# wing02/MyLdpcCppApi

Measured on AMD Instinct MI355X. Metric: decoded Mbit/s (info bits), DVB-S2 N=64800 rate-1/2, 50 iters, higher is better.
Workload: dtype f32; 1 GPU; DVB-S2-profile (64800,32400) rate-1/2 (seeded IRA table with the standard's structure, E=226799), batch 4096 frames per GPU, 50 iterations, sum-product fp32 (probability domain), all-zero codeword + AWGN sigma=0.95 (no frame converges), early termination on, inputs resident in HBM; global_batch=4096, frames_per_gpu=4096, algo=sp, frames_per_launch=4096, parallelism=frames sharded over 1 GPU(s), all-gather of decoded bytes, frames_converged=0

## Files before the change

include/ldpc_hip.h:

```cpp
#ifndef LDPC_HIP_H_
#define LDPC_HIP_H_

#include <stddef.h>
#include <stdint.h>

#ifdef __cplusplus
extern "C" {
#endif

#define LDPC_HIP_ABI_VERSION 3

enum ldpc_status {
    LDPC_OK = 0,
    LDPC_ERR_ARG = 1,
    LDPC_ERR_HIP = 2,
    LDPC_ERR_NOMEM = 3,
    LDPC_ERR_UNSUPPORTED = 4,
    LDPC_ERR_STATE = 5
};

enum ldpc_algo {
    LDPC_ALGO_SP = 0,
    LDPC_ALGO_MS = 1,
    LDPC_ALGO_LAYERED = 2,
// ... 75 lines not shown

typedef struct ldpc_decode_stats {
    int32_t iterations_launched;
    int32_t batch_time;
    int64_t frames;
    int64_t frames_converged;
    float ms_total;
    float ms_check;
    float ms_var;
    float ms_other;
    int32_t launches_check;
    int32_t launches_var;
    int64_t frame_rounds;
} ldpc_decode_stats;

int ldpc_abi_version(void);
const char *ldpc_last_error(void);
int ldpc_device_count(int *count);

int ldpc_graph_create(const int32_t *rows, const int32_t *cols, int64_t E, int32_t M, int32_t N,
                      ldpc_graph **out);
int ldpc_graph_destroy(ldpc_graph *g);
int ldpc_graph_info(const ldpc_graph *g, int32_t *M, int32_t *N, int64_t *E, int32_t *max_row_deg,
                    int32_t *max_col_deg);

void ldpc_decoder_config_init(ldpc_decoder_config *cfg);
int ldpc_decoder_config_init_sized(ldpc_decoder_config *cfg, uint32_t struct_size);
#define ldpc_decoder_config_init(cfg) ((void)ldpc_decoder_config_init_sized((cfg), (uint32_t)sizeof(ldpc_decoder_config)))
int ldpc_decoder_create(const ldpc_graph *g, const ldpc_decoder_config *cfg, ldpc_decoder **out);
int ldpc_decoder_create_multi(const ldpc_graph *g, const ldpc_decoder_config *cfg, const int32_t *devices,
                              int32_t n_devices, ldpc_decoder **out);
int ldpc_decoder_destroy(ldpc_decoder *d);
int ldpc_shard_range(int64_t frames, int32_t part, int32_t parts, int32_t unit, int64_t *lo, int64_t *hi);

int ldpc_decode(ldpc_decoder *d, const float *llr_host, int64_t frames, uint8_t *out_host,
                int64_t out_bytes, int32_t *iters);

int ldpc_decode_device(ldpc_decoder *d, const float *llr_dev, int64_t frames, uint8_t *out_dev,
                       int64_t out_bytes, int32_t *iters_dev, void *stream);

int64_t ldpc_out_bytes(int32_t K, int64_t frames, int32_t pack_mode);

enum ldpc_soft_kind { LDPC_SOFT_POSTERIOR = 1, LDPC_SOFT_EXTRINSIC = 2 };
int ldpc_decode_soft_device(ldpc_decoder *d, const float *llr_dev, int64_t frames, uint8_t *out_dev, int64_t out_bytes,
                            int32_t *iters_dev, float *soft_dev, int64_t soft_floats, int32_t soft_kind, void *stream);
int ldpc_decode_soft(ldpc_decoder *d, const float *llr_host, int64_t frames, uint8_t *out_host, int64_t out_bytes,
                     int32_t *iters, float *soft_host, int64_t soft_floats, int32_t soft_kind);

enum ldpc_llr_type { LDPC_LLR_F32 = 0, LDPC_LLR_F16 = 1, LDPC_LLR_I8 = 2 };
int ldpc_decode_typed_device(ldpc_decoder *d, const void *llr_dev, int32_t llr_type, float llr_unit, int64_t frames,
                             uint8_t *out_dev, int64_t out_bytes, int32_t *iters_dev, void *stream);
int ldpc_decode_soft_typed_device(ldpc_decoder *d, const void *llr_dev, int32_t llr_type, float llr_unit, int64_t frames,
                                  uint8_t *out_dev, int64_t out_bytes, int32_t *iters_dev, float *soft_dev,
                                  int64_t soft_floats, int32_t soft_kind, void *stream);
int ldpc_decode_typed(ldpc_decoder *d, const void *llr_host, int32_t llr_type, float llr_unit, int64_t frames,
                      uint8_t *out_host, int64_t out_bytes, int32_t *iters);
int ldpc_decode_soft_typed(ldpc_decoder *d, const void *llr_host, int32_t llr_type, float llr_unit, int64_t frames,
                           uint8_t *out_host, int64_t out_bytes, int32_t *iters, float *soft_host, int64_t soft_floats,
                           int32_t soft_kind);
int ldpc_llr_quantize_device(const float *y_dev, int64_t count, int32_t llr_type, float llr_unit, void *out_dev,
                             int32_t device, void *stream);

int ldpc_decoder_set_timing(ldpc_decoder *d, int enable);
int ldpc_decoder_stats(ldpc_decoder *d, ldpc_decode_stats *stats);
int ldpc_decoder_crc_stops(ldpc_decoder *d, int64_t *frames);

typedef struct ldpc_kernel_time {
    int32_t phase;
    int32_t degree;
    int32_t launches;
    float ms_total;
    int64_t bytes_total;
    char name[64];
    int64_t bytes_moved;
} ldpc_kernel_time;
int ldpc_decoder_kernel_times(ldpc_decoder *d, ldpc_kernel_time *out, int32_t capacity,
                              int32_t *count);

int ldpc_decoder_link_form(ldpc_decoder *d, int32_t *form, int32_t *calibrated, float ms[3]);

int ldpc_decoder_placement(ldpc_decoder *d, int32_t *candidates, int32_t *kept, float ms[16]);
int ldpc_decoder_array_addresses(ldpc_decoder *d, uint64_t out[4]);

int ldpc_decoder_set_tap(ldpc_decoder *d, int32_t iter);
int ldpc_decoder_dump(ldpc_decoder *d, int32_t which, float *host_out, int64_t count);

int ldpc_awgn_device(float *llr_dev, int64_t frames, int32_t N, const uint8_t *bits_dev, float sd,
                     uint64_t seed, int64_t first_frame, int32_t device, void *stream);
int ldpc_count_errors_device(const uint8_t *out_dev, const uint8_t *ref_dev, int64_t frames,
                             int64_t bytes_per_frame, int64_t errors[3], int32_t device, void *stream);

typedef struct ldpc_encoder ldpc_encoder;
enum ldpc_code_format {
    LDPC_CODE_PACKED = 0,
    LDPC_CODE_BITS = 1
};
enum ldpc_parity_kind { LDPC_PARITY_DUAL_DIAGONAL = 1, LDPC_PARITY_STAIRCASE = 2, LDPC_PARITY_DENSE = 3  };
int ldpc_parity_structure(const ldpc_graph *g, int32_t K, int32_t block_rows, int32_t out[8]);
int ldpc_encoder_create(const ldpc_graph *g, int32_t K, int32_t block_rows, int32_t max_frames, int32_t device,
                        ldpc_encoder **out);
int ldpc_encoder_destroy(ldpc_encoder *e);
int ldpc_encode_device(ldpc_encoder *e, const uint8_t *src_dev, int64_t src_bytes, int64_t frames, uint8_t *code_dev,
                       int64_t code_bytes, int32_t format, void *stream);
int ldpc_encode(ldpc_encoder *e, const uint8_t *src_host, int64_t src_bytes, uint8_t *code_host, int64_t code_bytes);
int64_t ldpc_code_bytes(int32_t N, int64_t frames, int32_t format);

int ldpc_graph_systematic_order(const ldpc_graph *g, int32_t *perm , int32_t *rank);
int ldpc_parity_dense(const ldpc_graph *g, int32_t K, int64_t out[4]);
int ldpc_parity_dense_rows(const ldpc_graph *g, int32_t K, int32_t first, int32_t rows, uint64_t *t_out, int64_t words);
int ldpc_encoder_create_dense(const ldpc_graph *g, int32_t K, int32_t max_frames, int32_t device, ldpc_encoder **out);

typedef struct ldpc_rate_spec {
    uint32_t struct_size;
    int32_t  N;
    int32_t  punctured;
    int32_t  filler_lo, filler_hi;
    float    fill_llr;
    float    erasure_llr;
} ldpc_rate_spec;
void ldpc_rate_spec_init(ldpc_rate_spec *spec, int32_t N);
int ldpc_rate_lengths(const ldpc_rate_spec *spec, int32_t *Ncb, int32_t *L);
int ldpc_rate_index(const ldpc_rate_spec *spec, int32_t k0, int32_t E, int32_t *index_out);
int ldpc_rate_match_device(const ldpc_rate_spec *spec, const uint8_t *code_dev, int32_t code_format, int64_t frames, int32_t k0,
                           int32_t E, uint8_t *tx_dev, int64_t tx_bytes, int32_t tx_format, int32_t device, void *stream);
int ldpc_rate_recover_device(const ldpc_rate_spec *spec, const float *rx_dev, int64_t frames, int32_t k0, int32_t E, float *soft_dev,
                             int32_t accumulate, float *y_dev, int32_t device, void *stream);
int ldpc_rate_match(const ldpc_rate_spec *spec, const uint8_t *code_host, int32_t code_format, int64_t frames, int32_t k0, int32_t E,
                    uint8_t *tx_host, int64_t tx_bytes, int32_t tx_format, int32_t device);
int ldpc_rate_recover(const ldpc_rate_spec *spec, const float *rx_host, int64_t frames, int32_t k0, int32_t E, float *soft_host,
                      int32_t accumulate, float *y_host, int32_t device);

typedef struct ldpc_modem_spec {
    uint32_t struct_size;
    int32_t  Qm;
    int32_t  interleave;
} ldpc_modem_spec;
void ldpc_modem_spec_init(ldpc_modem_spec *spec, int32_t Qm);
int64_t ldpc_modem_symbol_floats(const ldpc_modem_spec *spec, int32_t E);
int ldpc_modem_index(const ldpc_modem_spec *spec, int32_t E, int32_t *index_out);
int ldpc_modem_points(int32_t Qm, float *iq);
int ldpc_modem_transmit_device(const ldpc_modem_spec *spec, const uint8_t *tx_dev, int32_t tx_format, int64_t frames, int32_t E,
                               float sd, uint64_t seed, int64_t first_frame, float *sym_dev, int64_t sym_floats, int32_t device,
                               void *stream);
int ldpc_modem_demap_device(const ldpc_modem_spec *spec, const float *sym_dev, int64_t frames, int32_t E, float *rx_dev,
                            int32_t device, void *stream);
int ldpc_modem_transmit(const ldpc_modem_spec *spec, const uint8_t *tx_host, int32_t tx_format, int64_t frames, int32_t E, float sd,
                        uint64_t seed, int64_t first_frame, float *sym_host, int64_t sym_floats, int32_t device);
int ldpc_modem_demap(const ldpc_modem_spec *spec, const float *sym_host, int64_t frames, int32_t E, float *rx_host, int32_t device);

enum ldpc_crc_kind { LDPC_CRC16 = 16, LDPC_CRC24A = 24, LDPC_CRC24B = 25 };
typedef struct ldpc_tb_spec {
    uint32_t struct_size;
    int32_t  A;
    int32_t  tb_crc;
    int32_t  C;
    int32_t  cb_crc;
    int32_t  K;
} ldpc_tb_spec;
void ldpc_tb_spec_init(ldpc_tb_spec *spec, int32_t A, int32_t K);
int ldpc_tb_layout(const ldpc_tb_spec *spec, int32_t out[6]);
int ldpc_crc_bits(int32_t kind, const uint8_t *bytes, int64_t nbits, uint32_t *crc);
int ldpc_crc_weights(int32_t kind, int32_t nbits, uint32_t *w);
int ldpc_tb_frame_crc(const ldpc_tb_spec *spec, int32_t *kind, int32_t *bits);
int ldpc_tb_attach_device(const ldpc_tb_spec *spec, const uint8_t *payload_dev, int64_t tbs, uint8_t *src_dev, int64_t src_bytes,
                          int32_t device, void *stream);
int ldpc_tb_check_device(const ldpc_tb_spec *spec, const uint8_t *dec_dev, int64_t tbs, uint8_t *payload_dev, uint8_t *cb_ok_dev,
// ... 50 lines not shown
```

myldpccppapi_amd/_lib.py:

```python
import ctypes
import os
import sys

_HERE = os.path.dirname(os.path.abspath(__file__))
LIB_PATH = os.environ.get("LDPC_HIP_LIB") or os.path.join(_HERE, "libldpc_hip.so")
_lib = None


class LdpcError(RuntimeError):
    def __init__(self, code, message):
        super().__init__("ldpc_hip error %d: %s" % (code, message))
        self.code = code


class DecoderConfig(ctypes.Structure):
    _fields_ = [("struct_size", ctypes.c_uint32), ("K", ctypes.c_int32),
                ("max_batch", ctypes.c_int32), ("algo", ctypes.c_int32),
                ("msg_dtype", ctypes.c_int32), ("max_iter", ctypes.c_int32),
                ("llr_scale", ctypes.c_float), ("early_term", ctypes.c_int32),
                ("device", ctypes.c_int32), ("layer_rows", ctypes.c_int32),
                ("pack_mode", ctypes.c_int32), ("frames_per_lane", ctypes.c_int32),
                ("poll_interval", ctypes.c_int32),
                ("tune_flags", ctypes.c_int32), ("tune_rows_per_wave", ctypes.c_int32),
                ("tune_cols_per_wave", ctypes.c_int32), ("tune_link_rows", ctypes.c_int32),
                ("tune_compact", ctypes.c_int32), ("tune_ldsp_grid", ctypes.c_int32),
                ("tune_ldsp_shape", ctypes.c_int32), ("tune_place", ctypes.c_int32),
                ("host_input", ctypes.c_int32),
                ("host_copy_threads", ctypes.c_int32), ("tune_q_order", ctypes.c_int32),
                ("ms_scale", ctypes.c_float), ("ms_offset", ctypes.c_float)]


class DecoderConfigCrc(DecoderConfig):
    _fields_ = [("crc_kind", ctypes.c_int32), ("crc_bits", ctypes.c_int32)]


class _MsgTail(ctypes.Union):
    _fields_ = [("msg_reserved", ctypes.c_int32 * 3), ("post_bits", ctypes.c_int32)]


class DecoderConfigMsg(DecoderConfigCrc):
    _anonymous_ = ("_tail",)
    _fields_ = [("msg_bits", ctypes.c_int32), ("_tail", _MsgTail)]


class DecodeStats(ctypes.Structure):
    _fields_ = [("iterations_launched", ctypes.c_int32), ("batch_time", ctypes.c_int32),
                ("frames", ctypes.c_int64), ("frames_converged", ctypes.c_int64),
                ("ms_total", ctypes.c_float), ("ms_check", ctypes.c_float),
                ("ms_var", ctypes.c_float), ("ms_other", ctypes.c_float),
                ("launches_check", ctypes.c_int32), ("launches_var", ctypes.c_int32),
                ("frame_rounds", ctypes.c_int64)]


class KernelTime(ctypes.Structure):
    _fields_ = [("phase", ctypes.c_int32), ("degree", ctypes.c_int32), ("launches", ctypes.c_int32),
                ("ms_total", ctypes.c_float), ("bytes_total", ctypes.c_int64), ("name", ctypes.c_char * 64),
                ("bytes_moved", ctypes.c_int64)]


class RateSpec(ctypes.Structure):
    _fields_ = [("struct_size", ctypes.c_uint32), ("N", ctypes.c_int32), ("punctured", ctypes.c_int32),
                ("filler_lo", ctypes.c_int32), ("filler_hi", ctypes.c_int32),
                ("fill_llr", ctypes.c_float), ("erasure_llr", ctypes.c_float)]


class ModemSpec(ctypes.Structure):
    _fields_ = [("struct_size", ctypes.c_uint32), ("Qm", ctypes.c_int32), ("interleave", ctypes.c_int32)]


class TbSpec(ctypes.Structure):
    _fields_ = [("struct_size", ctypes.c_uint32), ("A", ctypes.c_int32), ("tb_crc", ctypes.c_int32), ("C", ctypes.c_int32),
                ("cb_crc", ctypes.c_int32), ("K", ctypes.c_int32)]


class BchSpec(ctypes.Structure):
    _fields_ = [("struct_size", ctypes.c_uint32), ("m", ctypes.c_int32), ("prim", ctypes.c_uint32), ("t", ctypes.c_int32),
                ("n", ctypes.c_int32), ("row_bytes", ctypes.c_int32)]


EXPORTS = (
    "ldpc_abi_version", "ldpc_last_error", "ldpc_device_count", "ldpc_graph_create",
    "ldpc_graph_destroy", "ldpc_graph_info", "ldpc_decoder_config_init", "ldpc_decoder_create",
    "ldpc_decoder_create_multi", "ldpc_shard_range", "ldpc_decoder_destroy", "ldpc_decode", "ldpc_decode_device", "ldpc_out_bytes",
    "ldpc_decoder_set_timing", "ldpc_decoder_stats", "ldpc_decoder_kernel_times", "ldpc_decoder_set_tap",
    "ldpc_decoder_dump", "ldpc_awgn_device", "ldpc_count_errors_device", "ldpc_hbm_probe_device", "ldpc_hbm_sustained_device",
    "ldpc_host_block_plan", "ldpc_host_locked_ranges", "ldpc_decoder_link_form", "ldpc_decoder_placement", "ldpc_decoder_array_addresses",
    "ldpc_parity_structure", "ldpc_encoder_create", "ldpc_encoder_destroy", "ldpc_encode_device", "ldpc_encode", "ldpc_code_bytes",
    "ldpc_rate_spec_init", "ldpc_rate_lengths", "ldpc_rate_index", "ldpc_rate_match_device", "ldpc_rate_recover_device",
    "ldpc_rate_match", "ldpc_rate_recover",
    "ldpc_modem_spec_init", "ldpc_modem_symbol_floats", "ldpc_modem_index", "ldpc_modem_points", "ldpc_modem_transmit_device",
    "ldpc_modem_demap_device", "ldpc_modem_transmit", "ldpc_modem_demap",
    "ldpc_tb_spec_init", "ldpc_tb_layout", "ldpc_crc_bits", "ldpc_tb_attach_device", "ldpc_tb_check_device", "ldpc_tb_tally_device",
    "ldpc_tb_attach", "ldpc_tb_check",
    "ldpc_decoder_crc_stops", "ldpc_crc_weights", "ldpc_tb_frame_crc", "ldpc_decoder_config_init_sized",
    "ldpc_decode_soft_device", "ldpc_decode_soft",
    "ldpc_decode_typed_device", "ldpc_decode_soft_typed_device", "ldpc_decode_typed", "ldpc_decode_soft_typed",
    "ldpc_llr_quantize_device",
    "ldpc_bch_spec_init", "ldpc_bch_layout", "ldpc_bch_generator", "ldpc_bch_encode_device", "ldpc_bch_decode_device",
    "ldpc_bch_tally_device", "ldpc_bch_encode", "ldpc_bch_decode",
    "ldpc_osd_create", "ldpc_osd_destroy", "ldpc_osd_device", "ldpc_osd_run", "ldpc_osd_info",
    "ldpc_graph_systematic_order", "ldpc_parity_dense", "ldpc_parity_dense_rows", "ldpc_encoder_create_dense",
)


def load():
    global _lib
    if _lib is not None:
        return _lib
    if not os.path.exists(LIB_PATH):
        raise OSError("%s not built: run `python -c 'import __graft_entry__ as g; g.build()'` "
                      "or `make -C myldpccppapi_amd/csrc`" % LIB_PATH)
    if "torch" not in sys.modules:
        try:
            import torch
        except Exception:
            pass
    L = ctypes.CDLL(LIB_PATH, mode=ctypes.RTLD_GLOBAL)
    i32p = ctypes.POINTER(ctypes.c_int32)
    i64p = ctypes.POINTER(ctypes.c_int64)
    vp = ctypes.c_void_p
    L.ldpc_abi_version.restype = ctypes.c_int
    L.ldpc_last_error.restype = ctypes.c_char_p
    L.ldpc_device_count.argtypes = [ctypes.POINTER(ctypes.c_int)]
    L.ldpc_graph_create.argtypes = [i32p, i32p, ctypes.c_int64, ctypes.c_int32, ctypes.c_int32,
                                    ctypes.POINTER(vp)]
    L.ldpc_graph_destroy.argtypes = [vp]
    L.ldpc_graph_info.argtypes = [vp, i32p, i32p, i64p, i32p, i32p]
    L.ldpc_decoder_config_init.argtypes = [ctypes.POINTER(DecoderConfig)]
    L.ldpc_decoder_config_init.restype = None
    L.ldpc_decoder_config_init_sized.argtypes = [ctypes.POINTER(DecoderConfig), ctypes.c_uint32]
    L.ldpc_decoder_create.argtypes = [vp, ctypes.POINTER(DecoderConfig), ctypes.POINTER(vp)]
    L.ldpc_decoder_create_multi.argtypes = [vp, ctypes.POINTER(DecoderConfig), i32p, ctypes.c_int32,
                                            ctypes.POINTER(vp)]
    L.ldpc_shard_range.argtypes = [ctypes.c_int64, ctypes.c_int32, ctypes.c_int32, ctypes.c_int32, i64p, i64p]
    L.ldpc_decoder_destroy.argtypes = [vp]
    L.ldpc_decode.argtypes = [vp, vp, ctypes.c_int64, vp, ctypes.c_int64, vp]
    L.ldpc_decode_device.argtypes = [vp, vp, ctypes.c_int64, vp, ctypes.c_int64, vp, vp]
    L.ldpc_decode_soft.argtypes = [vp, vp, ctypes.c_int64, vp, ctypes.c_int64, vp, vp, ctypes.c_int64, ctypes.c_int32]
    L.ldpc_decode_soft_device.argtypes = [vp, vp, ctypes.c_int64, vp, ctypes.c_int64, vp, vp, ctypes.c_int64, ctypes.c_int32, vp]
    f32, i32 = ctypes.c_float, ctypes.c_int32
    L.ldpc_decode_typed.argtypes = [vp, vp, i32, f32, ctypes.c_int64, vp, ctypes.c_int64, vp]
    L.ldpc_decode_typed_device.argtypes = [vp, vp, i32, f32, ctypes.c_int64, vp, ctypes.c_int64, vp, vp]
    L.ldpc_decode_soft_typed.argtypes = [vp, vp, i32, f32, ctypes.c_int64, vp, ctypes.c_int64, vp, vp, ctypes.c_int64, i32]
    L.ldpc_decode_soft_typed_device.argtypes = [vp, vp, i32, f32, ctypes.c_int64, vp, ctypes.c_int64, vp, vp, ctypes.c_int64, i32, vp]
    L.ldpc_llr_quantize_device.argtypes = [vp, ctypes.c_int64, i32, f32, vp, i32, vp]
    L.ldpc_out_bytes.argtypes = [ctypes.c_int32, ctypes.c_int64, ctypes.c_int32]
    L.ldpc_out_bytes.restype = ctypes.c_int64
    L.ldpc_decoder_set_timing.argtypes = [vp, ctypes.c_int]
    L.ldpc_decoder_stats.argtypes = [vp, ctypes.POINTER(DecodeStats)]
    L.ldpc_decoder_kernel_times.argtypes = [vp, ctypes.POINTER(KernelTime), ctypes.c_int32, i32p]
    L.ldpc_decoder_set_tap.argtypes = [vp, ctypes.c_int32]
    L.ldpc_decoder_dump.argtypes = [vp, ctypes.c_int32, vp, ctypes.c_int64]
    L.ldpc_awgn_device.argtypes = [vp, ctypes.c_int64, ctypes.c_int32, vp, ctypes.c_float, ctypes.c_uint64,
                                   ctypes.c_int64, ctypes.c_int32, vp]
    L.ldpc_count_errors_device.argtypes = [vp, vp, ctypes.c_int64, ctypes.c_int64, i64p, ctypes.c_int32, vp]
    L.ldpc_hbm_sustained_device.argtypes = [ctypes.c_int32, ctypes.c_int64, ctypes.c_int32, ctypes.POINTER(ctypes.c_double)]
    L.ldpc_hbm_probe_device.argtypes = [ctypes.c_int32, ctypes.c_int64, ctypes.c_int32,
                                        ctypes.POINTER(ctypes.c_double), ctypes.POINTER(ctypes.c_double)]
    L.ldpc_host_block_plan.argtypes = [ctypes.c_uint64, ctypes.c_int64, ctypes.c_int32, ctypes.c_int32, ctypes.c_int64,
                                       ctypes.POINTER(ctypes.c_uint64)]
    L.ldpc_host_locked_ranges.argtypes = [i64p, i64p]
    L.ldpc_decoder_array_addresses.argtypes = [vp, ctypes.POINTER(ctypes.c_uint64)]
    L.ldpc_decoder_placement.argtypes = [vp, i32p, i32p, ctypes.POINTER(ctypes.c_float)]
    L.ldpc_decoder_link_form.argtypes = [vp, i32p, i32p, ctypes.POINTER(ctypes.c_float)]
    L.ldpc_parity_structure.argtypes = [vp, ctypes.c_int32, ctypes.c_int32, i32p]
    L.ldpc_encoder_create.argtypes = [vp, ctypes.c_int32, ctypes.c_int32, ctypes.c_int32, ctypes.c_int32, ctypes.POINTER(vp)]
    L.ldpc_encoder_destroy.argtypes = [vp]
    L.ldpc_encode_device.argtypes = [vp, vp, ctypes.c_int64, ctypes.c_int64, vp, ctypes.c_int64, ctypes.c_int32, vp]
    L.ldpc_encode.argtypes = [vp, vp, ctypes.c_int64, vp, ctypes.c_int64]
    L.ldpc_code_bytes.argtypes = [ctypes.c_int32, ctypes.c_int64, ctypes.c_int32]
    L.ldpc_code_bytes.restype = ctypes.c_int64
    rsp = ctypes.POINTER(RateSpec)
    L.ldpc_rate_spec_init.argtypes = [rsp, ctypes.c_int32]
    L.ldpc_rate_spec_init.restype = None
    L.ldpc_rate_lengths.argtypes = [rsp, i32p, i32p]
    L.ldpc_rate_index.argtypes = [rsp, ctypes.c_int32, ctypes.c_int32, vp]
    L.ldpc_rate_match_device.argtypes = [rsp, vp, ctypes.c_int32, ctypes.c_int64, ctypes.c_int32, ctypes.c_int32, vp,
                                         ctypes.c_int64, ctypes.c_int32, ctypes.c_int32, vp]
    L.ldpc_rate_recover_device.argtypes = [rsp, vp, ctypes.c_int64, ctypes.c_int32, ctypes.c_int32, vp, ctypes.c_int32, vp,
                                           ctypes.c_int32, vp]
    L.ldpc_rate_match.argtypes = [rsp, vp, ctypes.c_int32, ctypes.c_int64, ctypes.c_int32, ctypes.c_int32, vp,
                                  ctypes.c_int64, ctypes.c_int32, ctypes.c_int32]
    L.ldpc_rate_recover.argtypes = [rsp, vp, ctypes.c_int64, ctypes.c_int32, ctypes.c_int32, vp, ctypes.c_int32, vp,
                                    ctypes.c_int32]
    msp = ctypes.POINTER(ModemSpec)
    L.ldpc_modem_spec_init.argtypes = [msp, ctypes.c_int32]
    L.ldpc_modem_spec_init.restype = None
    L.ldpc_modem_symbol_floats.argtypes = [msp, ctypes.c_int32]
    L.ldpc_modem_symbol_floats.restype = ctypes.c_int64
    L.ldpc_modem_index.argtypes = [msp, ctypes.c_int32, vp]
    L.ldpc_modem_points.argtypes = [ctypes.c_int32, vp]
    L.ldpc_modem_transmit_device.argtypes = [msp, vp, ctypes.c_int32, ctypes.c_int64, ctypes.c_int32, ctypes.c_float, ctypes.c_uint64,
                                             ctypes.c_int64, vp, ctypes.c_int64, ctypes.c_int32, vp]
    L.ldpc_modem_demap_device.argtypes = [msp, vp, ctypes.c_int64, ctypes.c_int32, vp, ctypes.c_int32, vp]
    L.ldpc_modem_transmit.argtypes = [msp, vp, ctypes.c_int32, ctypes.c_int64, ctypes.c_int32, ctypes.c_float, ctypes.c_uint64,
                                      ctypes.c_int64, vp, ctypes.c_int64, ctypes.c_int32]
    L.ldpc_modem_demap.argtypes = [msp, vp, ctypes.c_int64, ctypes.c_int32, vp, ctypes.c_int32]
    tsp = ctypes.POINTER(TbSpec)
    L.ldpc_tb_spec_init.argtypes = [tsp, ctypes.c_int32, ctypes.c_int32]
    L.ldpc_tb_spec_init.restype = None
    L.ldpc_tb_layout.argtypes = [tsp, i32p]
    L.ldpc_crc_bits.argtypes = [ctypes.c_int32, vp, ctypes.c_int64, ctypes.POINTER(ctypes.c_uint32)]
    L.ldpc_tb_attach_device.argtypes = [tsp, vp, ctypes.c_int64, vp, ctypes.c_int64, ctypes.c_int32, vp]
    L.ldpc_tb_check_device.argtypes = [tsp, vp, ctypes.c_int64, vp, vp, vp, ctypes.c_int32, vp]
    L.ldpc_tb_tally_device.argtypes = [vp, vp, vp, ctypes.c_int64, ctypes.c_int64, i64p, ctypes.c_int32, vp]
    L.ldpc_tb_attach.argtypes = [tsp, vp, ctypes.c_int64, vp, ctypes.c_int64, ctypes.c_int32]
    L.ldpc_tb_check.argtypes = [tsp, vp, ctypes.c_int64, vp, vp, vp, ctypes.c_int32]
    L.ldpc_decoder_crc_stops.argtypes = [vp, i64p]
    L.ldpc_crc_weights.argtypes = [ctypes.c_int32, ctypes.c_int32, vp]
    L.ldpc_tb_frame_crc.argtypes = [tsp, i32p, i32p]
    bsp = ctypes.POINTER(BchSpec)
    L.ldpc_bch_spec_init.argtypes = [bsp, ctypes.c_int32, ctypes.c_int32, ctypes.c_int32]
    L.ldpc_bch_spec_init.restype = None
    L.ldpc_bch_layout.argtypes = [bsp, i32p]
    L.ldpc_bch_generator.argtypes = [ctypes.c_int32, ctypes.c_uint32, ctypes.c_int32, vp, ctypes.c_int32, i32p]
    L.ldpc_bch_encode_device.argtypes = [bsp, vp, ctypes.c_int64, vp, ctypes.c_int64, ctypes.c_int32, vp]
    L.ldpc_bch_decode_device.argtypes = [bsp, vp, ctypes.c_int64, vp, vp, ctypes.c_int32, vp]
    L.ldpc_bch_tally_device.argtypes = [vp, vp, vp, ctypes.c_int64, ctypes.c_int64, i64p, ctypes.c_int32, vp]
    L.ldpc_bch_encode.argtypes = [bsp, vp, ctypes.c_int64, vp, ctypes.c_int64, ctypes.c_int32]
    L.ldpc_bch_decode.argtypes = [bsp, vp, ctypes.c_int64, vp, vp, ctypes.c_int32]
    L.ldpc_osd_create.argtypes = [vp, i32, i32, i32, ctypes.POINTER(vp)]
    L.ldpc_osd_destroy.argtypes = [vp]
    L.ldpc_osd_device.argtypes = [vp, vp, ctypes.c_int64, i32, f32, vp, ctypes.c_int64, vp, vp, vp, vp]
    L.ldpc_osd_run.argtypes = [vp, vp, ctypes.c_int64, i32, f32, vp, ctypes.c_int64, vp, vp, vp]
    L.ldpc_osd_info.argtypes = [vp, i32p]
    L.ldpc_graph_systematic_order.argtypes = [vp, vp, i32p]
    L.ldpc_parity_dense.argtypes = [vp, i32, i64p]
    L.ldpc_parity_dense_rows.argtypes = [vp, i32, i32, i32, vp, ctypes.c_int64]
    L.ldpc_encoder_create_dense.argtypes = [vp, i32, i32, i32, ctypes.POINTER(vp)]
    _lib = L
    return L


def check(rc):
    if rc != 0:
        raise LdpcError(rc, load().ldpc_last_error().decode("utf-8", "replace"))
```

myldpccppapi_amd/capi.py:

```python
import ctypes

import numpy as np

from . import _lib
from ._lib import DecoderConfig, DecodeStats, LdpcError

ALGO_SP, ALGO_MS, ALGO_LAYERED, ALGO_MS_FUSED, ALGO_LAYERED_HOST, ALGO_BP, ALGO_LAYERED_BP = 0, 1, 2, 3, 4, 5, 6
ALGO_LAYERED_FX = 8
MSG_F32, MSG_F16, MSG_F8, MSG_I8 = 0, 1, 2, 4
PACK_BYTES, PACK_BITS = 0, 1
CODE_PACKED, CODE_BITS = 0, 1
CODE_FORMATS = {"packed": CODE_PACKED, "bits": CODE_BITS}
PARITY_KINDS = {1: "dual_diagonal", 2: "staircase", 3: "dense"}
HOST_INPUT = {"auto": 0, "staged": 1, "lock_pages": 2}
SOFT_POSTERIOR, SOFT_EXTRINSIC = 1, 2
SOFT_KINDS = {"posterior": SOFT_POSTERIOR, "extrinsic": SOFT_EXTRINSIC}
LLR_F32, LLR_F16, LLR_I8 = 0, 1, 2
LLR_TYPES = {"f32": LLR_F32, "f16": LLR_F16, "i8": LLR_I8}
LLR_DTYPES = {np.dtype(np.float32): LLR_F32, np.dtype(np.float16): LLR_F16, np.dtype(np.int8): LLR_I8}
ALGOS = {"sp": ALGO_SP, "ms": ALGO_MS, "layered": ALGO_LAYERED, "ms_fused": ALGO_MS_FUSED,
         "layered_host": ALGO_LAYERED_HOST, "bp": ALGO_BP, "layered_bp": ALGO_LAYERED_BP, "layered_fx": ALGO_LAYERED_FX}

TUNE_FIELDS = {"fused": 0, "ldsp": 2, "ldsp_ext": 4, "ldsp_pack": 6, "link_narrow": 8, "check_wide": 10,
               "syn_xcd": 12, "fused_pack": 14, "fused_loop": 16, "device_tail": 18, "merge": 20, "link_deep": 22, "link_half": 24,
               "link_guided": 26, "tiles_first": 28}
TUNE_INTS = ("rows_per_wave", "cols_per_wave", "link_rows", "compact", "ldsp_grid", "ldsp_per_cu", "ldsp_waves", "place", "q_order")


def apply_tune(cfg, tune):
    flags, shape = 0, 0
    for k, v in (tune or {}).items():
        if k in TUNE_FIELDS:
            if v is not None:
                flags |= (1 if v else 2) << TUNE_FIELDS[k]
        elif k == "ldsp_per_cu":
            shape |= int(v) & 255
        elif k == "ldsp_waves":
            shape |= (int(v) & 255) << 8
        elif k in TUNE_INTS:
            setattr(cfg, "tune_" + k, int(v))
        else:
            raise KeyError("unknown tuning field %r" % k)
    cfg.tune_flags, cfg.tune_ldsp_shape = flags, shape


def hbm_probe(device=0, nbytes=1 << 30, reps=5, by_policy=False):
    g = ctypes.c_double(0.0)
    two = (ctypes.c_double * 2)(0.0, 0.0)
    _lib.check(_lib.load().ldpc_hbm_probe_device(int(device), int(nbytes), int(reps), ctypes.byref(g), two))
    return (g.value, two[0], two[1]) if by_policy else g.value


def hbm_sustained(device=0, nbytes=1 << 30, milliseconds=300):
    g = ctypes.c_double(0.0)
    _lib.check(_lib.load().ldpc_hbm_sustained_device(int(device), int(nbytes), int(milliseconds), ctypes.byref(g)))
    return g.value


def tune_from_env(env=None):
    import os
    env = os.environ if env is None else env
    t = {}
    for name, key in (("FUSED", "fused"), ("LDSP", "ldsp"), ("LDSP_EXT", "ldsp_ext"), ("LDSP_PACK", "ldsp_pack"),
                      ("LINK_NARROW", "link_narrow"), ("CHECK_WIDE", "check_wide"), ("SYN_XCD", "syn_xcd"),
                      ("FUSED_LOOP", "fused_loop"), ("DEVICE_TAIL", "device_tail"), ("MERGE", "merge"), ("LINK_DEEP", "link_deep"), ("LINK_HALF", "link_half"),
                      ("LINK_GUIDED", "link_guided"), ("TILES_FIRST", "tiles_first")):
        if "LDPC_TUNE_" + name in env:
            t[key] = int(env["LDPC_TUNE_" + name]) != 0
    if "LDPC_TUNE_NO_PACK" in env:
        t["fused_pack"] = False
    for name, key in (("RPW", "rows_per_wave"), ("CPW", "cols_per_wave"), ("LDSP_GRID", "ldsp_grid"),
                      ("LDSP_PER_CU", "ldsp_per_cu"), ("LDSP_WAVES", "ldsp_waves")):
        if "LDPC_TUNE_" + name in env:
            t[key] = int(env["LDPC_TUNE_" + name])
    for name, key in (("LINK_RPW", "link_rows"), ("COMPACT", "compact")):
        if "LDPC_TUNE_" + name in env:
            v = int(env["LDPC_TUNE_" + name])
            t[key] = v if v > 0 else -1
    return t


def shard_range(frames, part, parts, unit=1):
    lo, hi = ctypes.c_int64(), ctypes.c_int64()
    _lib.check(_lib.load().ldpc_shard_range(int(frames), int(part), int(parts), int(unit),
                                            ctypes.byref(lo), ctypes.byref(hi)))
    return lo.value, hi.value


def host_block_plan(base, frames, N, max_batch, group):
    out = (ctypes.c_uint64 * 6)()
    _lib.check(_lib.load().ldpc_host_block_plan(int(base), int(frames), int(N), int(max_batch), int(group), out))
    return tuple(int(x) for x in out)


def host_locked_ranges():
    a, b = ctypes.c_int64(-1), ctypes.c_int64(-1)
    _lib.check(_lib.load().ldpc_host_locked_ranges(ctypes.byref(a), ctypes.byref(b)))
    return a.value, b.value


def device_count():
    n = ctypes.c_int(0)
    rc = _lib.load().ldpc_device_count(ctypes.byref(n))
    return n.value if rc == 0 else 0


def quantize_device(y_ptr, count, llr_type, llr_unit, out_ptr, device=0, stream=None):
    _lib.check(_lib.load().ldpc_llr_quantize_device(y_ptr, int(count), LLR_TYPES.get(llr_type, llr_type), float(llr_unit), out_ptr,
                                                    int(device), stream))


def out_bytes(K, frames, pack_mode=PACK_BYTES):
    return int(_lib.load().ldpc_out_bytes(K, frames, pack_mode))


def code_bytes(N, frames, fmt="packed"):
    return int(_lib.load().ldpc_code_bytes(int(N), int(frames), CODE_FORMATS.get(fmt, fmt)))


def parity_structure(graph, K, block_rows=0):
    out = (ctypes.c_int32 * 8)()
    _lib.check(_lib.load().ldpc_parity_structure(graph._h, int(K), int(block_rows), out))
    return dict(kind=PARITY_KINDS[out[0]], c=out[1], x=out[2], a=out[3], b=out[4], ext_rows=out[5], z=out[6])
# ... 5 lines not shown
    _lib.check(_lib.load().ldpc_graph_systematic_order(graph._h, perm.ctypes.data, ctypes.byref(rank)))
    return perm, rank.value


def dense_parity(graph, K):
    out = (ctypes.c_int64 * 4)()
    _lib.check(_lib.load().ldpc_parity_dense(graph._h, int(K), out))
    return dict(rho=out[0], rank_hp=out[1], M=out[2], t_words=out[3])


def dense_parity_rows(graph, K, first, rows):
    tw = (graph.M + 63) // 64
    out = np.zeros((max(int(rows), 0), tw), np.uint64)
    _lib.check(_lib.load().ldpc_parity_dense_rows(graph._h, int(K), int(first), int(rows), out.ctypes.data, out.size))
    return out


class Graph:

    def __init__(self, rows, cols, M, N):
        L = _lib.load()
        self.rows = np.ascontiguousarray(rows, np.int32)
        self.cols = np.ascontiguousarray(cols, np.int32)
        if self.rows.shape != self.cols.shape or self.rows.ndim != 1:
            raise ValueError("rows and cols must be 1-D arrays of equal length")
        self.M, self.N, self.E = int(M), int(N), int(self.rows.size)
        self._h = ctypes.c_void_p()
        i32p = ctypes.POINTER(ctypes.c_int32)
        _lib.check(L.ldpc_graph_create(self.rows.ctypes.data_as(i32p), self.cols.ctypes.data_as(i32p),
                                       self.E, self.M, self.N, ctypes.byref(self._h)))

    def info(self):
        L = _lib.load()
        M, N, rd, cd = (ctypes.c_int32() for _ in range(4))
        E = ctypes.c_int64()
        _lib.check(L.ldpc_graph_info(self._h, ctypes.byref(M), ctypes.byref(N), ctypes.byref(E),
                                     ctypes.byref(rd), ctypes.byref(cd)))
        return dict(M=M.value, N=N.value, E=E.value, max_row_deg=rd.value, max_col_deg=cd.value)

    def close(self):
        h, self._h = getattr(self, "_h", None), None
        if h and _lib is not None and _lib._lib is not None:
            _lib._lib.ldpc_graph_destroy(h)

    def __del__(self):
        try:
            self.close()
        except Exception:
            pass


class Decoder:

    def __init__(self, graph, K, max_batch, algo="sp", max_iter=40, llr_scale=8.0, early_term=True,
                 device=0, layer_rows=0, pack_mode=PACK_BYTES, frames_per_lane=0, poll_interval=0,
                 msg_dtype=MSG_F32, tune=None, devices=None, host_input="auto", host_copy_threads=0,
                 ms_scale=0.0, ms_offset=0.0, crc_kind=0, crc_bits=0, msg_bits=0, post_bits=0):
        L = _lib.load()
        cfg = _lib.DecoderConfigMsg()
        _lib.check(L.ldpc_decoder_config_init_sized(ctypes.byref(cfg), ctypes.sizeof(cfg)))
        cfg.K, cfg.max_batch = int(K), int(max_batch)
        cfg.algo = ALGOS[algo] if isinstance(algo, str) else int(algo)
        cfg.msg_dtype = {"f32": MSG_F32, "f16": MSG_F16, "f8": MSG_F8, "i8": MSG_I8}.get(msg_dtype, msg_dtype)
        cfg.msg_bits = int(msg_bits)
        cfg.post_bits = int(post_bits)
        cfg.max_iter, cfg.llr_scale = int(max_iter), float(llr_scale)
        cfg.early_term, cfg.device, cfg.layer_rows = int(bool(early_term)), int(device), int(layer_rows)
        cfg.pack_mode, cfg.frames_per_lane, cfg.poll_interval = int(pack_mode), int(frames_per_lane), int(poll_interval)
        apply_tune(cfg, tune)
        cfg.host_input = HOST_INPUT[host_input] if isinstance(host_input, str) else int(host_input)
        cfg.host_copy_threads = int(host_copy_threads)
        cfg.ms_scale, cfg.ms_offset = float(ms_scale), float(ms_offset)
        cfg.crc_kind, cfg.crc_bits = int(CRC_KINDS.get(crc_kind, crc_kind)), int(crc_bits)
        self.cfg = cfg
        self.graph = graph
        self.K, self.N, self.E = int(K), graph.N, graph.E
        self._h = ctypes.c_void_p()
        if devices is None:
            _lib.check(L.ldpc_decoder_create(graph._h, ctypes.byref(cfg), ctypes.byref(self._h)))
        else:
            devs = (ctypes.c_int32 * len(devices))(*[int(x) for x in devices])
            _lib.check(L.ldpc_decoder_create_multi(graph._h, ctypes.byref(cfg), devs, len(devices),
                                                   ctypes.byref(self._h)))

    def decode(self, llr, want_iters=True, soft=None, llr_unit=None):
        L = _lib.load()
        if llr_unit is not None:
            llr = np.asarray(llr)
            if llr.dtype not in LLR_DTYPES:
                raise TypeError("llr_unit given: llr must be int8, float16 or float32, not %s" % llr.dtype)
            llr = np.ascontiguousarray(llr).reshape(-1, self.N)
            frames, ty = llr.shape[0], LLR_DTYPES[llr.dtype]
            out = np.zeros(out_bytes(self.K, frames, self.cfg.pack_mode), np.uint8)
            iters = np.zeros(frames, np.int32)
            if soft is None:
                _lib.check(L.ldpc_decode_typed(self._h, llr.ctypes.data, ty, float(llr_unit), frames, out.ctypes.data, out.size,
                                               iters.ctypes.data if want_iters else None))
                return out, iters
            vals = np.zeros((frames, self.N), np.float32)
            _lib.check(L.ldpc_decode_soft_typed(self._h, llr.ctypes.data, ty, float(llr_unit), frames, out.ctypes.data, out.size,
                                                iters.ctypes.data if want_iters else None, vals.ctypes.data, vals.size,
                                                SOFT_KINDS.get(soft, soft)))
            return out, iters, vals
        llr = np.ascontiguousarray(llr, np.float32).reshape(-1, self.N)
        frames = llr.shape[0]
        out = np.zeros(out_bytes(self.K, frames, self.cfg.pack_mode), np.uint8)
        iters = np.zeros(frames, np.int32)
        if soft is None:
            _lib.check(L.ldpc_decode(self._h, llr.ctypes.data, frames, out.ctypes.data, out.size,
                                     iters.ctypes.data if want_iters else None))
            return out, iters
        vals = np.zeros((frames, self.N), np.float32)
        _lib.check(L.ldpc_decode_soft(self._h, llr.ctypes.data, frames, out.ctypes.data, out.size,
                                      iters.ctypes.data if want_iters else None, vals.ctypes.data, vals.size,
                                      SOFT_KINDS.get(soft, soft)))
        return out, iters, vals

    def decode_device(self, llr_ptr, frames, out_ptr, out_nbytes, iters_ptr=None, stream=None, soft_ptr=None, soft_floats=0,
                      soft="posterior", llr_type=None, llr_unit=None):
        if llr_type is not None or llr_unit is not None:
            ty = LLR_TYPES.get(llr_type, llr_type) if llr_type is not None else LLR_F32
            unit = 1.0 if llr_unit is None else float(llr_unit)
            if soft_ptr is None and not soft_floats:
                _lib.check(_lib.load().ldpc_decode_typed_device(self._h, llr_ptr, ty, unit, frames, out_ptr, out_nbytes, iters_ptr,
                                                                stream))
            else:
                _lib.check(_lib.load().ldpc_decode_soft_typed_device(self._h, llr_ptr, ty, unit, frames, out_ptr, out_nbytes,
                                                                     iters_ptr, soft_ptr, int(soft_floats),
                                                                     SOFT_KINDS.get(soft, soft), stream))
        elif soft_ptr is None and not soft_floats:
            _lib.check(_lib.load().ldpc_decode_device(self._h, llr_ptr, frames, out_ptr, out_nbytes,
                                                      iters_ptr, stream))
        else:
            _lib.check(_lib.load().ldpc_decode_soft_device(self._h, llr_ptr, frames, out_ptr, out_nbytes, iters_ptr, soft_ptr,
                                                           int(soft_floats), SOFT_KINDS.get(soft, soft), stream))

    def set_timing(self, enable=True):
        _lib.check(_lib.load().ldpc_decoder_set_timing(self._h, int(enable)))

    def stats(self):
        st = DecodeStats()
        _lib.check(_lib.load().ldpc_decoder_stats(self._h, ctypes.byref(st)))
        return {f: getattr(st, f) for f, _ in st._fields_}

    def crc_stops(self):
        n = ctypes.c_int64(0)
        _lib.check(_lib.load().ldpc_decoder_crc_stops(self._h, ctypes.byref(n)))
        return n.value

    def kernel_times(self):
        arr = (_lib.KernelTime * 64)()
        n = ctypes.c_int32(0)
        _lib.check(_lib.load().ldpc_decoder_kernel_times(self._h, arr, 64, ctypes.byref(n)))
        return [dict(name=arr[i].name.decode(), phase=arr[i].phase, degree=arr[i].degree,
                     launches=arr[i].launches, ms_total=arr[i].ms_total, bytes_total=arr[i].bytes_total,
                     bytes_moved=arr[i].bytes_moved)
                for i in range(n.value)]

    def link_form(self):
        form, cal = ctypes.c_int32(-1), ctypes.c_int32(0)
        ms = (ctypes.c_float * 3)()
        _lib.check(_lib.load().ldpc_decoder_link_form(self._h, ctypes.byref(form), ctypes.byref(cal), ms))
        if form.value < 0:
            return None
        return {"form": ("wide", "narrow", "half")[form.value], "chosen_by_measurement": bool(cal.value),
                "ms_per_launch": {"wide": round(ms[0], 4), "narrow": round(ms[1], 4), "half": round(ms[2], 4)}}
# ... 365 lines not shown
```

myldpccppapi_amd/csrc/decoder.hpp:

```cpp
#pragma once

#include <hip/hip_runtime.h>
#include <stdint.h>

#include <memory>
#include <type_traits>
#include <vector>

#include "../../include/ldpc_hip.h"
#include "flood_tables.hpp"
#include "layered_kernels.hpp"
#include "fused_kernels.hpp"
#include "ldsp_kernels.hpp"
#include "engines.hpp"
#include "tune.hpp"
#include "host_stage.hpp"
#include "hip_host.hpp"

#ifndef LDPC_IDLE_FAT
#define LDPC_IDLE_FAT 8
#endif

namespace ldpc {

template <typename Fn> inline int dispatch_v(int V, Fn &&fn)
{
    return V == 1 ? fn(std::integral_constant<int, 1>{})
                  : V == 2 ? fn(std::integral_constant<int, 2>{}) : fn(std::integral_constant<int, 4>{});
}

template <typename Fn> inline void dispatch_msg(int msg_kind, Fn &&fn)
{
    if (msg_kind == LDPC_MSG_I8) fn(q8any{});
    else if (msg_kind == LDPC_MSG_F8) fn(f8{});
    else if (msg_kind == LDPC_MSG_F16) fn(_Float16{});
    else fn(float{});
}

struct RowClass {
    int degree = 0;
    int count = 0;
    DevBuf<int32_t> e0;
    std::vector<int32_t> h_e0;
    DevBuf<int32_t> link_col, link_pos;
    int linked = 0;
    int n_big = 0, small_rows = 1;
};
struct ColClass {
    int degree = 0;
    int count = 0;
    DevBuf<int32_t> col, edge;
    int64_t q_base = -1;
};

struct ClassGroup {
    int bucket = 0, lo = 0, hi = 0;
    int blocks = 0;
    int blocks_fat = 0;
    std::vector<int> members;
    DevBuf<GroupClass> table, table_fat;
};

constexpr int kIdleFat = LDPC_IDLE_FAT;

struct FloodPlan {
    DevBuf<uint8_t> chan, Q, R;
    int msg_size = 4;
    int msg_kind = LDPC_MSG_F32;
    int msg_bits = 0;
    DevBuf<int32_t> qpos, col_qedge;
    std::vector<int32_t> h_qpos;
    std::vector<RowClass> row_classes;
    std::vector<ColClass> col_classes;
    std::vector<ClassGroup> check_groups, var_groups;
    std::vector<int> check_solo, var_solo;
    DevBuf<int32_t> extra_e0, extra_deg;
    int n_extra = 0;
    int64_t extra_edges = 0;
    FloodFns fns;

    int link_form = 1;
    bool link_deep = false;
    bool syn_xcd = true;
    bool check_wide = false;
    int link_rpw = 16;
    int cus = 256;
    bool link_calibrated = false;
    float link_cal_ms[3] = {0, 0, 0};
    int place_candidates = 0, place_kept = 0;
    float place_ms[16] = {};

    bool tail_enabled = false;
    int TO = 0, TA = 0;
    DevBuf<int32_t> tail_state, tail_map, running;

    std::unique_ptr<ldpc_decoder> child;
    DevBuf<int32_t> cmap;
    DevBuf<int32_t> cinv;
    DevBuf<unsigned long long> cmoved;
    int child_capacity = kCompactCapacity;
    int compact_threshold = kCompactCapacity;
    bool is_child = false;
    ldpc_decoder *handed_to = nullptr;
    HostBuf<int32_t> h_active;
    DevBuf<int32_t> soft_map;

    HostBuf<int32_t> h_summary;
    Event ev_summary;
    bool summary_pending = false;
    int idle_after = 0;

    bool first_round_from_chan = false;
};

struct HostSlot {
    DevBuf<float> llr;
    DevBuf<uint8_t> out;
    DevBuf<int32_t> iters;
    HostBuf<uint8_t> h_out;
    HostBuf<int32_t> h_iters;
    DevBuf<float> soft;
    HostBuf<float> h_soft;
    HostBuf<uint8_t> h_head;
    Event h2d_done, all_done;
    bool busy = false;
    int64_t off = 0, n = 0, dst = 0, copy_bytes = 0;
    HostBuf<int32_t> h_sum;
    int g_iterations = 0, g_tiles = 0, g_children = 0, g_child_f[3] = {0, 0, 0};
};
struct RingChunk { HostBuf<uint8_t> h; Event ev; bool used = false; };
struct CallCounts { bool valid = false; int32_t iterations = 0, batch_time = 0; int64_t frames = 0, converged = 0, frame_rounds = 0, crc_stops = 0; };

struct HostPath {
    Stream copy_stream;
    HostSlot slot[3];
    CallCounts call;
    bool suppress_poll = false;
    std::vector<RingChunk> ring;
    size_t ring_next = 0;
    std::unique_ptr<Worker> stager;
    std::vector<std::unique_ptr<Worker>> copy_helpers;
    std::vector<Job> copy_jobs;
    Job stage_job[3];
    bool stage_pending[3] = {false, false, false};
    std::vector<void *> locked_blocks, stuck_blocks;
};

struct TimedSpan {
    Event a, b;
    int kind = 0;
    int degree = 0;
    int64_t bytes = 0;
    int64_t moved = 0;
    int lo = 0;
};

struct Timing {
    bool timing = false;
    int timing_every = 0;
    int64_t timing_calls = 0;
    std::vector<TimedSpan> spans;
// ... 105 lines not shown
```

myldpccppapi_amd/csrc/engine_flood.hip:

```cpp
#include <hip/hip_runtime.h>

#include <algorithm>
#include <map>
#include <vector>

#include "flood_round.hpp"
#include "flood_handover.hpp"
#include "crc_term_kernels.hpp"
#include "soft_kernels.hpp"
#include "decoder.hpp"
#include "graph.hpp"

using ldpc::set_error;

namespace {

using ldpc::DevBuf;
using ldpc::RowClass;
using ldpc::ColClass;
using ldpc::ClassGroup;
using ldpc::kIdleFat;
using ldpc::dispatch_v;
using ldpc::span_begin;
using ldpc::span_end;
using ldpc::kVarBuckets;
using ldpc::kCheckBuckets;
using ldpc::kVarBucketLo;
using ldpc::kVarBucketHi;
using ldpc::kCheckBucketLo;
using ldpc::kCheckBucketHi;

template <int V>
__global__ void summary_kernel(const int32_t *iters, const uint64_t *done, const uint64_t *fail,
                               int64_t frames, int32_t freeze, int32_t *summary)
{
    constexpr int F = 64 * V;
    const int64_t f = (int64_t)blockIdx.x * blockDim.x + threadIdx.x;
    if (f >= frames) return;
    const int64_t tile = f / F;
    const int fi = (int)(f % F);
    const int l = fi / V, v = fi % V;
    atomicMax(&summary[0], iters[f]);
    const uint64_t ok = freeze ? done[tile * V + v] : ~fail[tile * V + v];
    if ((ok >> l) & 1ull) atomicAdd(&summary[1], 1);
}

static inline dim3 flood_grid(const ldpc_decoder *d, unsigned blocks, unsigned tiles, int32_t *tiles_first, bool linked = false)
{
    const bool want = d->tune.tiles_first == 1 || (d->tune.tiles_first == 0 && linked);
    *tiles_first = (blocks <= 65535u && want) ? 1 : 0;
    return *tiles_first ? dim3(tiles, blocks) : dim3(blocks, tiles);
}

static ldpc::CheckArgs check_args(const ldpc_decoder *d, const ldpc::TailRef &tr, int rows_per_wave, bool from_chan,
                                  const int32_t *e0 = nullptr, int n_rows = 0, int degree = 0)
{
    ldpc::CheckArgs a{d->flood.Q.p, d->flood.R.p, e0, d->done.p, d->E, n_rows, rows_per_wave, degree, d->ms_scale, tr};
    a.ms_offset = d->ms_offset;
    a.qpos = d->flood.qpos.p;
    if (from_chan) { a.first_chan = d->flood.chan.p; a.edge_col = d->edge_col.p; a.N = d->N; }
    return a;
}

template <int V> int run_flooding(ldpc_decoder *d, const ldpc::LlrIn &llr, int64_t frames,
                                  uint8_t *out_dev, int64_t out_bytes, int32_t *iters_dev,
                                  hipStream_t s, int start_round = 1);

template <int V> int enqueue_check_phase(ldpc_decoder *d, hipStream_t s, int tiles, int64_t frames, int it, int max_iter,
                                         bool fat, const ldpc::TailRef &tr)
{
    using namespace ldpc;
    const int64_t msz = d->flood.msg_size;
    const bool from_chan = it == 1 && d->flood.first_round_from_chan;
    for (auto &rc : d->flood.row_classes) {
        if (!rc.linked) continue;
        LDPC_HIP_TRY(span_begin(d, s, 4, rc.degree,
                           (2 * msz * rc.degree * rc.count + msz * 5 * rc.linked + 2 * msz * d->flood.extra_edges) * frames,
                           msz * ((int64_t)rc.degree * rc.count + rc.linked +
                                  ((int64_t)rc.degree * rc.count - 2 * rc.linked) +
                                  (it < max_iter ? 2 * rc.linked : 0) + 2 * d->flood.extra_edges) * frames));
        CheckArgs a = check_args(d, tr, d->flood.link_rpw, false, rc.e0.p, rc.count, rc.degree);
        const bool soft_reads = d->soft.dst && (d->cfg.early_term || it == max_iter);
        LinkArgs lk{rc.link_col.p, rc.link_pos.p, d->flood.chan.p, d->flood.Q.p, d->hard.p, d->N,
                    (it < max_iter) ? 1 : 0, (d->tm.tap_iter || soft_reads) ? 1 : 0, d->flood.extra_e0.p, d->flood.extra_deg.p, d->flood.n_extra, 0,
                    rc.n_big, rc.small_rows};
        const int variant = (d->flood.link_form == 2 && !d->flood.fns.link_half[rc.degree]) ? 1 : d->flood.link_form;
        const int waves = link_chunk_count(d->flood.link_rpw, rc.n_big, rc.small_rows, rc.count) * (variant == 1 ? V : variant == 2 ? V / 2 : 1);
        lk.link_blocks = (waves + kWavesPerBlock - 1) / kWavesPerBlock;
        const dim3 grid = flood_grid(d, lk.link_blocks + (d->flood.n_extra + kWavesPerBlock - 1) / kWavesPerBlock, tiles, &a.tiles_first, true);
        (variant == 2 ? d->flood.fns.link_half : variant == 1 ? (d->flood.link_deep ? d->flood.fns.link_deep : d->flood.fns.link_narrow) : d->flood.fns.link)
            [rc.degree]<<<grid, kBlock, 0, s>>>(a, lk);
        LDPC_HIP_TRY(span_end(d, s));
    }
    for (auto &g : d->flood.check_groups) {
        int64_t edges = 0;
        for (int i : g.members) edges += (int64_t)d->flood.row_classes[i].degree * d->flood.row_classes[i].count;
        LDPC_HIP_TRY(span_begin(d, s, 5, g.hi, 2 * msz * edges * frames, -1, g.lo));
        CheckArgs a = check_args(d, tr, (d->tune.rows_per_wave ? d->tune.rows_per_wave : 2) * (fat ? kIdleFat : 1), from_chan);
        const dim3 grid = flood_grid(d, fat ? g.blocks_fat : g.blocks, tiles, &a.tiles_first);
        d->flood.fns.check_group[g.bucket]<<<grid, kBlock, 0, s>>>(a, fat ? g.table_fat.p : g.table.p, (int)g.members.size());
        LDPC_HIP_TRY(span_end(d, s));
    }
    for (int ci : d->flood.check_solo) {
        RowClass &rc = d->flood.row_classes[ci];
        LDPC_HIP_TRY(span_begin(d, s, 0, rc.degree, 2 * msz * rc.degree * rc.count * frames));
        const int slotk = rc.degree <= d->flood.fns.max_check_unrolled ? rc.degree : 0;
        const bool narrow = slotk && (!d->flood.check_wide || rc.degree > kMaxUnrolledDegree);
        const int rpw = (d->tune.rows_per_wave ? d->tune.rows_per_wave : (narrow ? 2 : 1)) * (fat ? kIdleFat : 1);
        CheckArgs a = check_args(d, tr, rpw, from_chan, rc.e0.p, rc.count, rc.degree);
        const int waves = ((rc.count + rpw - 1) / rpw) * (narrow ? V : 1);
        const dim3 grid = flood_grid(d, (waves + kWavesPerBlock - 1) / kWavesPerBlock, tiles, &a.tiles_first);
        (narrow ? d->flood.fns.check : d->flood.fns.check_wide)[slotk]<<<grid, kBlock, 0, s>>>(a);
        LDPC_HIP_TRY(span_end(d, s));
    }
    return LDPC_OK;
}

template <int V> int enqueue_var_phase(ldpc_decoder *d, hipStream_t s, int tiles, int64_t frames, int it, int max_iter,
                                       bool fat, const ldpc::TailRef &tr)
{
    using namespace ldpc;
    const int64_t msz = d->flood.msg_size;
    const int wq = (it < max_iter) ? 1 : 0;
    for (auto &g : d->flood.var_groups) {
        int64_t units = 0;
        for (int i : g.members) units += (int64_t)((wq ? 2 : 1) * d->flood.col_classes[i].degree + 1) * d->flood.col_classes[i].count;
        LDPC_HIP_TRY(span_begin(d, s, 6, g.hi, msz * units * frames, -1, g.lo));
        VarArgs a{d->flood.R.p, d->flood.Q.p, d->flood.chan.p, d->hard.p, d->done.p, nullptr, nullptr,
                  d->E, d->N, 0, (d->tune.cols_per_wave ? d->tune.cols_per_wave : 1) * (fat ? kIdleFat : 1), wq, 0, tr};
        const dim3 grid = flood_grid(d, fat ? g.blocks_fat : g.blocks, tiles, &a.tiles_first);
        d->flood.fns.var_group[g.bucket]<<<grid, kBlock, 0, s>>>(a, fat ? g.table_fat.p : g.table.p, (int)g.members.size());
        LDPC_HIP_TRY(span_end(d, s));
    }
    for (int ci : d->flood.var_solo) {
        ColClass &cc = d->flood.col_classes[ci];
        LDPC_HIP_TRY(span_begin(d, s, 1, cc.degree, msz * ((wq ? 2 : 1) * cc.degree + 1) * cc.count * frames));
        VarArgs a{d->flood.R.p, d->flood.Q.p, d->flood.chan.p, d->hard.p, d->done.p, cc.col.p, cc.edge.p,
                  d->E, d->N, cc.count, 1, wq, cc.degree, tr};
        const int cpw = (d->tune.cols_per_wave ? d->tune.cols_per_wave : 1) * (fat ? kIdleFat : 1);
        a.cols_per_wave = cpw;
        a.q_base = cc.q_base;
        const int slotk = cc.degree <= kMaxUnrolledDegree ? cc.degree : 0;
        const int waves = (cc.count + cpw - 1) / cpw;
        const dim3 grid = flood_grid(d, (waves + kWavesPerBlock - 1) / kWavesPerBlock, tiles, &a.tiles_first);
        d->flood.fns.var[slotk]<<<grid, kBlock, 0, s>>>(a);
        LDPC_HIP_TRY(span_end(d, s));
    }
    return LDPC_OK;
}

template <int V> int enqueue_soft(ldpc_decoder *d, hipStream_t s, int tiles, int64_t frames, const uint64_t *fail,
                                  const ldpc::TailRef &tr)
{
    using namespace ldpc;
    LDPC_HIP_TRY(span_begin(d, s, 7, 0, ((int64_t)d->flood.msg_size * (d->E + d->N) + 4 * (int64_t)d->N) * frames));
    SoftArgs a{d->flood.chan.p, d->flood.R.p, d->col_ptr.p, d->col_edge.p, d->done.p, fail, d->soft.dst, nullptr,
               d->soft.fmap, d->flood.tail_map.p, d->E, frames, d->N, d->soft.kind == LDPC_SOFT_EXTRINSIC ? 1 : 0, tr};
    const dim3 grid((unsigned)((d->N + kInitCols - 1) / kInitCols), (unsigned)tiles);
    dispatch_msg(d->flood.msg_kind, [&](auto t) { soft_settle_kernel<V, decltype(t)><<<grid, kBlock, 0, s>>>(a); });
    LDPC_HIP_TRY(span_end(d, s));
    return LDPC_OK;
}

template <int V> int compact_and_finish(ldpc_decoder *d, int64_t frames, int count, int it, hipStream_t s)
{
    using namespace ldpc;
    ldpc_decoder *c = d->flood.child.get();
    while (c->flood.child && count <= c->flood.child->cfg.max_batch) c = c->flood.child.get();
    const int cv = c->V, cf = 64 * cv;
    const unsigned ct = (unsigned)((count + cf - 1) / cf);
    const unsigned cg = ct * (unsigned)cv;
    if (cg > (unsigned)kBackWords) return set_error(LDPC_ERR_STATE, "hand-over of %d frames: more than %d mask words per column", count, kBackWords);
    LDPC_HIP_TRY(hipMemsetAsync(d->active.p, 0, sizeof(int32_t), s));
    compact_list_kernel<V><<<(unsigned)((frames + kBlock - 1) / kBlock), kBlock, 0, s>>>(d->done.p, frames, d->flood.cmap.p,
                                                                                         d->active.p, d->flood.child_capacity);
    const dim3 ge((unsigned)((d->E + kWavesPerBlock - 1) / kWavesPerBlock), cg);
    const dim3 gn((unsigned)((d->N + kWavesPerBlock - 1) / kWavesPerBlock), cg);
    const bool rowwise = count >= 128;
    const int ptiles = (int)((frames + 64 * V - 1) / (64 * V));
    dispatch_msg(d->flood.msg_kind, [&](auto t) {
        using T = decltype(t);
        const T *pq = (const T *)d->flood.Q.p, *pc = (const T *)d->flood.chan.p;
        T *cq = (T *)c->flood.Q.p, *cc = (T *)c->flood.chan.p;
        if (rowwise) {
            constexpr int rpb = gather_rows_per_block<T>();
            compact_gather_rows_kernel<V, T><<<(unsigned)((d->E + rpb - 1) / rpb), kBlock, 0, s>>>(pq, cq, d->flood.cmap.p, count, d->E, ptiles, cf, d->flood.qpos.p, c->flood.qpos.p);
            compact_gather_rows_kernel<V, T><<<(unsigned)((d->N + rpb - 1) / rpb), kBlock, 0, s>>>(pc, cc, d->flood.cmap.p, count, d->N, ptiles, cf);
        } else {
            compact_gather_kernel<V, T><<<ge, kBlock, 0, s>>>(pq, cq, d->flood.cmap.p, count, d->E, cf, d->flood.qpos.p, c->flood.qpos.p);
            compact_gather_kernel<V, T><<<gn, kBlock, 0, s>>>(pc, cc, d->flood.cmap.p, count, d->N, cf);
        }
    });
    LDPC_HIP_TRY(hipMemsetAsync(c->hard.p, 0, (size_t)ct * d->N * cv * sizeof(uint64_t), s));
    if (d->cfg.algo == LDPC_ALGO_SP) {
        if (ptiles * V <= kGatherParentWords && count <= 2 * kCompactCapacity)
            compact_hard_lds_kernel<V><<<(unsigned)((d->N + 63) / 64), kBlock, 0, s>>>(d->hard.p, c->hard.p, d->flood.cmap.p, count, d->N, cv, ptiles, (int)cg);
        else
            compact_hard_kernel<V><<<gn, kBlock, 0, s>>>(d->hard.p, c->hard.p, d->flood.cmap.p, count, d->N, cv);
    }
    compact_child_state_kernel<0><<<ct, 64, 0, s>>>(c->done.p, c->iters.p, count, d->cfg.max_iter, cv);
    LDPC_HIP_TRY(hipGetLastError());
    c->tm.timing = false;
    c->tm.tap_iter = 0;
    c->soft = SoftReq{};
    if (d->soft.dst) {
        LDPC_HIP_TRY(c->flood.soft_map.ensure((size_t)c->cfg.max_batch));
        soft_map_kernel<0><<<(unsigned)((count + kBlock - 1) / kBlock), kBlock, 0, s>>>(c->flood.soft_map.p, d->flood.cmap.p, d->soft.fmap, count);
        c->soft = SoftReq{d->soft.dst, d->soft.kind, c->flood.soft_map.p};
    }
    const int rc = dispatch_v(cv, [&](auto v) { return run_flooding<decltype(v)::value>(c, ldpc::LlrIn{}, count, nullptr, 0, nullptr, s, it + 1); });
    c->soft = SoftReq{};
    if (rc) return rc;
    d->flood.handed_to = c;
    LDPC_HIP_TRY(hipMemsetAsync(d->flood.cmoved.p, 0, d->flood.cmoved.n * sizeof(unsigned long long), s));
    compact_inverse_kernel<V><<<(unsigned)((count + 255) / 256), 256, 0, s>>>(d->flood.cmap.p, count, d->flood.cinv.p, d->flood.cmoved.p, cv);
    compact_hard_back_kernel<V><<<dim3((unsigned)((d->N + kBlock - 1) / kBlock), (unsigned)ptiles), kBlock, 0, s>>>(
        d->hard.p, c->hard.p, d->flood.cinv.p, d->flood.cmoved.p, d->N, cv, (int)cg);
    compact_finish_kernel<V><<<(unsigned)((count + 63) / 64), 64, 0, s>>>(d->done.p, d->iters.p, c->done.p, c->iters.p, d->flood.cmap.p, count, cv);
    LDPC_HIP_TRY(hipGetLastError());
    return LDPC_OK;
}

template <int V> int run_flooding(ldpc_decoder *d, const ldpc::LlrIn &llr, int64_t frames,
                                  uint8_t *out_dev, int64_t out_bytes, int32_t *iters_dev,
                                  hipStream_t s, int start_round)
{
    using namespace ldpc;
    const int F = 64 * V;
    const int tiles = (int)((frames + F - 1) / F);
    const int64_t msz = d->flood.msg_size;
    const int max_iter = d->cfg.max_iter;
    const int rounds = d->tm.tap_iter ? std::min(d->tm.tap_iter, max_iter) : max_iter;
    const bool freeze = d->cfg.early_term != 0;
    const size_t slot = (size_t)d->flood.TA * V;

    const bool resume = start_round > 1;
    LDPC_HIP_TRY(hipMemsetAsync(d->failw.p, 0, d->failw.n * sizeof(uint64_t), s));
    LDPC_HIP_TRY(hipMemsetAsync(d->summary.p, 0, 4 * sizeof(int32_t), s));
    d->flood.handed_to = nullptr;
    if (!resume && d->flood.summary_pending) {
        if (hipEventQuery(d->flood.ev_summary.e) == hipSuccess) {
            d->flood.summary_pending = false;
            d->flood.idle_after = (d->flood.h_summary.p[0] > 0 && d->flood.h_summary.p[0] < max_iter) ? d->flood.h_summary.p[0] + 1 : 0;
        } else {
            (void)hipGetLastError();
        }
    }
    const int idle_after = (freeze && !resume && !d->tm.tap_iter && d->cfg.poll_interval == 0) ? d->flood.idle_after : 0;
    const bool use_tail = d->flood.tail_enabled && freeze && !resume && !d->tm.tap_iter && tiles >= 4 * d->flood.TO;
    const TailRef tr{use_tail ? d->flood.tail_state.p : nullptr, d->T, d->flood.TO};
    TailArgs ta{};
    if (use_tail) {
        LDPC_HIP_TRY(hipMemsetAsync(d->flood.tail_state.p, 0, 4 * sizeof(int32_t), s));
        LDPC_HIP_TRY(hipMemsetAsync(d->flood.running.p, 0, d->flood.running.n * sizeof(int32_t), s));
        ta = TailArgs{d->flood.tail_state.p, d->flood.tail_map.p, d->flood.running.p, d->done.p, d->iters.p, d->flood.Q.p, d->flood.chan.p, d->hard.p,
                      d->E, frames, d->N, tiles, d->T, d->flood.TO * F, std::min(d->flood.compact_threshold, d->flood.TO * F), 0, max_iter};
    }

    bool q_less = (d->cfg.algo == LDPC_ALGO_MS || d->cfg.algo == LDPC_ALGO_BP) && !resume && !d->tm.tap_iter && max_iter > 1 && d->flood.n_extra == 0;
    for (auto &rc : d->flood.row_classes) if (rc.linked) q_less = false;
    for (int ci : d->flood.check_solo) if (d->flood.row_classes[ci].degree > d->flood.fns.max_check_unrolled) q_less = false;
    d->flood.first_round_from_chan = q_less;
    if (!resume) {
        LDPC_HIP_TRY(span_begin(d, s, 3));
        InitArgs a{llr.p, d->flood.chan.p, q_less ? nullptr : d->flood.Q.p, d->hard.p, d->col_ptr.p, d->flood.col_qedge.p,
                   d->E, frames, d->N, d->cfg.llr_scale, llr.unit};
        dim3 grid((d->N + kInitCols - 1) / kInitCols, tiles);
        d->flood.fns.init_in[llr.type]<<<grid, kBlock, 0, s>>>(a);
        StateArgs st{d->done.p, nullptr, d->iters.p, nullptr, frames, 0, max_iter, freeze ? 1 : 0};
        state_kernel<V><<<use_tail ? d->flood.TA : tiles, 64, 0, s>>>(st);
        LDPC_HIP_TRY(span_end(d, s));
    }

    int launched = start_round - 1;
    bool poll_dense = false;
    for (int it = start_round; it <= rounds; ++it) {
        const bool fat = idle_after > 0 && it > idle_after;
        {
            const int rcp = enqueue_check_phase<V>(d, s, tiles, frames, it, max_iter, fat, tr);
            if (rcp) return rcp;
        }
        {
            const int rcv = enqueue_var_phase<V>(d, s, tiles, frames, it, max_iter, fat, tr);
            if (rcv) return rcv;
        }
        launched = it;
        if (freeze || it == rounds) {
            LDPC_HIP_TRY(span_begin(d, s, 3));
            uint64_t *fw = d->failw.p + (size_t)it * slot;
            const int rbk = (d->M + kBlock - 1) / kBlock;
            SyndromeArgs sa{d->row_ptr.p, d->edge_col.p, d->hard.p, fw, d->done.p, d->M, d->N,
                            d->flood.syn_xcd ? tiles : 0, rbk, tr};
            dim3 sgrid = d->flood.syn_xcd ? dim3(8 * rbk * ((tiles + 7) / 8)) : dim3(rbk, tiles);
            syndrome_kernel<V><<<sgrid, kBlock, 0, s>>>(sa);
            if (d->cfg.crc_kind) {
                CrcTermArgs ca{d->hard.p, fw, d->done.p, d->crc_w.p, d->summary.p + 3, d->N, d->cfg.crc_bits, tr};
                crc_term_kernel<V><<<dim3((unsigned)tiles, V), 64 * crc_term_waves(d->cfg.crc_bits), 0, s>>>(ca);
            }
            if (d->soft.dst) {
                LDPC_HIP_TRY(span_end(d, s));
                const int rcs = enqueue_soft<V>(d, s, tiles, frames, (freeze && it < rounds) ? fw : nullptr, tr);
                if (rcs) return rcs;
                LDPC_HIP_TRY(span_begin(d, s, 3));
            }
            StateArgs st{d->done.p, fw, d->iters.p, nullptr, frames, it, max_iter, 1, tr, use_tail ? d->flood.running.p : nullptr,
                         d->summary.p + 2};
            const bool poll = freeze && it < rounds && d->cfg.poll_interval > 0 && !d->host.suppress_poll &&
                              ((it % d->cfg.poll_interval) == 0 || poll_dense);
            if (poll) {
                LDPC_HIP_TRY(hipMemsetAsync(d->active.p, 0, sizeof(int32_t), s));
                st.active = d->active.p;
            }
            state_kernel<V><<<tiles, 64, 0, s>>>(st);
            if (use_tail && it < rounds) {
                ta.iter = it;
                const unsigned tg = (unsigned)std::min<int64_t>(1024, d->E + 2 * (int64_t)d->N);
                dispatch_msg(d->flood.msg_kind, [&](auto t) { tail_gather_kernel<V, decltype(t)><<<tg, kBlock, 0, s>>>(ta); });
            }
            LDPC_HIP_TRY(span_end(d, s));
            if (poll) {
                LDPC_HIP_TRY(hipMemcpyAsync(d->flood.h_active.p, d->active.p, sizeof(int32_t),
                                       hipMemcpyDeviceToHost, s));
                LDPC_HIP_TRY(hipStreamSynchronize(s));
                const int running = *d->flood.h_active.p;
                if (running == 0) break;
                if ((int64_t)running * 10 <= frames * 9 && d->flood.child && tiles > 1 &&
                    (double)d->E * (double)frames * 4.0 * (double)msz > 1.5e9) poll_dense = true;
                if (d->flood.child && running <= d->flood.compact_threshold && (int64_t)running * 4 <= frames && tiles > 1 && !d->tm.tap_iter) {
                    const int rc = compact_and_finish<V>(d, frames, running, it, s);
                    if (rc) return rc;
                    launched = d->flood.handed_to->last_iterations;
                    break;
                }
            }
        }
    }
    d->last_iterations = launched;
    d->last_tiles = tiles;
    if (resume) return LDPC_OK;

    LDPC_HIP_TRY(span_begin(d, s, 3));
    if (use_tail) tail_scatter_kernel<V><<<2048, kBlock, 0, s>>>(ta);
    {
        PackArgs pa{d->hard.p, out_dev, d->iters.p, iters_dev, frames, out_bytes, d->N, d->cfg.K,
                    d->cfg.pack_mode};
        const bool pack = (out_dev || iters_dev) && frames;
        if (d->cfg.pack_mode == LDPC_PACK_BYTES) {
            if (pack) pack_kernel<V><<<pack_grid<V>(d->cfg.K, tiles), kBlock, 0, s>>>(pa);
        } else {
            const int64_t n = std::max<int64_t>(out_bytes, frames);
            dim3 grid((unsigned)((n + kBlock - 1) / kBlock));
            if (pack) pack_kernel<V><<<grid, kBlock, 0, s>>>(pa);
        }
        summary_kernel<V><<<(unsigned)((frames + 255) / 256), 256, 0, s>>>(
            d->iters.p, d->done.p, d->failw.p, frames, 1, d->summary.p);
        if (!d->flood.is_child && d->cfg.poll_interval == 0 && freeze && !d->flood.summary_pending) {
            LDPC_HIP_TRY(hipMemcpyAsync(d->flood.h_summary.p, d->summary.p, 2 * sizeof(int32_t), hipMemcpyDeviceToHost, s));
            LDPC_HIP_TRY(hipEventRecord(d->flood.ev_summary.e, s));
            d->flood.summary_pending = true;
        }
    }
    LDPC_HIP_TRY(span_end(d, s));
    LDPC_HIP_TRY(hipGetLastError());
    return LDPC_OK;
}

int build_classes(ldpc_decoder *d, const ldpc_graph *g)
{
    std::map<int, std::vector<int32_t>> rows_by_deg, cols_by_deg, rowids_by_deg;
    for (int32_t m = 0; m < g->M; ++m) {
        const int deg = g->row_ptr[m + 1] - g->row_ptr[m];
        if (deg > 0) { rows_by_deg[deg].push_back(g->row_ptr[m]); rowids_by_deg[deg].push_back(m); }
    }
    std::vector<char> fused_col((size_t)g->N, 0);
    d->flood.row_classes.resize(rows_by_deg.size());
    size_t i = 0;
    for (auto &kv : rows_by_deg) {
// ... 44 lines not shown
                for (int idx = 0; idx < rc.count; ++idx)
                    if (lcol[idx] >= 0) fused_col[lcol[idx]] = 0;
                rc.linked = 0;
            }
        }
    }
    for (int32_t n = 0; n < g->N; ++n) {
        const int deg = g->col_ptr[n + 1] - g->col_ptr[n];
        if (!fused_col[n]) cols_by_deg[deg].push_back(n);
    }
    d->flood.col_classes.resize(cols_by_deg.size());
    i = 0;
    for (auto &kv : cols_by_deg) {
        ColClass &cc = d->flood.col_classes[i++];
        cc.degree = kv.first;
        cc.count = (int)kv.second.size();
        std::vector<int32_t> edges;
        edges.reserve((size_t)cc.count * std::max(cc.degree, 1));
        for (int32_t n : kv.second)
            for (int32_t p = g->col_ptr[n]; p < g->col_ptr[n + 1]; ++p) edges.push_back(g->col_edge[p]);
        if (edges.empty()) edges.push_back(0);
        LDPC_HIP_TRY(cc.col.upload(kv.second));
        LDPC_HIP_TRY(cc.edge.upload(edges));
    }
    {
        d->flood.h_qpos.assign((size_t)g->E, -1);
        int64_t slot = 0;
        if (d->tune.q_order >= 0)
            for (ColClass &cc : d->flood.col_classes) {
                cc.q_base = slot;
                const std::vector<int32_t> &members = cols_by_deg[cc.degree];
                for (size_t ci = 0; ci < members.size(); ++ci)
                    for (int k = 0; k < cc.degree; ++k)
                        d->flood.h_qpos[(size_t)g->col_edge[(size_t)g->col_ptr[members[ci]] + k]] = (int32_t)(slot + (int64_t)k * cc.count + (int64_t)ci);
                slot += (int64_t)cc.degree * cc.count;
            }
        for (int64_t e = 0; e < g->E; ++e)
            if (d->flood.h_qpos[(size_t)e] < 0) d->flood.h_qpos[(size_t)e] = d->tune.q_order >= 0 ? (int32_t)slot++ : (int32_t)e;
        std::vector<int32_t> cq((size_t)g->E);
        for (int64_t p = 0; p < g->E; ++p) cq[(size_t)p] = d->flood.h_qpos[(size_t)g->col_edge[(size_t)p]];
        LDPC_HIP_TRY(d->flood.qpos.upload(d->flood.h_qpos));
        LDPC_HIP_TRY(d->flood.col_qedge.upload(cq));
    }
    return LDPC_OK;
}

int plan_launches(ldpc_decoder *d)
{
    using ldpc::GroupClass;
    const int V = d->V;
    const bool merge = ldpc::tune_pick(d->tune.merge, true) && !d->flood.check_wide;
    d->flood.check_groups.clear(); d->flood.var_groups.clear(); d->flood.check_solo.clear(); d->flood.var_solo.clear();
    d->flood.n_extra = 0; d->flood.extra_edges = 0;
    int linked_classes = 0;
    int64_t unlinked_rows = 0;
    for (auto &rc : d->flood.row_classes) { if (rc.linked) ++linked_classes; else unlinked_rows += rc.count; }
    const bool as_extra = merge && linked_classes == 1 && unlinked_rows > 0 && unlinked_rows <= 64;
    std::vector<int> cb[kCheckBuckets], vb[kVarBuckets];
    std::vector<int32_t> xe0, xdeg;
    for (int i = 0; i < (int)d->flood.row_classes.size(); ++i) {
        RowClass &rc = d->flood.row_classes[i];
        if (rc.linked) continue;
        if (as_extra) {
            for (int32_t e : rc.h_e0) { xe0.push_back(e); xdeg.push_back(rc.degree); d->flood.extra_edges += rc.degree; }
            continue;
        }
        int b = -1;
        for (int k = 0; k < kCheckBuckets; ++k)
            if (rc.degree >= kCheckBucketLo[k] && rc.degree <= kCheckBucketHi[k] && rc.degree <= d->flood.fns.max_check_unrolled &&
                d->flood.fns.check_group[k]) b = k;
        if (merge && b >= 0) cb[b].push_back(i); else d->flood.check_solo.push_back(i);
    }
    if (as_extra) {
        d->flood.n_extra = (int)xe0.size();
        LDPC_HIP_TRY(d->flood.extra_e0.upload(xe0));
        LDPC_HIP_TRY(d->flood.extra_deg.upload(xdeg));
    }
    for (int i = 0; i < (int)d->flood.col_classes.size(); ++i) {
        const ColClass &cc = d->flood.col_classes[i];
        int b = -1;
        for (int k = 0; k < kVarBuckets; ++k)
            if (cc.degree >= kVarBucketLo[k] && cc.degree <= kVarBucketHi[k] && d->flood.fns.var_group[k]) b = k;
        if (merge && b >= 0) vb[b].push_back(i); else d->flood.var_solo.push_back(i);
    }
    const int rpw = d->tune.rows_per_wave ? d->tune.rows_per_wave : 2, cpw = d->tune.cols_per_wave ? d->tune.cols_per_wave : 1;
    auto make = [&](std::vector<ClassGroup> &groups, std::vector<int> &solo, const std::vector<int> &members, int bucket,
                    int lo, int hi, bool rows) -> hipError_t {
        if (members.size() < 2) { for (int i : members) solo.push_back(i); return hipSuccess; }
        groups.emplace_back();
        ClassGroup &g = groups.back();
        g.bucket = bucket; g.lo = lo; g.hi = hi; g.members = members;
        std::vector<GroupClass> tab, tabf;
        constexpr int fatk = kIdleFat;
        for (int i : members) {
            GroupClass gc{};
            if (rows) {
                const RowClass &rc = d->flood.row_classes[i];
                gc.degree = rc.degree; gc.count = rc.count; gc.ids = rc.e0.p; gc.edges = nullptr; gc.q_base = -1;
            } else {
                const ColClass &cc = d->flood.col_classes[i];
                gc.degree = cc.degree; gc.count = cc.count; gc.ids = cc.col.p; gc.edges = cc.edge.p; gc.q_base = cc.q_base;
            }
            auto blocks_of = [&](int per_wave) {
                const int waves = ((gc.count + per_wave - 1) / per_wave) * (rows ? V / d->flood.fns.check_group_width : 1);
                return (waves + ldpc::kWavesPerBlock - 1) / ldpc::kWavesPerBlock;
            };
            gc.block_begin = g.blocks;
            tab.push_back(gc);
            g.blocks += blocks_of(rows ? rpw : cpw);
            gc.block_begin = g.blocks_fat;
            tabf.push_back(gc);
            g.blocks_fat += blocks_of((rows ? rpw : cpw) * fatk);
        }
        const hipError_t e = g.table.upload(tab);
        return e != hipSuccess ? e : g.table_fat.upload(tabf);
    };
    for (int k = 0; k < kCheckBuckets; ++k) LDPC_HIP_TRY(make(d->flood.check_groups, d->flood.check_solo, cb[k], k, kCheckBucketLo[k], kCheckBucketHi[k], true));
    for (int k = 0; k < kVarBuckets; ++k) LDPC_HIP_TRY(make(d->flood.var_groups, d->flood.var_solo, vb[k], k, kVarBucketLo[k], kVarBucketHi[k], false));
    return LDPC_OK;
}

int setup_flooding(ldpc_decoder *d, const ldpc_graph *g, size_t TF)
{
    const ldpc_decoder_config *cfg = &d->cfg;
    const bool i8 = cfg->msg_dtype == LDPC_MSG_I8;
    d->flood.msg_kind = cfg->msg_dtype;
    d->flood.msg_bits = i8 ? (cfg->msg_bits ? cfg->msg_bits : 8) : 0;
    d->flood.msg_size = (i8 || cfg->msg_dtype == LDPC_MSG_F8) ? 1 : cfg->msg_dtype == LDPC_MSG_F16 ? 2 : 4;
    LDPC_HIP_TRY(d->flood.chan.alloc(TF * d->N * d->flood.msg_size));
    LDPC_HIP_TRY(d->flood.Q.alloc(TF * (size_t)d->E * d->flood.msg_size));
    LDPC_HIP_TRY(d->flood.R.alloc(TF * (size_t)d->E * d->flood.msg_size));
    int rc = build_classes(d, g);
    if (rc) return rc;
    ldpc::FloodFns *fns = &d->flood.fns;
    if (cfg->algo == LDPC_ALGO_SP) ldpc::fill_flood_sp(d->V, fns);
    else if (i8) {
        const int q = d->flood.msg_bits;
        if (d->ms_corr) (q == 4 ? ldpc::fill_flood_msci4 : q == 5 ? ldpc::fill_flood_msci5 : q == 6 ? ldpc::fill_flood_msci6 : ldpc::fill_flood_msci8)(d->V, fns);
        else (q == 4 ? ldpc::fill_flood_msi4 : q == 5 ? ldpc::fill_flood_msi5 : q == 6 ? ldpc::fill_flood_msi6 : ldpc::fill_flood_msi8)(d->V, fns);
    }
    else if (cfg->algo == LDPC_ALGO_BP && cfg->msg_dtype == LDPC_MSG_F16) ldpc::fill_flood_bp16(d->V, fns);
    else if (cfg->algo == LDPC_ALGO_BP) ldpc::fill_flood_bp(d->V, fns);
    else if (d->ms_corr && cfg->msg_dtype == LDPC_MSG_F8) ldpc::fill_flood_msc8(d->V, fns);
    else if (cfg->msg_dtype == LDPC_MSG_F8) ldpc::fill_flood_ms8(d->V, fns);
    else if (d->ms_corr && cfg->msg_dtype == LDPC_MSG_F16) ldpc::fill_flood_msc16(d->V, fns);
    else if (d->ms_corr) ldpc::fill_flood_msc(d->V, fns);
    else if (cfg->msg_dtype == LDPC_MSG_F16) ldpc::fill_flood_ms16(d->V, fns);
    else ldpc::fill_flood_ms(d->V, fns);
    return plan_launches(d);
}

template <int V> int calibrate_link(ldpc_decoder *d)
{
    using namespace ldpc;
    RowClass *rcp = nullptr;
    for (auto &rc : d->flood.row_classes) if (rc.linked) rcp = &rc;
    if (!rcp || !d->flood.fns.link[rcp->degree] || !d->flood.fns.link_narrow[rcp->degree]) return LDPC_OK;
    RowClass &rc = *rcp;
    const int tiles = d->T;
    hipStream_t s = d->stream.s;
    LDPC_HIP_TRY(hipMemsetAsync(d->flood.Q.p, 0, d->flood.Q.n, s));
    LDPC_HIP_TRY(hipMemsetAsync(d->flood.chan.p, 0, d->flood.chan.n, s));
    LDPC_HIP_TRY(hipMemsetAsync(d->done.p, 0, d->done.n * sizeof(uint64_t), s));
    ldpc::Event ev[2];
    LDPC_HIP_TRY(ev[0].create());
    LDPC_HIP_TRY(ev[1].create());
    float best[3] = {1e30f, 1e30f, 1e30f};
    const int candidates = d->flood.fns.link_half[rc.degree] ? 3 : 2;
    const bool skip_narrow = d->flood.msg_size == 1;
    hipError_t err = hipSuccess;
    for (int rep = 0; rep < 4 && err == hipSuccess; ++rep) {
        for (int nar = 0; nar < candidates && err == hipSuccess; ++nar) {
            if (nar == 1 && skip_narrow) continue;
            CheckArgs a = check_args(d, TailRef{nullptr, 0, 0}, d->flood.link_rpw, false, rc.e0.p, rc.count, rc.degree);
            LinkArgs lk{rc.link_col.p, rc.link_pos.p, d->flood.chan.p, d->flood.Q.p, d->hard.p, d->N, 1, 0, nullptr, nullptr, 0, 0,
                        rc.n_big, rc.small_rows};
            const int waves = link_chunk_count(d->flood.link_rpw, rc.n_big, rc.small_rows, rc.count) * (nar == 1 ? V : nar == 2 ? V / 2 : 1);
            lk.link_blocks = (waves + kWavesPerBlock - 1) / kWavesPerBlock;
            const dim3 grid = flood_grid(d, lk.link_blocks, tiles, &a.tiles_first, true);
            err = hipEventRecord(ev[0].e, s);
            (nar == 2 ? d->flood.fns.link_half : nar == 1 ? d->flood.fns.link_narrow : d->flood.fns.link)[rc.degree]<<<grid, kBlock, 0, s>>>(a, lk);
            if (err == hipSuccess) err = hipEventRecord(ev[1].e, s);
            if (err == hipSuccess) err = hipEventSynchronize(ev[1].e);
            float ms = 0;
            if (err == hipSuccess) err = hipEventElapsedTime(&ms, ev[0].e, ev[1].e);
            if (err == hipSuccess && rep > 0 && ms < best[nar]) best[nar] = ms;
        }
    }
    if (err != hipSuccess) return set_error(LDPC_ERR_HIP, "link calibration: %s", hipGetErrorString(err));
    LDPC_HIP_TRY(hipGetLastError());
    int pick = 0;
    for (int k = 0; k < candidates; ++k) { d->flood.link_cal_ms[k] = best[k]; if (best[k] < best[pick]) pick = k; }
    d->flood.link_form = pick;
    d->flood.link_calibrated = true;
    return LDPC_OK;
}

template <int V> int time_check_phase(ldpc_decoder *d, float *ms_out)
{
    hipStream_t s = d->stream.s;
    LDPC_HIP_TRY(hipMemsetAsync(d->flood.Q.p, 0, d->flood.Q.n, s));
    LDPC_HIP_TRY(hipMemsetAsync(d->flood.chan.p, 0, d->flood.chan.n, s));
    LDPC_HIP_TRY(hipMemsetAsync(d->done.p, 0, d->done.n * sizeof(uint64_t), s));
    ldpc::Event ev[2];
    LDPC_HIP_TRY(ev[0].create());
    LDPC_HIP_TRY(ev[1].create());
    float best = 1e30f;
    hipError_t err = hipSuccess;
    int rc = LDPC_OK;
    for (int rep = 0; rep < 4 && err == hipSuccess && rc == LDPC_OK; ++rep) {
        err = hipEventRecord(ev[0].e, s);
        rc = enqueue_check_phase<V>(d, s, d->T, (int64_t)d->T * d->F, 1, d->cfg.max_iter, false, ldpc::TailRef{nullptr, 0, 0});
        if (rc == LDPC_OK)
            rc = enqueue_var_phase<V>(d, s, d->T, (int64_t)d->T * d->F, 1, d->cfg.max_iter, false, ldpc::TailRef{nullptr, 0, 0});
        if (err == hipSuccess) err = hipEventRecord(ev[1].e, s);
        if (err == hipSuccess) err = hipEventSynchronize(ev[1].e);
        float ms = 0;
        if (err == hipSuccess) err = hipEventElapsedTime(&ms, ev[0].e, ev[1].e);
        if (err == hipSuccess && rep > 0 && ms < best) best = ms;
    }
    if (rc) return rc;
    if (err != hipSuccess) return set_error(LDPC_ERR_HIP, "placement search: %s", hipGetErrorString(err));
    *ms_out = best;
    return LDPC_OK;
}

template <int V> int placement_search(ldpc_decoder *d, size_t TF)
{
    const size_t bq = TF * (size_t)d->E * d->flood.msg_size, bc = TF * d->N * d->flood.msg_size;
    const int want = d->tune.place == 0 ? (2 * bq + bc >= ((size_t)256 << 20) ? 6 : 1) : d->tune.place;
    if (want <= 1) return LDPC_OK;
    float best_ms = 0.0f;
    int rc = time_check_phase<V>(d, &best_ms);
    if (rc) return rc;
    std::vector<DevBuf<uint8_t>> held;
    d->flood.place_ms[0] = best_ms;
    d->flood.place_candidates = 1;
    d->flood.place_kept = 0;
    float lo = best_ms, hi = best_ms;
    for (int stage = 0; stage < 2; ++stage) {
        DevBuf<uint8_t> &arr = stage == 0 ? d->flood.R : d->flood.Q;
        for (int c = 1; c < want; ++c) {
            if (lo < 0.91f * hi && best_ms <= lo && d->flood.place_candidates >= 4) break;
            size_t free_b = 0, total_b = 0;
            if (hipMemGetInfo(&free_b, &total_b) != hipSuccess || free_b < 2 * bq + ((size_t)2 << 30)) break;
            DevBuf<uint8_t> cand, spacer;
            const size_t period = (size_t)16 << 30;
            if (c == 1 && arr.n < period && free_b > period + 2 * bq + ((size_t)2 << 30)) {
                if (spacer.alloc(period - arr.n) != hipSuccess) (void)hipGetLastError();
            }
            if (cand.alloc(arr.n) != hipSuccess) { (void)hipGetLastError(); break; }
            spacer.release();
            std::swap(arr, cand);
            float ms = 0.0f;
            rc = time_check_phase<V>(d, &ms);
            if (rc) return rc;
            if (d->flood.place_candidates < 16) d->flood.place_ms[d->flood.place_candidates] = ms;
            lo = std::min(lo, ms); hi = std::max(hi, ms);
            if (ms < best_ms) {
                best_ms = ms;
                d->flood.place_kept = d->flood.place_candidates;
            } else {
                std::swap(arr, cand);
            }
            ++d->flood.place_candidates;
            held.push_back(std::move(cand));
        }
    }
    return LDPC_OK;
}

}

int ldpc::engine_flood_setup(ldpc_decoder *d, const ldpc_graph *g, size_t TF, bool top_level)
{
    int rc = setup_flooding(d, g, TF);
    if (rc || !top_level) return rc;
    const ldpc::Tune &tune = d->tune;
    if (tune.link_narrow == 0 && tune.link_half == 0 && !tune.link_deep && d->V >= 2) {
        rc = dispatch_v(d->V, [&](auto v) { return calibrate_link<decltype(v)::value>(d); });
        if (rc) return rc;
    }
    return dispatch_v(d->V, [&](auto v) { return placement_search<decltype(v)::value>(d, TF); });
}

int ldpc::engine_flood_run(ldpc_decoder *d, const LlrIn &llr, int64_t frames, uint8_t *out_dev, int64_t out_bytes,
                           int32_t *iters_dev, hipStream_t s)
{
    return dispatch_v(d->V, [&](auto v) { return run_flooding<decltype(v)::value>(d, llr, frames, out_dev, out_bytes, iters_dev, s); });
}
```

myldpccppapi_amd/csrc/flood_check.hpp:

```cpp
#pragma once

#include "flood_common.hpp"

namespace ldpc {

template <int D, int V>
__device__ __forceinline__ void check_sp(const float (&x)[D][V], float (&out)[D][V])
{
#pragma unroll
    for (int v = 0; v < V; ++v) {
        if (D == 1) { out[0][v] = 1.0f; continue; }
        {
            float p = x[1][v];
#pragma unroll
            for (int j = 2; j < D; ++j) p *= x[j][v];
            out[0][v] = p;
        }
        float pre = x[0][v];
#pragma unroll
        for (int k = 1; k < D; ++k) {
            float p = pre;
#pragma unroll
            for (int j = k + 1; j < D; ++j) p *= x[j][v];
            out[k][v] = p;
// ... 3 lines not shown
}

template <int D, int V, bool CORR = false, typename T = float>
__device__ __forceinline__ void check_ms(const float (&x)[D][V], float (&out)[D][V], MsCorr c = MsCorr{1.0f, 0.0f})
{
#pragma unroll
    for (int v = 0; v < V; ++v) {
        float m1 = 1000.0f, m2 = 1000.0f;
        int idx = -1;
        unsigned par = 0;
#pragma unroll
        for (int j = 0; j < D; ++j) {
            const float a = __builtin_fabsf(x[j][v]);
            par ^= (x[j][v] < 0.0f) ? 1u : 0u;
            if (a < m1) { m2 = m1; m1 = a; idx = j; }
            else if (a < m2) { m2 = a; }
        }
        if (CORR) { m1 = ms_corr<T>(m1, c); m2 = ms_corr<T>(m2, c); }
        else { m1 = MsgStart<T>::of(m1); m2 = MsgStart<T>::of(m2); }
#pragma unroll
        for (int k = 0; k < D; ++k) {
            const float b = (k == idx) ? m2 : m1;
            const unsigned s = par ^ ((x[k][v] < 0.0f) ? 1u : 0u);
            out[k][v] = s ? -b : b;
        }
    }
}

__device__ __forceinline__ float bp_clamp(float x)
{
    const float a = fminf(__builtin_fabsf(x), 1000.0f);
    return (x < 0.0f) ? -a : a;
}
__device__ __forceinline__ float bp_corr(float x) { return fmaxf(__builtin_fmaf(-0.25f, x, 0.6931472f), 0.0f); }
__device__ __forceinline__ float bp_boxplus(float u, float v)
{
    const float au = __builtin_fabsf(u), av = __builtin_fabsf(v);
    const float m = fminf(au, av);
    const float s = au + av;
    const float d = __builtin_fabsf(au - av);
    const float g = fmaxf((m + bp_corr(s)) - bp_corr(d), 0.0f);
    return ((u < 0.0f) != (v < 0.0f)) ? -g : g;
}

template <int D, int W, typename T>
__device__ __forceinline__ void check_bp(const float (&x)[D][W], float (&out)[D][W])
{
#pragma unroll
    for (int w = 0; w < W; ++w) {
        float t[D];
#pragma unroll
        for (int j = 0; j < D; ++j) t[j] = bp_clamp(x[j][w]);
        if constexpr (D == 1) {
            out[0][w] = MsgRound<T>::of(1000.0f);
        } else if constexpr (D == 2) {
            out[0][w] = MsgRound<T>::of(t[1]);
            out[1][w] = MsgRound<T>::of(t[0]);
        } else {
            float b[D];
            b[D - 1] = t[D - 1];
#pragma unroll
            for (int j = D - 2; j >= 1; --j) b[j] = bp_boxplus(t[j], b[j + 1]);
            out[0][w] = MsgRound<T>::of(b[1]);
            float f = t[0];
#pragma unroll
            for (int k = 1; k <= D - 2; ++k) {
                out[k][w] = MsgRound<T>::of(bp_boxplus(f, b[k + 1]));
                f = bp_boxplus(f, t[k]);
            }
            out[D - 1][w] = MsgRound<T>::of(f);
        }
    }
}

template <int ALGO, int D, int W, typename T>
__device__ __forceinline__ void check_node(const float (&x)[D][W], float (&out)[D][W], const MsCorr &c)
{
    if (ALGO == kAlgoSP) check_sp<D, W>(x, out);
    else if (ALGO == kAlgoBP) check_bp<D, W, T>(x, out);
    else if (ALGO == kAlgoMS) check_ms<D, W, false, T>(x, out);
    else check_ms<D, W, true, T>(x, out, c);
}

template <int ALGO, int D, int V, int W, typename T>
__device__ __forceinline__ void check_rows(const T *Qu, unsigned lane_off, T *Rt, const int32_t *__restrict__ e0s, int r_begin, int r_end,
                                           const T *Ct, const int32_t *__restrict__ edge_col,
                                           const int32_t *__restrict__ qpos, const MsCorr &c)
{
    const int lane = threadIdx.x & 63;
    constexpr size_t F = 64 * V;
    for (int r = r_begin; r < r_end; ++r) {
        const int e0 = e0s[r];
        float x[D][W], out[D][W];
        if (ALGO != kAlgoSP && Ct) {
#pragma unroll
            for (int k = 0; k < D; ++k) vload<W>(x[k], Ct + (size_t)edge_col[e0 + k] * F);
        } else {
            int sl[D];
            row_slots<D>(qpos, e0, lane, sl);
#pragma unroll
            for (int k = 0; k < D; ++k) vload<W>(x[k], Qu + (size_t)sl[k] * F + lane_off);
        }
        check_node<ALGO, D, W, T>(x, out, c);
#pragma unroll
        for (int k = 0; k < D; ++k) vstore<W>(Rt + (size_t)(e0 + k) * F, out[k]);
    }
}

template <int ALGO, int D, int V, int W, typename T>
__global__ __launch_bounds__(kBlock) void check_kernel(const CheckArgs a)
{
    constexpr size_t F = 64 * V;
    constexpr int SUB = V / W;
    const int lane = threadIdx.x & 63;
    const GridPos gp = grid_pos(a.tiles_first);
    const int tile = tile_select<V>(a.tail, a.done, gp.row);
    if (tile < 0) return;
    const int wave = gp.block * kWavesPerBlock + wave_id_in_block();
    const int sub = wave % SUB;
    const int r_begin = (wave / SUB) * a.rows_per_wave;
    const int r_end = min(r_begin + a.rows_per_wave, a.n_rows);
    const unsigned lane_off = (unsigned)sub * 64 * W + (unsigned)lane * W;
    const T *Qu = static_cast<const T *>(a.Q) + (size_t)tile * (size_t)a.E * F;
    T *Rt = static_cast<T *>(a.R) + (size_t)tile * (size_t)a.E * F + lane_off;

    const T *Ct = (ALGO != kAlgoSP && a.first_chan)
                      ? static_cast<const T *>(a.first_chan) + (size_t)tile * (size_t)a.N * F + lane_off : nullptr;
    check_rows<ALGO, D, V, W, T>(Qu, lane_off, Rt, a.cls_e0, r_begin, r_end, Ct, a.edge_col, a.qpos, ms_corr_of(a));
}

template <int ALGO, int V, typename T>
__device__ __forceinline__ void check_row_generic(const T *Qu, unsigned lane_off, T *Rt, int e0, int D,
                                                  const int32_t *__restrict__ qpos, const MsCorr &c)
{
    constexpr size_t F = 64 * V;
    if (ALGO == kAlgoBP) {
        auto load = [&](int j, float (&t)[V]) {
            vload<V>(t, Qu + (size_t)edge_slot(qpos, e0 + j) * F + lane_off);
#pragma unroll
            for (int v = 0; v < V; ++v) t[v] = bp_clamp(t[v]);
        };
        auto store = [&](int k, float (&o)[V]) {
#pragma unroll
            for (int v = 0; v < V; ++v) o[v] = MsgRound<T>::of(o[v]);
            vstore<V>(Rt + (size_t)(e0 + k) * F, o);
        };
        if (D <= 0) return;
        float f[V], b[V], t[V];
        if (D == 1) {
#pragma unroll
            for (int v = 0; v < V; ++v) b[v] = 1000.0f;
            store(0, b);
            return;
        }
        load(0, f);
        for (int k = 0; k < D - 1; ++k) {
            load(D - 1, b);
            for (int j = D - 2; j > k; --j) {
                load(j, t);
#pragma unroll
                for (int v = 0; v < V; ++v) b[v] = bp_boxplus(t[v], b[v]);
            }
            if (k == 0) { store(0, b); continue; }
            float o[V];
#pragma unroll
            for (int v = 0; v < V; ++v) o[v] = bp_boxplus(f[v], b[v]);
            store(k, o);
            load(k, t);
#pragma unroll
            for (int v = 0; v < V; ++v) f[v] = bp_boxplus(f[v], t[v]);
        }
        store(D - 1, f);
        return;
    }
    if (ALGO != kAlgoSP) {
        float m1[V], m2[V];
        int idx[V];
        unsigned par[V];
#pragma unroll
        for (int v = 0; v < V; ++v) { m1[v] = 1000.0f; m2[v] = 1000.0f; idx[v] = -1; par[v] = 0; }
        for (int j = 0; j < D; ++j) {
            float xj[V];
            vload<V>(xj, Qu + (size_t)edge_slot(qpos, e0 + j) * F + lane_off);
#pragma unroll
            for (int v = 0; v < V; ++v) {
                const float m = __builtin_fabsf(xj[v]);
                par[v] ^= (xj[v] < 0.0f) ? 1u : 0u;
                if (m < m1[v]) { m2[v] = m1[v]; m1[v] = m; idx[v] = j; }
                else if (m < m2[v]) { m2[v] = m; }
            }
        }
        if (ALGO == kAlgoMSC) {
#pragma unroll
            for (int v = 0; v < V; ++v) { m1[v] = ms_corr<T>(m1[v], c); m2[v] = ms_corr<T>(m2[v], c); }
        } else {
#pragma unroll
            for (int v = 0; v < V; ++v) { m1[v] = MsgStart<T>::of(m1[v]); m2[v] = MsgStart<T>::of(m2[v]); }
        }
        for (int k = 0; k < D; ++k) {
            float xk[V], o[V];
            vload<V>(xk, Qu + (size_t)edge_slot(qpos, e0 + k) * F + lane_off);
#pragma unroll
            for (int v = 0; v < V; ++v) {
                const float b = (k == idx[v]) ? m2[v] : m1[v];
                const unsigned sg = par[v] ^ ((xk[v] < 0.0f) ? 1u : 0u);
                o[v] = sg ? -b : b;
            }
            vstore<V>(Rt + (size_t)(e0 + k) * F, o);
        }
        return;
    }
    for (int k = 0; k < D; ++k) {
        float o[V];
        float p[V];
#pragma unroll
        for (int v = 0; v < V; ++v) p[v] = 1.0f;
        for (int j = 0; j < D; ++j) {
            if (j == k) continue;
            float xj[V];
            vload<V>(xj, Qu + (size_t)edge_slot(qpos, e0 + j) * F + lane_off);
#pragma unroll
            for (int v = 0; v < V; ++v) p[v] *= xj[v];
        }
#pragma unroll
        for (int v = 0; v < V; ++v) o[v] = p[v];
        vstore<V>(Rt + (size_t)(e0 + k) * F, o);
    }
}

template <int ALGO, int V, typename T>
__global__ __launch_bounds__(kBlock) void check_kernel_generic(const CheckArgs a)
{
    constexpr size_t F = 64 * V;
    const int lane = threadIdx.x & 63;
    const GridPos gp = grid_pos(a.tiles_first);
    const int tile = tile_select<V>(a.tail, a.done, gp.row);
    if (tile < 0) return;
    const int wave = gp.block * kWavesPerBlock + wave_id_in_block();
    const int r_begin = wave * a.rows_per_wave;
    const int r_end = min(r_begin + a.rows_per_wave, a.n_rows);
    const T *Qu = static_cast<const T *>(a.Q) + (size_t)tile * (size_t)a.E * F;
    T *Rt = static_cast<T *>(a.R) + (size_t)tile * (size_t)a.E * F + (size_t)lane * V;
    for (int r = r_begin; r < r_end; ++r) check_row_generic<ALGO, V, T>(Qu, (unsigned)lane * V, Rt, a.cls_e0[r], a.degree, a.qpos, ms_corr_of(a));
}

template <int ALGO, int V, typename T, int D, int DLO, int W = 1> struct CheckDispatch {
    static __device__ __forceinline__ void run(int deg, const T *Qu, unsigned lane_off, T *Rt, const int32_t *e0s, int rb, int re,
                                               const T *Ct, const int32_t *edge_col, const int32_t *qpos, const MsCorr &c)
    {
        if (deg == D) check_rows<ALGO, D, V, W, T>(Qu, lane_off, Rt, e0s, rb, re, Ct, edge_col, qpos, c);
        else CheckDispatch<ALGO, V, T, D - 1, DLO, W>::run(deg, Qu, lane_off, Rt, e0s, rb, re, Ct, edge_col, qpos, c);
    }
};
template <int ALGO, int V, typename T, int DLO, int W> struct CheckDispatch<ALGO, V, T, DLO, DLO, W> {
    static __device__ __forceinline__ void run(int, const T *Qu, unsigned lane_off, T *Rt, const int32_t *e0s, int rb, int re,
                                               const T *Ct, const int32_t *edge_col, const int32_t *qpos, const MsCorr &c)
    {
        check_rows<ALGO, DLO, V, W, T>(Qu, lane_off, Rt, e0s, rb, re, Ct, edge_col, qpos, c);
    }
};

template <int ALGO, int V, typename T, int DLO, int DHI, int W = 1>
__global__ __launch_bounds__(kBlock) void check_group_kernel(const CheckArgs a, const GroupClass *__restrict__ cls, int n_classes)
{
    constexpr size_t F = 64 * V;
    constexpr int SUB = V / W;
    const int lane = threadIdx.x & 63;
    const GridPos gp = grid_pos(a.tiles_first);
    const int tile = tile_select<V>(a.tail, a.done, gp.row);
    if (tile < 0) return;
    int c = 0;
    while (c + 1 < n_classes && gp.block >= cls[c + 1].block_begin) ++c;
    const int wave = (gp.block - cls[c].block_begin) * kWavesPerBlock + wave_id_in_block();
    const int sub = wave % SUB;
    const int r_begin = (wave / SUB) * a.rows_per_wave;
    const int r_end = min(r_begin + a.rows_per_wave, cls[c].count);
    const unsigned lane_off = (unsigned)sub * 64 * W + (unsigned)lane * W;
    const T *Qu = static_cast<const T *>(a.Q) + (size_t)tile * (size_t)a.E * F;
    T *Rt = static_cast<T *>(a.R) + (size_t)tile * (size_t)a.E * F + lane_off;
    const T *Ct = (ALGO != kAlgoSP && a.first_chan)
                      ? static_cast<const T *>(a.first_chan) + (size_t)tile * (size_t)a.N * F + lane_off : nullptr;
    CheckDispatch<ALGO, V, T, DHI, DLO, W>::run(cls[c].degree, Qu, lane_off, Rt, cls[c].ids, r_begin, r_end, Ct, a.edge_col, a.qpos, ms_corr_of(a));
}

}
```

myldpccppapi_amd/csrc/flood_link.hpp:

```cpp
#pragma once

#include "flood_check.hpp"
#include "flood_var.hpp"

namespace ldpc {

struct LinkArgs {
    const int32_t *__restrict__ link_col;
    const int32_t *__restrict__ link_pos;
    const void *__restrict__ chan;
    void *Qw;
    uint64_t *hard;
    int32_t N;
    int32_t write_q;
    int32_t store_all;
    const int32_t *__restrict__ extra_e0;
    const int32_t *__restrict__ extra_deg;
    int32_t n_extra;
    int32_t link_blocks;
    int32_t n_big, small_rows;
};

__host__ __device__ inline void link_chunk_rows(int c, int rows_per_wave, int n_big, int small_rows, int n_rows,
                                               int *rb, int *re)
{
    int b, e;
    if (c < n_big) { b = c * rows_per_wave; e = b + rows_per_wave; }
    else { b = n_big * rows_per_wave + (c - n_big) * small_rows; e = b + small_rows; }
    *rb = b < n_rows ? b : n_rows;
    *re = e < n_rows ? e : n_rows;
}
__host__ __device__ inline int link_chunk_count(int rows_per_wave, int n_big, int small_rows, int n_rows)
{
    const int rest = n_rows - n_big * rows_per_wave;
    return n_big + (rest > 0 ? (rest + small_rows - 1) / small_rows : 0);
}

template <int ALGO, int V, typename T>
__device__ __forceinline__ void link_extra_rows(const CheckArgs &a, const LinkArgs &g, int tile, int block)
{
    constexpr size_t F = 64 * V;
    const int lane = threadIdx.x & 63;
    const int w = (block - g.link_blocks) * kWavesPerBlock + wave_id_in_block();
    if (w >= g.n_extra) return;
    const T *Qu = static_cast<const T *>(a.Q) + (size_t)tile * (size_t)a.E * F;
    T *Rt = static_cast<T *>(a.R) + (size_t)tile * (size_t)a.E * F + (size_t)lane * V;
    check_row_generic<ALGO, V, T>(Qu, (unsigned)lane * V, Rt, g.extra_e0[w], g.extra_deg[w], a.qpos, ms_corr_of(a));
}

#ifdef LDPC_LINK_WIDE_WAVES
#define LDPC_LINK_WIDE_ATTR __attribute__((amdgpu_waves_per_eu(LDPC_LINK_WIDE_WAVES, LDPC_LINK_WIDE_WAVES)))
#else
#define LDPC_LINK_WIDE_ATTR
#endif
template <int ALGO, int D, int V, typename T>
__global__ __launch_bounds__(kBlock) LDPC_LINK_WIDE_ATTR void check_link_kernel(const CheckArgs a, const LinkArgs g)
{
    constexpr size_t F = 64 * V;
    const int lane = threadIdx.x & 63;
    const GridPos gp = grid_pos(a.tiles_first);
    const int tile = tile_select<V>(a.tail, a.done, gp.row);
    if (tile < 0) return;
    if (gp.block >= g.link_blocks) { link_extra_rows<ALGO, V, T>(a, g, tile, gp.block); return; }
    const int wave = gp.block * kWavesPerBlock + wave_id_in_block();
    int r_begin, r_end;
    link_chunk_rows(wave, a.rows_per_wave, g.n_big, g.small_rows, a.n_rows, &r_begin, &r_end);
    const size_t lane_off = (size_t)lane * V;
    const unsigned lane_q = (unsigned)lane * V;
    const T *Qt = static_cast<const T *>(a.Q) + (size_t)tile * (size_t)a.E * F;
    T *Qwt = static_cast<T *>(g.Qw) + (size_t)tile * (size_t)a.E * F;
    T *Rt = static_cast<T *>(a.R) + (size_t)tile * (size_t)a.E * F + lane_off;
    const T *chan_t = static_cast<const T *>(g.chan) + (size_t)tile * (size_t)g.N * F + lane_off;
    uint64_t *hard_t = g.hard + (size_t)tile * (size_t)g.N * V;
    uint64_t frozen[V];
#pragma unroll
    for (int v = 0; v < V; ++v) frozen[v] = a.done[(size_t)tile * V + v];

    int pend_col = -1, pend_edge = 0, pend_kb = 0;
    float pend_r[V];
#pragma unroll
    for (int v = 0; v < V; ++v) pend_r[v] = 0.0f;

    float x[D][V];
    int qc[D], qn[D];
#pragma unroll
    for (int k = 0; k < D; ++k) qc[k] = qn[k] = 0;
    if (r_begin < r_end) {
        row_slots<D>(a.qpos, a.cls_e0[r_begin], lane, qc);
#pragma unroll
        for (int k = 0; k < D; ++k) vload<V>(x[k], Qt + (size_t)qc[k] * F + lane_q);
    }
    for (int r = r_begin; r < r_end; ++r) {
        const int e0 = a.cls_e0[r];
        const int next_col = (r + 1 < r_end) ? g.link_col[r] : -1;
        const int pos = g.link_pos[r];
        const int ka = next_col >= 0 ? (pos & 255) : -1;
        const int kb = pend_col >= 0 ? pend_kb : -1;
        if (r + 1 < r_end) row_slots<D>(a.qpos, a.cls_e0[r + 1], lane, qn);
        float ch[V];
        uint64_t old_w[V];
        if (pend_col >= 0) {
            vload<V>(ch, chan_t + (size_t)pend_col * F);
#pragma unroll
            for (int v = 0; v < V; ++v) old_w[v] = hard_t[(size_t)pend_col * V + v];
        }
        float out[D][V];
        check_node<ALGO, D, V, T>(x, out, ms_corr_of(a));
        if (r + 1 < r_end) {
#pragma unroll
            for (int k = 0; k < D; ++k) vload<V>(x[k], Qt + (size_t)qn[k] * F + lane_q);
        }
#pragma unroll
        for (int k = 0; k < D; ++k)
            if ((k != ka && k != kb) || g.store_all) vstore<V>(Rt + (size_t)(e0 + k) * F, out[k]);

        if (pend_col >= 0) {
            float rr[2][V], q[2][V];
#pragma unroll
            for (int v = 0; v < V; ++v) {
                rr[0][v] = pend_r[v];
                float t = out[0][v];
#pragma unroll
                for (int k = 1; k < D; ++k) t = (k == kb) ? out[k][v] : t;
                rr[1][v] = t;
            }
            uint64_t new_w[V];
            if (ALGO == kAlgoSP) {
                float f0[V], f1[V];
                var_sp<2, V>(ch, rr, q, f0, f1);
#pragma unroll
                for (int v = 0; v < V; ++v) {
                    const bool oldb = (old_w[v] >> lane) & 1ull;
                    const bool b = (f0[v] > f1[v]) ? false : ((f0[v] < f1[v]) ? true : oldb);
                    new_w[v] = __ballot(b);
                }
            } else {
#pragma unroll
                for (int v = 0; v < V; ++v) {
                    float p = ch[v];
                    p += rr[0][v];
                    p += rr[1][v];
                    q[0][v] = p - rr[0][v];
                    q[1][v] = p - rr[1][v];
                    new_w[v] = __ballot(!(p > 0.0f));
                }
            }
            if (lane == 0) {
#pragma unroll
                for (int v = 0; v < V; ++v)
                    hard_t[(size_t)pend_col * V + v] = (old_w[v] & frozen[v]) | (new_w[v] & ~frozen[v]);
            }
            if (g.write_q) {
                int qw1 = qc[0];
#pragma unroll
                for (int k = 1; k < D; ++k) qw1 = (k == kb) ? qc[k] : qw1;
                vstore<V>(Qwt + (size_t)pend_edge * F + lane_q, q[0]);
                vstore<V>(Qwt + (size_t)qw1 * F + lane_q, q[1]);
            }
        }
        pend_col = next_col;
        if (next_col >= 0) {
            pend_edge = qc[0];
#pragma unroll
            for (int k = 1; k < D; ++k) pend_edge = (k == ka) ? qc[k] : pend_edge;
            pend_kb = (pos >> 8) & 255;
#pragma unroll
            for (int v = 0; v < V; ++v) {
                float t = out[0][v];
#pragma unroll
                for (int k = 1; k < D; ++k) t = (k == ka) ? out[k][v] : t;
                pend_r[v] = t;
            }
        }
#pragma unroll
        for (int k = 0; k < D; ++k) qc[k] = qn[k];
    }
}

template <int ALGO, int D, int V, typename T, int W = 1>
__global__ __launch_bounds__(kBlock) void check_link_narrow_kernel(const CheckArgs a, const LinkArgs g)
{
    constexpr size_t F = 64 * V;
    constexpr int SUBS = V / W;
    constexpr int FB = 64 / SUBS;
    const int lane = threadIdx.x & 63;
    const GridPos gp = grid_pos(a.tiles_first);
    const int tile = tile_select<V>(a.tail, a.done, gp.row);
    if (tile < 0) return;
    if (gp.block >= g.link_blocks) { link_extra_rows<ALGO, V, T>(a, g, tile, gp.block); return; }
    const int wave = gp.block * kWavesPerBlock + wave_id_in_block();
    const int sub = wave % SUBS;
    int r_begin, r_end;
    link_chunk_rows(wave / SUBS, a.rows_per_wave, g.n_big, g.small_rows, a.n_rows, &r_begin, &r_end);
    const size_t lane_off = (size_t)sub * 64 * W + (size_t)lane * W;
    const unsigned lane_q = (unsigned)lane_off;
    const T *Qt = static_cast<const T *>(a.Q) + (size_t)tile * (size_t)a.E * F;
    T *Qwt = static_cast<T *>(g.Qw) + (size_t)tile * (size_t)a.E * F;
    T *Rt = static_cast<T *>(a.R) + (size_t)tile * (size_t)a.E * F + lane_off;
    const T *chan_t = static_cast<const T *>(g.chan) + (size_t)tile * (size_t)g.N * F + lane_off;
    uint8_t *hard_b = reinterpret_cast<uint8_t *>(g.hard + (size_t)tile * (size_t)g.N * V) + (size_t)sub * (FB / 8);
    const uint64_t frozen_field = (a.done[(size_t)tile * V + (lane < V ? lane : 0)] >> (sub * FB)) &
                                  (FB == 64 ? ~0ull : ((1ull << (FB & 63)) - 1ull));

    auto load_field = [&](int col, int word) -> uint64_t {
        const uint8_t *p = hard_b + ((size_t)col * V + word) * 8;
        if (FB == 64) return *reinterpret_cast<const uint64_t *>(p);
        if (FB == 32) return *reinterpret_cast<const uint32_t *>(p);
        return *reinterpret_cast<const uint16_t *>(p);
    };

    int pend_col = -1, pend_edge = 0, pend_kb = 0;
    float pend_r[W];
#pragma unroll
    for (int w = 0; w < W; ++w) pend_r[w] = 0.0f;
    float x[D][W];
    int qc[D], qn[D];
#pragma unroll
    for (int k = 0; k < D; ++k) qc[k] = qn[k] = 0;
    if (r_begin < r_end) {
        row_slots<D>(a.qpos, a.cls_e0[r_begin], lane, qc);
#pragma unroll
        for (int k = 0; k < D; ++k) vload<W>(x[k], Qt + (size_t)qc[k] * F + lane_q);
    }
    for (int r = r_begin; r < r_end; ++r) {
        const int e0 = a.cls_e0[r];
        const int next_col = (r + 1 < r_end) ? g.link_col[r] : -1;
        const int pos = g.link_pos[r];
        const int ka = next_col >= 0 ? (pos & 255) : -1;
        const int kb = pend_col >= 0 ? pend_kb : -1;
        if (r + 1 < r_end) row_slots<D>(a.qpos, a.cls_e0[r + 1], lane, qn);
        float ch[W];
        uint64_t old_mine[W];
#pragma unroll
        for (int w = 0; w < W; ++w) { ch[w] = 0.0f; old_mine[w] = 0; }
        if (pend_col >= 0) {
            vload<W>(ch, chan_t + (size_t)pend_col * F);
#pragma unroll
            for (int w = 0; w < W; ++w) old_mine[w] = load_field(pend_col, (W * lane + w) % V);
        }
        float out[D][W];
        check_node<ALGO, D, W, T>(x, out, ms_corr_of(a));
        if (r + 1 < r_end) {
#pragma unroll
            for (int k = 0; k < D; ++k) vload<W>(x[k], Qt + (size_t)qn[k] * F + lane_q);
        }
#pragma unroll
        for (int k = 0; k < D; ++k)
            if ((k != ka && k != kb) || g.store_all) vstore<W>(Rt + (size_t)(e0 + k) * F, out[k]);

        if (pend_col >= 0) {
            float rr[2][W], q[2][W];
#pragma unroll
            for (int w = 0; w < W; ++w) {
                rr[0][w] = pend_r[w];
                float t = out[0][w];
#pragma unroll
                for (int k = 1; k < D; ++k) t = (k == kb) ? out[k][w] : t;
                rr[1][w] = t;
            }
            uint64_t ballot[W];
            if (ALGO == kAlgoSP) {
                float f0[W], f1[W];
                var_sp<2, W>(ch, rr, q, f0, f1);
#pragma unroll
                for (int w = 0; w < W; ++w) {
                    const bool oldb = (old_mine[w] >> ((W * lane + w) / V)) & 1ull;
                    const bool bit = (f0[w] > f1[w]) ? false : ((f0[w] < f1[w]) ? true : oldb);
                    ballot[w] = __ballot(bit);
                }
            } else {
#pragma unroll
                for (int w = 0; w < W; ++w) {
                    float p = ch[w];
                    p += rr[0][w];
                    p += rr[1][w];
                    q[0][w] = p - rr[0][w];
                    q[1][w] = p - rr[1][w];
                    ballot[w] = __ballot(!(p > 0.0f));
                }
            }
            if (lane < V) {
                uint64_t bw = ballot[0];
#pragma unroll
                for (int w = 1; w < W; ++w) bw = (lane % W == w) ? ballot[w] : bw;
                const uint64_t nf = compress_stride<SUBS>(bw >> (lane / W));
                const uint64_t of = load_field(pend_col, lane);
                const uint64_t res = (of & frozen_field) | (nf & ~frozen_field);
                uint8_t *p = hard_b + ((size_t)pend_col * V + lane) * 8;
                if (FB == 64) *reinterpret_cast<uint64_t *>(p) = res;
                else if (FB == 32) *reinterpret_cast<uint32_t *>(p) = (uint32_t)res;
                else *reinterpret_cast<uint16_t *>(p) = (uint16_t)res;
            }
            if (g.write_q) {
                int qw1 = qc[0];
#pragma unroll
                for (int k = 1; k < D; ++k) qw1 = (k == kb) ? qc[k] : qw1;
                vstore<W>(Qwt + (size_t)pend_edge * F + lane_q, q[0]);
                vstore<W>(Qwt + (size_t)qw1 * F + lane_q, q[1]);
            }
        }
        pend_col = next_col;
        if (next_col >= 0) {
            pend_edge = qc[0];
#pragma unroll
            for (int k = 1; k < D; ++k) pend_edge = (k == ka) ? qc[k] : pend_edge;
            pend_kb = (pos >> 8) & 255;
#pragma unroll
            for (int w = 0; w < W; ++w) {
                float t = out[0][w];
#pragma unroll
                for (int k = 1; k < D; ++k) t = (k == ka) ? out[k][w] : t;
                pend_r[w] = t;
            }
        }
#pragma unroll
        for (int k = 0; k < D; ++k) qc[k] = qn[k];
    }
}

template <int ALGO, int D, int V, typename T>
__global__ __launch_bounds__(kBlock) void check_link_narrow2_kernel(const CheckArgs a, const LinkArgs g)
{
    constexpr size_t F = 64 * V;
    constexpr int FB = 64 / V;
    const int lane = threadIdx.x & 63;
    const GridPos gp = grid_pos(a.tiles_first);
    const int tile = tile_select<V>(a.tail, a.done, gp.row);
    if (tile < 0) return;
    if (gp.block >= g.link_blocks) { link_extra_rows<ALGO, V, T>(a, g, tile, gp.block); return; }
    const int wave = gp.block * kWavesPerBlock + wave_id_in_block();
    const int sub = wave % V;
    int r_begin, r_end;
    link_chunk_rows(wave / V, a.rows_per_wave, g.n_big, g.small_rows, a.n_rows, &r_begin, &r_end);
    const size_t lane_off = (size_t)sub * 64 + lane;
    const T *Qt = static_cast<const T *>(a.Q) + (size_t)tile * (size_t)a.E * F + lane_off;
    T *Qwt = static_cast<T *>(g.Qw) + (size_t)tile * (size_t)a.E * F + lane_off;
    T *Rt = static_cast<T *>(a.R) + (size_t)tile * (size_t)a.E * F + lane_off;
    const T *chan_t = static_cast<const T *>(g.chan) + (size_t)tile * (size_t)g.N * F + lane_off;
    const int my_word = lane % V, my_bit = lane / V;
    uint8_t *hard_b = reinterpret_cast<uint8_t *>(g.hard + (size_t)tile * (size_t)g.N * V) + (size_t)sub * (FB / 8);
    const uint64_t frozen_field = (a.done[(size_t)tile * V + (lane < V ? lane : 0)] >> (sub * FB)) &
                                  (FB == 64 ? ~0ull : ((1ull << FB) - 1ull));

    auto load_field = [&](int col, int word) -> uint64_t {
        const uint8_t *p = hard_b + ((size_t)col * V + word) * 8;
        if (V == 1) return *reinterpret_cast<const uint64_t *>(p);
        if (V == 2) return *reinterpret_cast<const uint32_t *>(p);
        return *reinterpret_cast<const uint16_t *>(p);
    };

    int pend_col = -1, pend_edge = 0, pend_kb = 0;
    float pend_r = 0.0f;
    float b0[D], b1[D], b2[D];
    auto load_row = [&](float (&dst)[D], int r) {
        const int e = a.cls_e0[r];
#pragma unroll
        for (int k = 0; k < D; ++k) { float t[1]; vload<1>(t, Qt + (size_t)edge_slot(a.qpos, e + k) * F); dst[k] = t[0]; }
    };
    if (r_begin < r_end) load_row(b0, r_begin);
    if (r_begin + 1 < r_end) load_row(b1, r_begin + 1);
    auto step = [&](int r, float (&x)[D], float (&pre)[D]) {
        const int e0 = a.cls_e0[r];
        const int next_col = (r + 1 < r_end) ? g.link_col[r] : -1;
        const int pos = g.link_pos[r];
        const int ka = next_col >= 0 ? (pos & 255) : -1;
        const int kb = pend_col >= 0 ? pend_kb : -1;
        float ch[1] = {0.0f};
        uint64_t old_mine = 0;
        if (pend_col >= 0) {
            vload<1>(ch, chan_t + (size_t)pend_col * F);
            old_mine = load_field(pend_col, my_word);
        }
        if (r + 2 < r_end) load_row(pre, r + 2);
        float xx[D][1], out[D][1];
#pragma unroll
        for (int k = 0; k < D; ++k) xx[k][0] = x[k];
        check_node<ALGO, D, 1, T>(xx, out, ms_corr_of(a));
#pragma unroll
        for (int k = 0; k < D; ++k)
            if ((k != ka && k != kb) || g.store_all) vstore<1>(Rt + (size_t)(e0 + k) * F, out[k]);

        if (pend_col >= 0) {
            float rr[2][1], q[2][1];
            rr[0][0] = pend_r;
            float t = out[0][0];
#pragma unroll
            for (int k = 1; k < D; ++k) t = (k == kb) ? out[k][0] : t;
            rr[1][0] = t;
            bool bit;
            if (ALGO == kAlgoSP) {
                float f0[1], f1[1];
                var_sp<2, 1>(ch, rr, q, f0, f1);
                const bool oldb = (old_mine >> my_bit) & 1ull;
                bit = (f0[0] > f1[0]) ? false : ((f0[0] < f1[0]) ? true : oldb);
            } else {
                float p = ch[0];
                p += rr[0][0];
                p += rr[1][0];
                q[0][0] = p - rr[0][0];
                q[1][0] = p - rr[1][0];
                bit = !(p > 0.0f);
            }
            const uint64_t ballot = __ballot(bit);
            if (lane < V) {
                const uint64_t nf = compress_stride<V>(ballot >> lane);
                const uint64_t of = load_field(pend_col, lane);
                const uint64_t res = (of & frozen_field) | (nf & ~frozen_field);
                uint8_t *p = hard_b + ((size_t)pend_col * V + lane) * 8;
                if (V == 1) *reinterpret_cast<uint64_t *>(p) = res;
                else if (V == 2) *reinterpret_cast<uint32_t *>(p) = (uint32_t)res;
                else *reinterpret_cast<uint16_t *>(p) = (uint16_t)res;
            }
            if (g.write_q) {
                vstore<1>(Qwt + (size_t)edge_slot(a.qpos, pend_edge) * F, q[0]);
                vstore<1>(Qwt + (size_t)edge_slot(a.qpos, e0 + kb) * F, q[1]);
            }
        }
        pend_col = next_col;
        if (next_col >= 0) {
            pend_edge = e0 + ka;
            pend_kb = (pos >> 8) & 255;
            float t = out[0][0];
#pragma unroll
            for (int k = 1; k < D; ++k) t = (k == ka) ? out[k][0] : t;
            pend_r = t;
        }
    };
    for (int r = r_begin; r < r_end; r += 3) {
        step(r, b0, b2);
        if (r + 1 < r_end) step(r + 1, b1, b0);
        if (r + 2 < r_end) step(r + 2, b2, b1);
    }
}

}
```

myldpccppapi_amd/csrc/flood_round.hpp:

```cpp
#pragma once

#include "flood_common.hpp"
#include "ldpc_expf.h"
#include "llr_input.hpp"

namespace ldpc {

struct InitArgs {
    const void *__restrict__ llr;
    void *__restrict__ chan;
    void *__restrict__ Q;
    uint64_t *__restrict__ hard;
    const int32_t *__restrict__ col_ptr;
    const int32_t *__restrict__ col_edge;
    int64_t E;
    int64_t frames;
    int32_t N;
    float llr_scale;
    float llr_unit;
};

constexpr int kInitCols = 32;

template <int ALGO, int V, typename T, typename IN = float>
__global__ __launch_bounds__(kBlock) void init_kernel(const InitArgs a)
{
    constexpr int F = 64 * V;
    constexpr int LD = F + 1;
    __shared__ float patch[kInitCols * LD];
    const int tile = blockIdx.y;
    const int n0 = blockIdx.x * kInitCols;
    const IN *__restrict__ llr = static_cast<const IN *>(a.llr);
    if constexpr (!std::is_same<IN, float>::value) {
        llr_patch_fill<IN, F, LD, kInitCols, kBlock, false>(patch, llr, a.llr_unit, a.frames, a.N, tile, n0, 1.0f);
    } else if ((a.N & 3) == 0 && n0 + kInitCols <= a.N && (reinterpret_cast<uintptr_t>(llr) & 15) == 0) {
        const int c4 = (threadIdx.x & 7) * 4, f0 = threadIdx.x >> 3;
        float4 vals[F / 32];
#pragma unroll
        for (int i = 0; i < F / 32; ++i) {
            const int64_t frame = (int64_t)tile * F + f0 + 32 * i;
            vals[i] = float4{1.0f, 1.0f, 1.0f, 1.0f};
            if (frame < a.frames) vals[i] = *reinterpret_cast<const float4 *>(llr + (size_t)frame * a.N + n0 + c4);
        }
#pragma unroll
        for (int i = 0; i < F / 32; ++i) {
            const int f = f0 + 32 * i;
            patch[(c4 + 0) * LD + f] = vals[i].x;
            patch[(c4 + 1) * LD + f] = vals[i].y;
            patch[(c4 + 2) * LD + f] = vals[i].z;
            patch[(c4 + 3) * LD + f] = vals[i].w;
        }
    } else {
        const int c = threadIdx.x & (kInitCols - 1);
        const int n = n0 + c;
        for (int f = threadIdx.x / kInitCols; f < F; f += kBlock / kInitCols) {
            const int64_t frame = (int64_t)tile * F + f;
            float y = 1.0f;
            if (frame < a.frames && n < a.N) y = llr[(size_t)frame * a.N + n];
            patch[c * LD + f] = y;
        }
    }
    __syncthreads();
    const int lane = threadIdx.x & 63;
    for (int c = threadIdx.x >> 6; c < kInitCols; c += kWavesPerBlock) {
        const int n = n0 + c;
        if (n >= a.N) break;
        float ch[V], q[V];
#pragma unroll
        for (int v = 0; v < V; ++v) {
            const float y = patch[c * LD + lane * V + v];
            if (ALGO == kAlgoSP) {
                const float t = ldpc_expf(a.llr_scale * y);
                ch[v] = t;
                q[v] = t / (1.0f + t) - 1.0f / (1.0f + t);
            } else if (ALGO == kAlgoBP) {
                float t = a.llr_scale * y;
                asm volatile("" : "+v"(t));
                ch[v] = q[v] = t;
            } else {
                const float c = MsgChan<T>::of(y, a.llr_scale);
                ch[v] = c;
                q[v] = c;
            }
        }
        vstore<V>(static_cast<T *>(a.chan) + ((size_t)tile * a.N + n) * F + (size_t)lane * V, ch);
        if (a.Q) {
            const int p0 = a.col_ptr[n], deg = a.col_ptr[n + 1] - p0;
            T *Qt = static_cast<T *>(a.Q) + (size_t)tile * (size_t)a.E * F + (size_t)lane * V;
            for (int k0 = 0; k0 < deg; k0 += 64) {
                const int m = min(64, deg - k0);
                const int mine = a.col_edge[p0 + k0 + (lane < m ? lane : m - 1)];
                for (int k = 0; k < m; ++k)
                    vstore<V>(Qt + (size_t)__builtin_amdgcn_readlane(mine, k) * F, q);
            }
        }
        if (lane < V) a.hard[((size_t)tile * a.N + n) * V + lane] = 0;
    }
}

struct SyndromeArgs {
    const int32_t *__restrict__ row_ptr;
    const int32_t *__restrict__ edge_col;
    const uint64_t *__restrict__ hard;
    uint64_t *__restrict__ fail;
    const uint64_t *__restrict__ done;
    int32_t M, N;
    int32_t tiles;
    int32_t row_blocks;
    TailRef tail;
};

template <int V> __global__ __launch_bounds__(kBlock) void syndrome_kernel(const SyndromeArgs a)
{
    int tile, rb;
    if (a.tiles > 0) {
        const int xcd = blockIdx.x & 7, j = blockIdx.x >> 3;
        tile = xcd + 8 * (j / a.row_blocks);
        rb = j % a.row_blocks;
        if (tile >= a.tiles) return;
    } else {
        tile = blockIdx.y;
        rb = blockIdx.x;
    }
    tile = tile_select<V>(a.tail, a.done, tile);
    if (tile < 0) return;
    const int m = rb * kBlock + threadIdx.x;
    const uint64_t *hard_t = a.hard + (size_t)tile * (size_t)a.N * V;
    uint64_t s[V];
#pragma unroll
    for (int v = 0; v < V; ++v) s[v] = 0;
    if (m < a.M) {
        for (int p = a.row_ptr[m]; p < a.row_ptr[m + 1]; ++p) {
            const int c = a.edge_col[p];
#pragma unroll
            for (int v = 0; v < V; ++v) s[v] ^= hard_t[(size_t)c * V + v];
        }
    }
    __shared__ uint64_t part[kWavesPerBlock][V];
#pragma unroll
    for (int v = 0; v < V; ++v) {
        uint64_t x = s[v];
#pragma unroll
        for (int off = 32; off >= 1; off >>= 1) {
            const uint32_t lo = __shfl_xor((uint32_t)x, off);
            const uint32_t hi = __shfl_xor((uint32_t)(x >> 32), off);
            x |= ((uint64_t)hi << 32) | lo;
        }
        if ((threadIdx.x & 63) == 0) part[threadIdx.x >> 6][v] = x;
    }
    __syncthreads();
    if (threadIdx.x < V) {
        uint64_t x = 0;
#pragma unroll
        for (int w = 0; w < kWavesPerBlock; ++w) x |= part[w][threadIdx.x];
        unsigned long long *dst = reinterpret_cast<unsigned long long *>(&a.fail[(size_t)tile * V + threadIdx.x]);
        const uint64_t seen = __hip_atomic_load(dst, __ATOMIC_RELAXED, __HIP_MEMORY_SCOPE_AGENT);
        if (x & ~seen) atomicOr(dst, (unsigned long long)x);
    }
}

struct StateArgs {
    uint64_t *__restrict__ done;
    const uint64_t *__restrict__ fail;
    int32_t *__restrict__ iters;
    int32_t *__restrict__ active;
    int64_t frames;
    int32_t iter;
    int32_t max_iter;
    int32_t freeze;
    TailRef tail;
    int32_t *__restrict__ running;
    int32_t *__restrict__ tile_rounds;
};

template <int V> __global__ void state_kernel(const StateArgs a)
{
    constexpr int F = 64 * V;
    int tile = blockIdx.x;
    if (a.tail.state && a.iter > 0 && a.tail.state[0]) {
        if (tile >= a.tail.n_tiles) return;
        tile = a.tail.base_tile + tile;
    }
    const int lane = threadIdx.x;
    int n_active = 0;
    bool worked = false;
#pragma unroll
    for (int v = 0; v < V; ++v) {
        const int64_t frame = (int64_t)tile * F + (int64_t)lane * V + v;
        const bool valid = frame < a.frames;
        uint64_t d;
        if (a.iter == 0) {
            d = __ballot(!valid);
            a.iters[(size_t)tile * F + lane * V + v] = a.max_iter;
        } else {
            const uint64_t old = a.done[(size_t)tile * V + v];
            worked = worked || old != ~0ull;
            const uint64_t clean = ~a.fail[(size_t)tile * V + v];
            const uint64_t newly = clean & ~old;
            if ((newly >> lane) & 1ull) a.iters[(size_t)tile * F + lane * V + v] = a.iter;
            d = a.freeze ? (old | clean) : old;
        }
        if (lane == 0) a.done[(size_t)tile * V + v] = d;
        n_active += __popcll(~d);
    }
    if (lane == 0 && n_active && a.active) atomicAdd(a.active, n_active);
    if (lane == 0 && n_active && a.running) atomicAdd(&a.running[a.iter], n_active);
    if (lane == 0 && worked && a.tile_rounds) atomicAdd(a.tile_rounds, 1);
}

struct PackArgs {
    const uint64_t *__restrict__ hard;
    uint8_t *__restrict__ out;
    const int32_t *__restrict__ iters_tile;
    int32_t *__restrict__ iters_out;
    int64_t frames;
    int64_t out_bytes;
    int32_t N, K;
    int32_t pack_mode;
};

template <int V> inline dim3 pack_grid(int32_t K, int tiles)
{
    const int chunks = K / 8 > 0 ? (K / 8 + 63) / 64 : 1;
    return dim3((unsigned)((chunks * V + kWavesPerBlock - 1) / kWavesPerBlock), (unsigned)tiles);
}

template <int V> __global__ __launch_bounds__(kBlock) void pack_kernel(const PackArgs a)
{
    constexpr int F = 64 * V;
    if (a.pack_mode == 0) {
        const int tile = blockIdx.y;
        const int kb = a.K / 8;
        if (blockIdx.x == 0 && a.iters_out) {
            for (int f = threadIdx.x; f < F; f += kBlock) {
                const int64_t frame = (int64_t)tile * F + f;
                if (frame < a.frames) a.iters_out[frame] = a.iters_tile[frame];
            }
        }
        if (!a.out) return;
        const int unit = (int)blockIdx.x * kWavesPerBlock + wave_id_in_block();
        const int v = unit % V;
// ... 36 lines not shown
```

myldpccppapi_amd/csrc/flood_tables.hpp:

```cpp
#pragma once

#include "flood_kernels.hpp"

namespace ldpc {

using CheckFn = void (*)(const CheckArgs);
using VarFn = void (*)(const VarArgs);
using LinkFn = void (*)(const CheckArgs, const LinkArgs);
using CheckGroupFn = void (*)(const CheckArgs, const GroupClass *, int);
using VarGroupFn = void (*)(const VarArgs, const GroupClass *, int);
using InitFn = void (*)(const InitArgs);

constexpr int kVarBuckets = 3, kCheckBuckets = 4;
constexpr int kVarBucketLo[kVarBuckets] = {1, 5, 9}, kVarBucketHi[kVarBuckets] = {4, 8, 16};
constexpr int kCheckBucketLo[kCheckBuckets] = {1, 9, 17, 25}, kCheckBucketHi[kCheckBuckets] = {8, 16, 24, 32};

struct FloodFns {
    CheckFn check[kMaxUnrolledCheckDegreeMS + 1] = {};
    CheckFn check_wide[kMaxUnrolledCheckDegreeMS + 1] = {};
    LinkFn link[kMaxUnrolledDegree + 1] = {};
    LinkFn link_narrow[kMaxUnrolledDegree + 1] = {};
    LinkFn link_deep[kMaxUnrolledDegree + 1] = {};
    LinkFn link_half[kMaxUnrolledDegree + 1] = {};
    VarFn var[kMaxUnrolledDegree + 1] = {};
    CheckGroupFn check_group[kCheckBuckets] = {};
    int check_group_width = 1;
    VarGroupFn var_group[kVarBuckets] = {};
    InitFn init = nullptr;
    InitFn init_in[3] = {};
    int max_check_unrolled = kMaxUnrolledDegree;
};

void fill_flood_sp(int V, FloodFns *f);
void fill_flood_ms(int V, FloodFns *f);
void fill_flood_ms16(int V, FloodFns *f);
void fill_flood_msc(int V, FloodFns *f);
void fill_flood_msc16(int V, FloodFns *f);
void fill_flood_ms8(int V, FloodFns *f);
void fill_flood_msc8(int V, FloodFns *f);
void fill_flood_msi4(int V, FloodFns *f);
void fill_flood_msci4(int V, FloodFns *f);
void fill_flood_msi5(int V, FloodFns *f);
void fill_flood_msci5(int V, FloodFns *f);
void fill_flood_msi6(int V, FloodFns *f);
void fill_flood_msci6(int V, FloodFns *f);
void fill_flood_msi8(int V, FloodFns *f);
void fill_flood_msci8(int V, FloodFns *f);
void fill_flood_bp(int V, FloodFns *f);
void fill_flood_bp16(int V, FloodFns *f);

}
```

myldpccppapi_amd/csrc/flood_tables_impl.hpp:

```cpp
#pragma once

#include "flood_tables.hpp"

namespace ldpc {
namespace tables {

template <int ALGO, int V, typename T, int D> struct FloodTable {
    static void fill(CheckFn *c, CheckFn *cw, VarFn *v)
    {
        c[D] = check_kernel<ALGO, D, V, 1, T>;
        cw[D] = check_kernel<ALGO, D, V, V, T>;
        v[D] = var_kernel<ALGO, D, V, T>;
        FloodTable<ALGO, V, T, D - 1>::fill(c, cw, v);
    }
};
template <int ALGO, int V, typename T> struct FloodTable<ALGO, V, T, 0> {
    static void fill(CheckFn *c, CheckFn *cw, VarFn *v)
    {
        c[0] = cw[0] = check_kernel_generic<ALGO, V, T>;
        v[0] = var_kernel_generic<ALGO, V, T>;
    }
};

template <int ALGO, int V, typename T, int D> struct CheckTableMS {
    static void fill(CheckFn *c, CheckFn *cw)
    {
        c[D] = cw[D] = check_kernel<ALGO, D, V, 1, T>;
        CheckTableMS<ALGO, V, T, D - 1>::fill(c, cw);
    }
};
template <int ALGO, int V, typename T> struct CheckTableMS<ALGO, V, T, kMaxUnrolledDegree> {
    static void fill(CheckFn *, CheckFn *) {}
};

template <int ALGO, int V, typename T, int D> struct LinkHalf {
    static LinkFn get() { return nullptr; }
};
template <int ALGO, typename T, int D> struct LinkHalf<ALGO, 4, T, D> {
    static LinkFn get() { return check_link_narrow_kernel<ALGO, D, 4, T, 2>; }
};
template <int ALGO, int V, typename T, int D> struct LinkTable {
    static void fill(LinkFn *t, LinkFn *tn, LinkFn *td, LinkFn *th)
    {
        t[D] = check_link_kernel<ALGO, D, V, T>;
        tn[D] = check_link_narrow_kernel<ALGO, D, V, T>;
        td[D] = check_link_narrow2_kernel<ALGO, D, V, T>;
        th[D] = LinkHalf<ALGO, V, T, D>::get();
        LinkTable<ALGO, V, T, D - 1>::fill(t, tn, td, th);
    }
};
template <int ALGO, int V, typename T> struct LinkTable<ALGO, V, T, 1> {
    static void fill(LinkFn *, LinkFn *, LinkFn *, LinkFn *) {}
};

template <int ALGO, int V, typename T> void fill_v(FloodFns *f)
{
    constexpr int DM = kMaxUnrolledDegree;
    FloodTable<ALGO, V, T, DM>::fill(f->check, f->check_wide, f->var);
    LinkTable<ALGO, V, T, DM>::fill(f->link, f->link_narrow, f->link_deep, f->link_half);
    constexpr int GW = sizeof(T) == 1 ? V : (sizeof(T) == 2 && V == 4) ? 2 : 1;
    f->check_group_width = GW;
    f->check_group[0] = check_group_kernel<ALGO, V, T, 1, 8, GW>;
    f->check_group[1] = check_group_kernel<ALGO, V, T, 9, 16, GW>;
    f->check_group[2] = f->check_group[3] = nullptr;
    f->var_group[0] = var_group_kernel<ALGO, V, T, 1, 4>;
    f->var_group[1] = var_group_kernel<ALGO, V, T, 5, 8>;
    f->var_group[2] = var_group_kernel<ALGO, V, T, 9, 16>;
    f->init = f->init_in[kLlrF32] = init_kernel<ALGO, V, T>;
    f->init_in[kLlrF16] = init_kernel<ALGO, V, T, _Float16>;
    f->init_in[kLlrI8] = init_kernel<ALGO, V, T, int8_t>;
    f->max_check_unrolled = DM;
    if (ALGO != kAlgoSP) {
        CheckTableMS<ALGO, V, T, kMaxUnrolledCheckDegreeMS>::fill(f->check, f->check_wide);
        f->check_group[2] = check_group_kernel<ALGO, V, T, 17, 24, GW>;
        f->check_group[3] = check_group_kernel<ALGO, V, T, 25, 32, GW>;
        f->max_check_unrolled = kMaxUnrolledCheckDegreeMS;
    }
}

template <int ALGO, typename T> void fill(int V, FloodFns *f)
{
    *f = FloodFns();
    if (V == 1) fill_v<ALGO, 1, T>(f);
    else if (V == 2) fill_v<ALGO, 2, T>(f);
    else fill_v<ALGO, 4, T>(f);
}

}
}
```

myldpccppapi_amd/csrc/introspect.hip:

```cpp
#include <hip/hip_runtime.h>

#include <algorithm>
#include <cstdio>
#include <cstring>
#include <vector>

#include "decoder.hpp"

using ldpc::set_error;

extern "C" {

int ldpc_decoder_set_timing(ldpc_decoder *d, int enable)
{
    if (!d) return set_error(LDPC_ERR_ARG, "decoder is NULL");
    if (!d->shards.empty()) {
        for (ldpc_decoder *sh : d->shards) {
            const int rc = ldpc_decoder_set_timing(sh, enable);
            if (rc) return rc;
        }
        return LDPC_OK;
    }
    if (d->tm.have_last) {
        LDPC_HIP_TRY(hipSetDevice(d->cfg.device));
// ... 114 lines not shown
    static const char *algo_name_corr_f16[] = {"sp16", "msc16", "layered16", "ms_fused16", "layered_host16", "bp16", "layered_bp16"};
    static const char *algo_name_f8[] = {"sp8", "ms8", "layered8", "ms_fused8", "layered_host8", "bp8", "layered_bp8"};
    static const char *algo_name_corr_f8[] = {"sp8", "msc8", "layered8", "ms_fused8", "layered_host8", "bp8", "layered_bp8"};
    const int msz = d->flood.msg_size;
    char name_i8[8];
    snprintf(name_i8, sizeof name_i8, "%s%d", d->ms_corr ? "msci" : "msi", d->flood.msg_bits);
    const char *algo_name_i8[] = {"sp", name_i8, "layered", "ms_fused", "layered_host", "bp", "layered_bp"};
    const char **algo_name = d->flood.msg_kind == LDPC_MSG_I8 ? algo_name_i8
                             : d->ms_corr ? (msz == 1 ? algo_name_corr_f8 : msz == 2 ? algo_name_corr_f16 : algo_name_corr_f32)
                                          : (msz == 1 ? algo_name_f8 : msz == 2 ? algo_name_f16 : algo_name_f32);
    for (size_t i = 0; i < d->tm.spans_used; ++i) {
        const ldpc::TimedSpan &sp = d->tm.spans[i];
        float ms = 0;
        LDPC_HIP_TRY(hipEventElapsedTime(&ms, sp.a.e, sp.b.e));
        const int phase = (sp.kind == 4 || sp.kind == 5) ? 0 : (sp.kind == 6 ? 1 : ((sp.kind == 7 || sp.kind == 8) ? 3 : sp.kind));
        char name[64];
        if (sp.kind == 3) snprintf(name, sizeof name, "other");
        else if (sp.kind == 7) snprintf(name, sizeof name, "soft_settle_kernel");
        else if (sp.kind == 8) snprintf(name, sizeof name, "llr_widen_kernel");
        else if (d->use_fused && d->use_ldsp)
            snprintf(name, sizeof name, "%s[%dx%d,%d]", d->cfg.algo == LDPC_ALGO_LAYERED
                     ? (d->ms_corr ? "layered_ldsp_corr_kernel" : "layered_ldsp_kernel")
                     : (d->ms_corr ? "flood_ldsp_corr_kernel" : "flood_ldsp_kernel"),
                     d->ldsp.grid, d->ldsp.block, d->ldsp.wg_frames);
        else if (d->use_fused)
            snprintf(name, sizeof name, "%s", d->cfg.algo == LDPC_ALGO_SP ? "fused_sp_kernel"
                     : d->cfg.algo == LDPC_ALGO_LAYERED ? "fused_layered_kernel" : "fused_flood_kernel");
        else if (d->cfg.algo == LDPC_ALGO_LAYERED_FX)
            snprintf(name, sizeof name, "layer_kernel<lfx,%d,%d>", sp.degree, d->V);
        else if (sp.kind == 5 || sp.kind == 6)
            snprintf(name, sizeof name, "%s<%s,%d-%d,%d>", sp.kind == 5 ? "check_group_kernel" : "var_group_kernel",
                     algo_name[d->cfg.algo], sp.lo, sp.degree, d->V);
        else snprintf(name, sizeof name, "%s<%s,%d,%d>", phase_name[sp.kind], algo_name[d->cfg.algo], sp.degree, d->V);
        int k = 0;
        for (; k < *count; ++k)
            if (!strcmp(out[k].name, name)) break;
        if (k == *count) {
            if (*count == capacity) continue;
            ++*count;
            memset(&out[k], 0, sizeof out[k]);
            out[k].phase = phase;
            out[k].degree = sp.degree;
            memcpy(out[k].name, name, sizeof name);
        }
        ++out[k].launches;
        out[k].ms_total += ms;
        out[k].bytes_total += sp.bytes;
        out[k].bytes_moved += sp.moved;
    }
    return LDPC_OK;
}

int ldpc_decoder_link_form(ldpc_decoder *d, int32_t *form, int32_t *calibrated, float ms[3])
{
    if (!d) return set_error(LDPC_ERR_ARG, "decoder is NULL");
    if (!d->shards.empty()) return ldpc_decoder_link_form(d->shards[0], form, calibrated, ms);
    bool linked = false;
    for (auto &rc : d->flood.row_classes) linked = linked || rc.linked;
    if (form) *form = linked ? d->flood.link_form : -1;
    if (calibrated) *calibrated = d->flood.link_calibrated ? 1 : 0;
    if (ms) for (int k = 0; k < 3; ++k) ms[k] = d->flood.link_calibrated && d->flood.link_cal_ms[k] < 1e29f ? d->flood.link_cal_ms[k] : 0.0f;
    return LDPC_OK;
}

int ldpc_decoder_placement(ldpc_decoder *d, int32_t *candidates, int32_t *kept, float ms[16])
{
    if (!d) return set_error(LDPC_ERR_ARG, "decoder is NULL");
    if (!d->shards.empty()) return ldpc_decoder_placement(d->shards[0], candidates, kept, ms);
    if (candidates) *candidates = d->flood.place_candidates;
    if (kept) *kept = d->flood.place_kept;
    if (ms) for (int k = 0; k < 16; ++k) ms[k] = k < d->flood.place_candidates ? d->flood.place_ms[k] : 0.0f;
    return LDPC_OK;
}

int ldpc_decoder_array_addresses(ldpc_decoder *d, uint64_t out[4])
{
    if (!d || !out) return set_error(LDPC_ERR_ARG, "decoder/out is NULL");
    if (!d->shards.empty()) return ldpc_decoder_array_addresses(d->shards[0], out);
    out[0] = (uint64_t)(uintptr_t)d->flood.Q.p; out[1] = (uint64_t)(uintptr_t)d->flood.R.p;
    out[2] = (uint64_t)(uintptr_t)d->flood.chan.p; out[3] = (uint64_t)(uintptr_t)d->hard.p;
    return LDPC_OK;
}

int ldpc_decoder_set_tap(ldpc_decoder *d, int32_t iter)
{
    if (!d) return set_error(LDPC_ERR_ARG, "decoder is NULL");
    if (iter < 0) return set_error(LDPC_ERR_ARG, "iter < 0");
    if (!d->shards.empty()) return set_error(LDPC_ERR_STATE, "debug taps need a single-device handle");
    d->tm.tap_iter = iter;
    return LDPC_OK;
}

static float e4m3_widen(uint8_t b)
{
    const uint32_t sign = (uint32_t)(b & 0x80) << 24, e = (b >> 3) & 15, m = b & 7;
    uint32_t bits;
    if (e == 15 && m == 7) bits = 0x7fc00000u;
    else if (e == 0) {
        const float sub = (float)m * 0.001953125f;
        memcpy(&bits, &sub, 4);
    } else bits = ((e + 120) << 23) | (m << 20);
    bits |= sign;
    float out;
    memcpy(&out, &bits, 4);
    return out;
}

int ldpc_decoder_dump(ldpc_decoder *d, int32_t which, float *host_out, int64_t count)
{
    if (!d || !host_out) return set_error(LDPC_ERR_ARG, "decoder/host_out is NULL");
    if (!d->shards.empty()) return set_error(LDPC_ERR_STATE, "debug taps need a single-device handle");
    if (!d->tm.have_last) return set_error(LDPC_ERR_STATE, "no decode call to dump");
    LDPC_HIP_TRY(hipSetDevice(d->cfg.device));
    d->wait_for_own_work();
    const int64_t frames = d->last_frames;
    const int V = d->V, F = d->F;
    const int tiles = (int)((frames + F - 1) / F);
    if (d->use_fused && d->cfg.algo == LDPC_ALGO_SP) {
        if (!d->fused.dump_p.p) return set_error(LDPC_ERR_STATE, "fused dump needs set_tap() before the decode");
        const int64_t per = (which == 0 || which == 1) ? d->E : d->N;
        if (which < 0 || which > 3 || count != frames * per) return set_error(LDPC_ERR_ARG, "bad `which`/count");
        if (which == 3) {
            std::vector<uint8_t> b((size_t)count);
            LDPC_HIP_TRY(hipMemcpy(b.data(), d->fused.dump_b.p, (size_t)count, hipMemcpyDeviceToHost));
            for (int64_t i = 0; i < count; ++i) host_out[i] = (float)b[i];
            return LDPC_OK;
        }
        const float *src = which == 0 ? d->fused.dump_r.p : (which == 1 ? d->fused.dump_q.p : d->fused.dump_p.p);
        LDPC_HIP_TRY(hipMemcpy(host_out, src, (size_t)count * sizeof(float), hipMemcpyDeviceToHost));
        return LDPC_OK;
    }
    if (d->use_fused) {
        const float *dump_r = d->use_ldsp ? d->ldsp.dump_r.p : d->fused.dump_r.p;
        const float *dump_p = d->use_ldsp ? d->ldsp.dump_p.p : d->fused.dump_p.p;
        const float *src = which == 0 ? dump_r : (which == 2 ? dump_p : nullptr);
        const int64_t per = which == 0 ? d->E : d->N;
        if (which == 3) {
            if (!dump_p || count != frames * d->N) return set_error(LDPC_ERR_ARG, "fused dump needs set_tap() and count = frames*N");
            LDPC_HIP_TRY(hipMemcpy(host_out, dump_p, (size_t)count * sizeof(float), hipMemcpyDeviceToHost));
            const bool notpos = d->cfg.algo == LDPC_ALGO_MS;
            for (int64_t i = 0; i < count; ++i)
                host_out[i] = (notpos ? !(host_out[i] > 0.0f) : (host_out[i] < 0.0f)) ? 1.0f : 0.0f;
            return LDPC_OK;
        }
        if (!src || count != frames * per) return set_error(LDPC_ERR_ARG, "fused dump: set_tap() first; which in {0,2,3}");
        LDPC_HIP_TRY(hipMemcpy(host_out, src, (size_t)count * sizeof(float), hipMemcpyDeviceToHost));
        return LDPC_OK;
    }
    if (d->cfg.algo == LDPC_ALGO_LAYERED || d->cfg.algo == LDPC_ALGO_LAYERED_HOST || d->cfg.algo == LDPC_ALGO_LAYERED_BP ||
        d->cfg.algo == LDPC_ALGO_LAYERED_FX) {
        hipError_t e = ldpc::layered_dump(&d->layered, which, host_out, count, frames, d->hard.p,
                                          d->h_cols.data());
        if (e == hipErrorInvalidValue) return set_error(LDPC_ERR_ARG, "bad `which`/count for layered dump");
        if (e != hipSuccess) return set_error(LDPC_ERR_HIP, "layered dump: %s", hipGetErrorString(e));
        return LDPC_OK;
    }
    if (which == 0 || which == 1 || which == 2) {
        const int64_t per = (which == 2) ? d->N : d->E;
        if (count != frames * per) return set_error(LDPC_ERR_ARG, "count must be frames*%lld", (long long)per);
        const uint8_t *src = which == 0 ? d->flood.R.p : (which == 1 ? d->flood.Q.p : d->flood.chan.p);
        const size_t esz = (size_t)d->flood.msg_size;
        std::vector<uint8_t> tile((size_t)per * F * esz);
        for (int t = 0; t < tiles; ++t) {
            LDPC_HIP_TRY(hipMemcpy(tile.data(), src + (size_t)t * per * F * esz, tile.size(), hipMemcpyDeviceToHost));
            for (int fi = 0; fi < F; ++fi) {
                const int64_t f = (int64_t)t * F + fi;
// ... 37 lines not shown
```

myldpccppapi_amd/csrc/tune.hpp:

```cpp
#pragma once

#include "../../include/ldpc_hip.h"

namespace ldpc {

struct Tune {
    int fused = 0, ldsp = 0, ldsp_ext = 0, ldsp_pack = 0, link_narrow = 0, check_wide = 0, syn_xcd = 0,
        fused_pack = 0, fused_loop = 0, device_tail = 0, merge = 0, link_deep = 0, link_half = 0, link_guided = 0, tiles_first = 0;
    int rows_per_wave = 0, cols_per_wave = 0;
    int link_rows = 0;
    int compact = 0;
    int ldsp_grid = 0, ldsp_per_cu = 0, ldsp_waves = 0;
    int place = 0;
    int q_order = 0;
};

inline Tune tune_from_config(const ldpc_decoder_config &c)
{
    Tune t;
    auto f = [&](int field) { return (c.tune_flags >> field) & 3; };
    t.fused = f(LDPC_TUNE_FUSED);
    t.ldsp = f(LDPC_TUNE_LDSP);
    t.ldsp_ext = f(LDPC_TUNE_LDSP_EXT);
    t.ldsp_pack = f(LDPC_TUNE_LDSP_PACK);
    t.link_narrow = f(LDPC_TUNE_LINK_NARROW);
    t.check_wide = f(LDPC_TUNE_CHECK_WIDE);
    t.syn_xcd = f(LDPC_TUNE_SYN_XCD);
    t.fused_pack = f(LDPC_TUNE_FUSED_PACK);
    t.fused_loop = f(LDPC_TUNE_FUSED_LOOP);
    t.device_tail = f(LDPC_TUNE_DEVICE_TAIL);
    t.merge = f(LDPC_TUNE_MERGE);
    t.link_deep = f(LDPC_TUNE_LINK_DEEP);
    t.link_half = f(LDPC_TUNE_LINK_HALF);
    t.link_guided = f(LDPC_TUNE_LINK_GUIDED);
    t.tiles_first = f(LDPC_TUNE_TILES_FIRST);
    t.rows_per_wave = c.tune_rows_per_wave;
    t.cols_per_wave = c.tune_cols_per_wave;
    t.link_rows = c.tune_link_rows;
    t.compact = c.tune_compact;
    t.ldsp_grid = c.tune_ldsp_grid;
    t.ldsp_per_cu = c.tune_ldsp_shape & 255;
    t.ldsp_waves = (c.tune_ldsp_shape >> 8) & 255;
    t.place = c.tune_place;
    t.q_order = c.tune_q_order;
    return t;
}

inline bool tune_pick(int tri, bool dflt) { return tri == 1 ? true : (tri == 2 ? false : dflt); }
inline bool tune_forced_on(int tri) { return tri == 1; }
inline bool tune_forced_off(int tri) { return tri == 2; }

inline bool tune_valid(const ldpc_decoder_config &c)
{
    for (int field = 0; field <= LDPC_TUNE_TILES_FIRST; field += 2)
        if (((c.tune_flags >> field) & 3) == 3) return false;
    if (c.tune_flags >> (LDPC_TUNE_TILES_FIRST + 2)) return false;
    return c.tune_rows_per_wave >= 0 && c.tune_rows_per_wave <= 4096 && c.tune_cols_per_wave >= 0 &&
           c.tune_cols_per_wave <= 4096 && c.tune_link_rows >= -1 && c.tune_link_rows <= 4096 &&
           c.tune_compact >= -1 && c.tune_ldsp_grid >= 0 && c.tune_ldsp_shape >= 0 && c.tune_ldsp_shape < 65536 &&
           c.tune_place >= 0 && c.tune_place <= 8 && c.host_input >= 0 && c.host_input <= 2 && c.host_copy_threads >= 0 && c.host_copy_threads <= 16 &&
           c.tune_q_order >= -1 && c.tune_q_order <= 1;
}

}
```

Before: 1128 Mbit/s.

## Read channel LLRs directly in first SP round and add class-ordered syndrome kernel

Extends the first-round-from-channel path, which skips writing the initial Q messages, to sum-product decoding. In that round, check kernels read channel values and convert them to the probability-domain message inline. Also adds a syndrome kernel that walks rows grouped by row class through a small device table. Both are on by default and can be turned off through a new handle-level tuning call. The aim is to remove the initial E-sized Q write and first-round Q read, at the cost of many more kernel instantiations.

```diff
diff --git a/include/ldpc_hip.h b/include/ldpc_hip.h
--- a/include/ldpc_hip.h
+++ b/include/ldpc_hip.h
@@ -181,6 +181,8 @@
 int ldpc_decoder_placement(ldpc_decoder *d, int32_t *candidates, int32_t *kept, float ms[16]);
 int ldpc_decoder_array_addresses(ldpc_decoder *d, uint64_t out[4]);
 
+int ldpc_decoder_set_round_tuning(ldpc_decoder *d, int32_t tune_first_chan, int32_t tune_syn_class);
+
 int ldpc_decoder_set_tap(ldpc_decoder *d, int32_t iter);
 int ldpc_decoder_dump(ldpc_decoder *d, int32_t which, float *host_out, int64_t count);
 
diff --git a/myldpccppapi_amd/_lib.py b/myldpccppapi_amd/_lib.py
--- a/myldpccppapi_amd/_lib.py
+++ b/myldpccppapi_amd/_lib.py
@@ -85,6 +85,7 @@
     "ldpc_decoder_set_timing", "ldpc_decoder_stats", "ldpc_decoder_kernel_times", "ldpc_decoder_set_tap",
     "ldpc_decoder_dump", "ldpc_awgn_device", "ldpc_count_errors_device", "ldpc_hbm_probe_device", "ldpc_hbm_sustained_device",
     "ldpc_host_block_plan", "ldpc_host_locked_ranges", "ldpc_decoder_link_form", "ldpc_decoder_placement", "ldpc_decoder_array_addresses",
+    "ldpc_decoder_set_round_tuning",
     "ldpc_parity_structure", "ldpc_encoder_create", "ldpc_encoder_destroy", "ldpc_encode_device", "ldpc_encode", "ldpc_code_bytes",
     "ldpc_rate_spec_init", "ldpc_rate_lengths", "ldpc_rate_index", "ldpc_rate_match_device", "ldpc_rate_recover_device",
     "ldpc_rate_match", "ldpc_rate_recover",
@@ -161,6 +162,7 @@
                                        ctypes.POINTER(ctypes.c_uint64)]
     L.ldpc_host_locked_ranges.argtypes = [i64p, i64p]
     L.ldpc_decoder_array_addresses.argtypes = [vp, ctypes.POINTER(ctypes.c_uint64)]
+    L.ldpc_decoder_set_round_tuning.argtypes = [vp, ctypes.c_int32, ctypes.c_int32]
     L.ldpc_decoder_placement.argtypes = [vp, i32p, i32p, ctypes.POINTER(ctypes.c_float)]
     L.ldpc_decoder_link_form.argtypes = [vp, i32p, i32p, ctypes.POINTER(ctypes.c_float)]
     L.ldpc_parity_structure.argtypes = [vp, ctypes.c_int32, ctypes.c_int32, i32p]
diff --git a/myldpccppapi_amd/capi.py b/myldpccppapi_amd/capi.py
--- a/myldpccppapi_amd/capi.py
+++ b/myldpccppapi_amd/capi.py
@@ -25,6 +25,7 @@
                "syn_xcd": 12, "fused_pack": 14, "fused_loop": 16, "device_tail": 18, "merge": 20, "link_deep": 22, "link_half": 24,
                "link_guided": 26, "tiles_first": 28}
 TUNE_INTS = ("rows_per_wave", "cols_per_wave", "link_rows", "compact", "ldsp_grid", "ldsp_per_cu", "ldsp_waves", "place", "q_order")
+TUNE_HANDLE = ("first_chan", "syn_class")
 
 
 def apply_tune(cfg, tune):
@@ -39,6 +40,8 @@
             shape |= (int(v) & 255) << 8
         elif k in TUNE_INTS:
             setattr(cfg, "tune_" + k, int(v))
+        elif k in TUNE_HANDLE:
+            pass
         else:
             raise KeyError("unknown tuning field %r" % k)
     cfg.tune_flags, cfg.tune_ldsp_shape = flags, shape
@@ -210,6 +213,9 @@
             devs = (ctypes.c_int32 * len(devices))(*[int(x) for x in devices])
             _lib.check(L.ldpc_decoder_create_multi(graph._h, ctypes.byref(cfg), devs, len(devices),
                                                    ctypes.byref(self._h)))
+        handle_tune = [{None: 0, True: 1, False: 2}[(tune or {}).get(k)] for k in TUNE_HANDLE]
+        if any(handle_tune):
+            _lib.check(L.ldpc_decoder_set_round_tuning(self._h, *handle_tune))
 
     def decode(self, llr, want_iters=True, soft=None, llr_unit=None):
         L = _lib.load()
diff --git a/myldpccppapi_amd/csrc/decoder.hpp b/myldpccppapi_amd/csrc/decoder.hpp
--- a/myldpccppapi_amd/csrc/decoder.hpp
+++ b/myldpccppapi_amd/csrc/decoder.hpp
@@ -77,6 +77,8 @@
     DevBuf<int32_t> extra_e0, extra_deg;
     int n_extra = 0;
     int64_t extra_edges = 0;
+    DevBuf<SynClass> syn_table;
+    int syn_classes = 0, syn_blocks = 0;
     FloodFns fns;
 
     int link_form = 1;
diff --git a/myldpccppapi_amd/csrc/engine_flood.hip b/myldpccppapi_amd/csrc/engine_flood.hip
--- a/myldpccppapi_amd/csrc/engine_flood.hip
+++ b/myldpccppapi_amd/csrc/engine_flood.hip
@@ -66,6 +66,18 @@
                                   uint8_t *out_dev, int64_t out_bytes, int32_t *iters_dev,
                                   hipStream_t s, int start_round = 1);
 
+static const ldpc::LinkFn *link_table(const ldpc_decoder *d, int variant, bool first)
+{
+    const ldpc::FloodFns &f = d->flood.fns;
+    if (variant == 2) return first ? f.link_half_first : f.link_half;
+    if (variant == 1) return d->flood.link_deep ? (first ? f.link_deep_first : f.link_deep) : (first ? f.link_narrow_first : f.link_narrow);
+    return first ? f.link_first : f.link;
+}
+static int link_variant(const ldpc_decoder *d, int degree)
+{
+    return (d->flood.link_form == 2 && !d->flood.fns.link_half[degree]) ? 1 : d->flood.link_form;
+}
+
 template <int V> int enqueue_check_phase(ldpc_decoder *d, hipStream_t s, int tiles, int64_t frames, int it, int max_iter,
                                          bool fat, const ldpc::TailRef &tr)
 {
@@ -79,17 +91,16 @@
                            msz * ((int64_t)rc.degree * rc.count + rc.linked +
                                   ((int64_t)rc.degree * rc.count - 2 * rc.linked) +
                                   (it < max_iter ? 2 * rc.linked : 0) + 2 * d->flood.extra_edges) * frames));
-        CheckArgs a = check_args(d, tr, d->flood.link_rpw, false, rc.e0.p, rc.count, rc.degree);
+        CheckArgs a = check_args(d, tr, d->flood.link_rpw, from_chan, rc.e0.p, rc.count, rc.degree);
         const bool soft_reads = d->soft.dst && (d->cfg.early_term || it == max_iter);
         LinkArgs lk{rc.link_col.p, rc.link_pos.p, d->flood.chan.p, d->flood.Q.p, d->hard.p, d->N,
                     (it < max_iter) ? 1 : 0, (d->tm.tap_iter || soft_reads) ? 1 : 0, d->flood.extra_e0.p, d->flood.extra_deg.p, d->flood.n_extra, 0,
                     rc.n_big, rc.small_rows};
-        const int variant = (d->flood.link_form == 2 && !d->flood.fns.link_half[rc.degree]) ? 1 : d->flood.link_form;
+        const int variant = link_variant(d, rc.degree);
         const int waves = link_chunk_count(d->flood.link_rpw, rc.n_big, rc.small_rows, rc.count) * (variant == 1 ? V : variant == 2 ? V / 2 : 1);
         lk.link_blocks = (waves + kWavesPerBlock - 1) / kWavesPerBlock;
         const dim3 grid = flood_grid(d, lk.link_blocks + (d->flood.n_extra + kWavesPerBlock - 1) / kWavesPerBlock, tiles, &a.tiles_first, true);
-        (variant == 2 ? d->flood.fns.link_half : variant == 1 ? (d->flood.link_deep ? d->flood.fns.link_deep : d->flood.fns.link_narrow) : d->flood.fns.link)
-            [rc.degree]<<<grid, kBlock, 0, s>>>(a, lk);
+        link_table(d, variant, from_chan)[rc.degree]<<<grid, kBlock, 0, s>>>(a, lk);
         LDPC_HIP_TRY(span_end(d, s));
     }
     for (auto &g : d->flood.check_groups) {
@@ -98,7 +109,7 @@
         LDPC_HIP_TRY(span_begin(d, s, 5, g.hi, 2 * msz * edges * frames, -1, g.lo));
         CheckArgs a = check_args(d, tr, (d->tune.rows_per_wave ? d->tune.rows_per_wave : 2) * (fat ? kIdleFat : 1), from_chan);
         const dim3 grid = flood_grid(d, fat ? g.blocks_fat : g.blocks, tiles, &a.tiles_first);
-        d->flood.fns.check_group[g.bucket]<<<grid, kBlock, 0, s>>>(a, fat ? g.table_fat.p : g.table.p, (int)g.members.size());
+        (from_chan ? d->flood.fns.check_group_first : d->flood.fns.check_group)[g.bucket]<<<grid, kBlock, 0, s>>>(a, fat ? g.table_fat.p : g.table.p, (int)g.members.size());
         LDPC_HIP_TRY(span_end(d, s));
     }
     for (int ci : d->flood.check_solo) {
@@ -110,7 +121,7 @@
         CheckArgs a = check_args(d, tr, rpw, from_chan, rc.e0.p, rc.count, rc.degree);
         const int waves = ((rc.count + rpw - 1) / rpw) * (narrow ? V : 1);
         const dim3 grid = flood_grid(d, (waves + kWavesPerBlock - 1) / kWavesPerBlock, tiles, &a.tiles_first);
-        (narrow ? d->flood.fns.check : d->flood.fns.check_wide)[slotk]<<<grid, kBlock, 0, s>>>(a);
+        (narrow ? (from_chan ? d->flood.fns.check_first : d->flood.fns.check) : (from_chan ? d->flood.fns.check_wide_first : d->flood.fns.check_wide))[slotk]<<<grid, kBlock, 0, s>>>(a);
         LDPC_HIP_TRY(span_end(d, s));
     }
     return LDPC_OK;
@@ -257,12 +268,16 @@
                       d->E, frames, d->N, tiles, d->T, d->flood.TO * F, std::min(d->flood.compact_threshold, d->flood.TO * F), 0, max_iter};
     }
 
-    bool q_less = (d->cfg.algo == LDPC_ALGO_MS || d->cfg.algo == LDPC_ALGO_BP) && !resume && !d->tm.tap_iter && max_iter > 1 && d->flood.n_extra == 0;
-    for (auto &rc : d->flood.row_classes) if (rc.linked) q_less = false;
-    for (int ci : d->flood.check_solo) if (d->flood.row_classes[ci].degree > d->flood.fns.max_check_unrolled) q_less = false;
+    bool q_less = tune_pick(d->tune.first_chan, true) && !resume && !d->tm.tap_iter && max_iter > 1;
+    for (auto &rc : d->flood.row_classes) if (rc.linked && !link_table(d, link_variant(d, rc.degree), true)[rc.degree]) q_less = false;
+    for (auto &g : d->flood.check_groups) if (!d->flood.fns.check_group_first[g.bucket]) q_less = false;
+    for (int ci : d->flood.check_solo) {
+        const int deg = d->flood.row_classes[ci].degree;
+        if (deg > d->flood.fns.max_check_unrolled || !d->flood.fns.check_first[deg] || !d->flood.fns.check_wide_first[deg]) q_less = false;
+    }
     d->flood.first_round_from_chan = q_less;
     if (!resume) {
-        LDPC_HIP_TRY(span_begin(d, s, 3));
+        LDPC_HIP_TRY(span_begin(d, s, 3, 0, ((int64_t)llr_elem_size(llr.type) * d->N + msz * (d->N + (q_less ? 0 : d->E))) * frames));
         InitArgs a{llr.p, d->flood.chan.p, q_less ? nullptr : d->flood.Q.p, d->hard.p, d->col_ptr.p, d->flood.col_qedge.p,
                    d->E, frames, d->N, d->cfg.llr_scale, llr.unit};
         dim3 grid((d->N + kInitCols - 1) / kInitCols, tiles);
@@ -288,11 +303,13 @@
         if (freeze || it == rounds) {
             LDPC_HIP_TRY(span_begin(d, s, 3));
             uint64_t *fw = d->failw.p + (size_t)it * slot;
-            const int rbk = (d->M + kBlock - 1) / kBlock;
+            const bool by_class = tune_pick(d->tune.syn_class, true) && d->flood.syn_classes > 0;
+            const int rbk = by_class ? d->flood.syn_blocks : (d->M + kBlock - 1) / kBlock;
             SyndromeArgs sa{d->row_ptr.p, d->edge_col.p, d->hard.p, fw, d->done.p, d->M, d->N,
                             d->flood.syn_xcd ? tiles : 0, rbk, tr};
             dim3 sgrid = d->flood.syn_xcd ? dim3(8 * rbk * ((tiles + 7) / 8)) : dim3(rbk, tiles);
-            syndrome_kernel<V><<<sgrid, kBlock, 0, s>>>(sa);
+            if (by_class) syndrome_class_kernel<V><<<sgrid, kBlock, 0, s>>>(sa, d->flood.syn_table.p, d->flood.syn_classes);
+            else syndrome_kernel<V><<<sgrid, kBlock, 0, s>>>(sa);
             if (d->cfg.crc_kind) {
                 CrcTermArgs ca{d->hard.p, fw, d->done.p, d->crc_w.p, d->summary.p + 3, d->N, d->cfg.crc_bits, tr};
                 crc_term_kernel<V><<<dim3((unsigned)tiles, V), 64 * crc_term_waves(d->cfg.crc_bits), 0, s>>>(ca);
@@ -503,6 +520,14 @@
         for (int k = 0; k < kVarBuckets; ++k)
             if (cc.degree >= kVarBucketLo[k] && cc.degree <= kVarBucketHi[k] && d->flood.fns.var_group[k]) b = k;
         if (merge && b >= 0) vb[b].push_back(i); else d->flood.var_solo.push_back(i);
+    }
+    {
+        std::vector<ldpc::SynRows> all;
+        for (const RowClass &rc : d->flood.row_classes) all.push_back(ldpc::SynRows{rc.degree, rc.count, rc.e0.p});
+        std::vector<ldpc::SynClass> syn;
+        d->flood.syn_blocks = ldpc::syn_class_table(all, ldpc::kBlock, &syn);
+        d->flood.syn_classes = (int)syn.size();
+        if (!syn.empty()) LDPC_HIP_TRY(d->flood.syn_table.upload(syn));
     }
     const int rpw = d->tune.rows_per_wave ? d->tune.rows_per_wave : 2, cpw = d->tune.cols_per_wave ? d->tune.cols_per_wave : 1;
     auto make = [&](std::vector<ClassGroup> &groups, std::vector<int> &solo, const std::vector<int> &members, int bucket,
@@ -629,6 +654,7 @@
     float best = 1e30f;
     hipError_t err = hipSuccess;
     int rc = LDPC_OK;
+    d->flood.first_round_from_chan = false;
     for (int rep = 0; rep < 4 && err == hipSuccess && rc == LDPC_OK; ++rep) {
         err = hipEventRecord(ev[0].e, s);
         rc = enqueue_check_phase<V>(d, s, d->T, (int64_t)d->T * d->F, 1, d->cfg.max_iter, false, ldpc::TailRef{nullptr, 0, 0});
diff --git a/myldpccppapi_amd/csrc/flood_check.hpp b/myldpccppapi_amd/csrc/flood_check.hpp
--- a/myldpccppapi_amd/csrc/flood_check.hpp
+++ b/myldpccppapi_amd/csrc/flood_check.hpp
@@ -109,7 +109,18 @@
     else check_ms<D, W, true, T>(x, out, c);
 }
 
-template <int ALGO, int D, int V, int W, typename T>
+template <int ALGO, int W> __device__ __forceinline__ void first_q(float (&x)[W])
+{
+    if (ALGO == kAlgoSP) {
+#pragma unroll
+        for (int w = 0; w < W; ++w) {
+            const float t = x[w];
+            x[w] = t / (1.0f + t) - 1.0f / (1.0f + t);
+        }
+    }
+}
+
+template <int ALGO, int D, int V, int W, typename T, bool FIRST = false>
 __device__ __forceinline__ void check_rows(const T *Qu, unsigned lane_off, T *Rt, const int32_t *__restrict__ e0s, int r_begin, int r_end,
                                            const T *Ct, const int32_t *__restrict__ edge_col,
                                            const int32_t *__restrict__ qpos, const MsCorr &c)
@@ -119,9 +130,13 @@
     for (int r = r_begin; r < r_end; ++r) {
         const int e0 = e0s[r];
         float x[D][W], out[D][W];
-        if (ALGO != kAlgoSP && Ct) {
+        if ((FIRST || ALGO != kAlgoSP) && Ct) {
 #pragma unroll
             for (int k = 0; k < D; ++k) vload<W>(x[k], Ct + (size_t)edge_col[e0 + k] * F);
+            if constexpr (ALGO == kAlgoSP) {
+#pragma unroll
+                for (int k = 0; k < D; ++k) first_q<ALGO, W>(x[k]);
+            }
         } else {
             int sl[D];
             row_slots<D>(qpos, e0, lane, sl);
@@ -134,7 +149,7 @@
     }
 }
 
-template <int ALGO, int D, int V, int W, typename T>
+template <int ALGO, int D, int V, int W, typename T, bool FIRST = false>
 __global__ __launch_bounds__(kBlock) void check_kernel(const CheckArgs a)
 {
     constexpr size_t F = 64 * V;
@@ -151,12 +166,12 @@
     const T *Qu = static_cast<const T *>(a.Q) + (size_t)tile * (size_t)a.E * F;
     T *Rt = static_cast<T *>(a.R) + (size_t)tile * (size_t)a.E * F + lane_off;
 
-    const T *Ct = (ALGO != kAlgoSP && a.first_chan)
+    const T *Ct = ((FIRST || ALGO != kAlgoSP) && a.first_chan)
                       ? static_cast<const T *>(a.first_chan) + (size_t)tile * (size_t)a.N * F + lane_off : nullptr;
-    check_rows<ALGO, D, V, W, T>(Qu, lane_off, Rt, a.cls_e0, r_begin, r_end, Ct, a.edge_col, a.qpos, ms_corr_of(a));
-}
-
-template <int ALGO, int V, typename T>
+    check_rows<ALGO, D, V, W, T, FIRST>(Qu, lane_off, Rt, a.cls_e0, r_begin, r_end, Ct, a.edge_col, a.qpos, ms_corr_of(a));
+}
+
+template <int ALGO, int V, typename T, bool FIRST = false>
 __device__ __forceinline__ void check_row_generic(const T *Qu, unsigned lane_off, T *Rt, int e0, int D,
                                                   const int32_t *__restrict__ qpos, const MsCorr &c)
 {
@@ -246,6 +261,7 @@
             if (j == k) continue;
             float xj[V];
             vload<V>(xj, Qu + (size_t)edge_slot(qpos, e0 + j) * F + lane_off);
+            if constexpr (FIRST) first_q<ALGO, V>(xj);
 #pragma unroll
             for (int v = 0; v < V; ++v) p[v] *= xj[v];
         }
@@ -271,23 +287,23 @@
     for (int r = r_begin; r < r_end; ++r) check_row_generic<ALGO, V, T>(Qu, (unsigned)lane * V, Rt, a.cls_e0[r], a.degree, a.qpos, ms_corr_of(a));
 }
 
-template <int ALGO, int V, typename T, int D, int DLO, int W = 1> struct CheckDispatch {
+template <int ALGO, int V, typename T, int D, int DLO, int W = 1, bool FIRST = false> struct CheckDispatch {
     static __device__ __forceinline__ void run(int deg, const T *Qu, unsigned lane_off, T *Rt, const int32_t *e0s, int rb, int re,
                                                const T *Ct, const int32_t *edge_col, const int32_t *qpos, const MsCorr &c)
     {
-        if (deg == D) check_rows<ALGO, D, V, W, T>(Qu, lane_off, Rt, e0s, rb, re, Ct, edge_col, qpos, c);
-        else CheckDispatch<ALGO, V, T, D - 1, DLO, W>::run(deg, Qu, lane_off, Rt, e0s, rb, re, Ct, edge_col, qpos, c);
+        if (deg == D) check_rows<ALGO, D, V, W, T, FIRST>(Qu, lane_off, Rt, e0s, rb, re, Ct, edge_col, qpos, c);
+        else CheckDispatch<ALGO, V, T, D - 1, DLO, W, FIRST>::run(deg, Qu, lane_off, Rt, e0s, rb, re, Ct, edge_col, qpos, c);
     }
 };
-template <int ALGO, int V, typename T, int DLO, int W> struct CheckDispatch<ALGO, V, T, DLO, DLO, W> {
+template <int ALGO, int V, typename T, int DLO, int W, bool FIRST> struct CheckDispatch<ALGO, V, T, DLO, DLO, W, FIRST> {
     static __device__ __forceinline__ void run(int, const T *Qu, unsigned lane_off, T *Rt, const int32_t *e0s, int rb, int re,
                                                const T *Ct, const int32_t *edge_col, const int32_t *qpos, const MsCorr &c)
     {
-        check_rows<ALGO, DLO, V, W, T>(Qu, lane_off, Rt, e0s, rb, re, Ct, edge_col, qpos, c);
+        check_rows<ALGO, DLO, V, W, T, FIRST>(Qu, lane_off, Rt, e0s, rb, re, Ct, edge_col, qpos, c);
     }
 };
 
-template <int ALGO, int V, typename T, int DLO, int DHI, int W = 1>
+template <int ALGO, int V, typename T, int DLO, int DHI, int W = 1, bool FIRST = false>
 __global__ __launch_bounds__(kBlock) void check_group_kernel(const CheckArgs a, const GroupClass *__restrict__ cls, int n_classes)
 {
     constexpr size_t F = 64 * V;
@@ -305,9 +321,9 @@
     const unsigned lane_off = (unsigned)sub * 64 * W + (unsigned)lane * W;
     const T *Qu = static_cast<const T *>(a.Q) + (size_t)tile * (size_t)a.E * F;
     T *Rt = static_cast<T *>(a.R) + (size_t)tile * (size_t)a.E * F + lane_off;
-    const T *Ct = (ALGO != kAlgoSP && a.first_chan)
+    const T *Ct = ((FIRST || ALGO != kAlgoSP) && a.first_chan)
                       ? static_cast<const T *>(a.first_chan) + (size_t)tile * (size_t)a.N * F + lane_off : nullptr;
-    CheckDispatch<ALGO, V, T, DHI, DLO, W>::run(cls[c].degree, Qu, lane_off, Rt, cls[c].ids, r_begin, r_end, Ct, a.edge_col, a.qpos, ms_corr_of(a));
-}
-
-}
+    CheckDispatch<ALGO, V, T, DHI, DLO, W, FIRST>::run(cls[c].degree, Qu, lane_off, Rt, cls[c].ids, r_begin, r_end, Ct, a.edge_col, a.qpos, ms_corr_of(a));
+}
+
+}
diff --git a/myldpccppapi_amd/csrc/flood_link.hpp b/myldpccppapi_amd/csrc/flood_link.hpp
--- a/myldpccppapi_amd/csrc/flood_link.hpp
+++ b/myldpccppapi_amd/csrc/flood_link.hpp
@@ -36,24 +36,30 @@
     return n_big + (rest > 0 ? (rest + small_rows - 1) / small_rows : 0);
 }
 
-template <int ALGO, int V, typename T>
+template <int ALGO, int V, typename T, bool FIRST = false>
 __device__ __forceinline__ void link_extra_rows(const CheckArgs &a, const LinkArgs &g, int tile, int block)
 {
     constexpr size_t F = 64 * V;
     const int lane = threadIdx.x & 63;
     const int w = (block - g.link_blocks) * kWavesPerBlock + wave_id_in_block();
     if (w >= g.n_extra) return;
-    const T *Qu = static_cast<const T *>(a.Q) + (size_t)tile * (size_t)a.E * F;
     T *Rt = static_cast<T *>(a.R) + (size_t)tile * (size_t)a.E * F + (size_t)lane * V;
-    check_row_generic<ALGO, V, T>(Qu, (unsigned)lane * V, Rt, g.extra_e0[w], g.extra_deg[w], a.qpos, ms_corr_of(a));
-}
+    if constexpr (FIRST) {
+        const T *Cu = static_cast<const T *>(g.chan) + (size_t)tile * (size_t)g.N * F;
+        check_row_generic<ALGO, V, T, true>(Cu, (unsigned)lane * V, Rt, g.extra_e0[w], g.extra_deg[w], a.edge_col, ms_corr_of(a));
+    } else {
+        const T *Qu = static_cast<const T *>(a.Q) + (size_t)tile * (size_t)a.E * F;
+        check_row_generic<ALGO, V, T>(Qu, (unsigned)lane * V, Rt, g.extra_e0[w], g.extra_deg[w], a.qpos, ms_corr_of(a));
+    }
+}
+
 
 #ifdef LDPC_LINK_WIDE_WAVES
 #define LDPC_LINK_WIDE_ATTR __attribute__((amdgpu_waves_per_eu(LDPC_LINK_WIDE_WAVES, LDPC_LINK_WIDE_WAVES)))
 #else
 #define LDPC_LINK_WIDE_ATTR
 #endif
-template <int ALGO, int D, int V, typename T>
+template <int ALGO, int D, int V, typename T, bool FIRST = false>
 __global__ __launch_bounds__(kBlock) LDPC_LINK_WIDE_ATTR void check_link_kernel(const CheckArgs a, const LinkArgs g)
 {
     constexpr size_t F = 64 * V;
@@ -61,7 +67,7 @@
     const GridPos gp = grid_pos(a.tiles_first);
     const int tile = tile_select<V>(a.tail, a.done, gp.row);
     if (tile < 0) return;
-    if (gp.block >= g.link_blocks) { link_extra_rows<ALGO, V, T>(a, g, tile, gp.block); return; }
+    if (gp.block >= g.link_blocks) { link_extra_rows<ALGO, V, T, FIRST>(a, g, tile, gp.block); return; }
     const int wave = gp.block * kWavesPerBlock + wave_id_in_block();
     int r_begin, r_end;
     link_chunk_rows(wave, a.rows_per_wave, g.n_big, g.small_rows, a.n_rows, &r_begin, &r_end);
@@ -87,8 +93,15 @@
     for (int k = 0; k < D; ++k) qc[k] = qn[k] = 0;
     if (r_begin < r_end) {
         row_slots<D>(a.qpos, a.cls_e0[r_begin], lane, qc);
-#pragma unroll
-        for (int k = 0; k < D; ++k) vload<V>(x[k], Qt + (size_t)qc[k] * F + lane_q);
+        if constexpr (FIRST) {
+            int cc[D];
+            row_slots<D>(a.edge_col, a.cls_e0[r_begin], lane, cc);
+#pragma unroll
+            for (int k = 0; k < D; ++k) vload<V>(x[k], chan_t + (size_t)cc[k] * F);
+        } else {
+#pragma unroll
+            for (int k = 0; k < D; ++k) vload<V>(x[k], Qt + (size_t)qc[k] * F + lane_q);
+        }
     }
     for (int r = r_begin; r < r_end; ++r) {
         const int e0 = a.cls_e0[r];
@@ -105,10 +118,21 @@
             for (int v = 0; v < V; ++v) old_w[v] = hard_t[(size_t)pend_col * V + v];
         }
         float out[D][V];
+        if constexpr (FIRST) {
+#pragma unroll
+            for (int k = 0; k < D; ++k) first_q<ALGO, V>(x[k]);
+        }
         check_node<ALGO, D, V, T>(x, out, ms_corr_of(a));
         if (r + 1 < r_end) {
-#pragma unroll
-            for (int k = 0; k < D; ++k) vload<V>(x[k], Qt + (size_t)qn[k] * F + lane_q);
+            if constexpr (FIRST) {
+                int cn[D];
+                row_slots<D>(a.edge_col, a.cls_e0[r + 1], lane, cn);
+#pragma unroll
+                for (int k = 0; k < D; ++k) vload<V>(x[k], chan_t + (size_t)cn[k] * F);
+            } else {
+#pragma unroll
+                for (int k = 0; k < D; ++k) vload<V>(x[k], Qt + (size_t)qn[k] * F + lane_q);
+            }
         }
 #pragma unroll
         for (int k = 0; k < D; ++k)
@@ -177,7 +201,7 @@
     }
 }
 
-template <int ALGO, int D, int V, typename T, int W = 1>
+template <int ALGO, int D, int V, typename T, int W = 1, bool FIRST = false>
 __global__ __launch_bounds__(kBlock) void check_link_narrow_kernel(const CheckArgs a, const LinkArgs g)
 {
     constexpr size_t F = 64 * V;
@@ -187,7 +211,7 @@
     const GridPos gp = grid_pos(a.tiles_first);
     const int tile = tile_select<V>(a.tail, a.done, gp.row);
     if (tile < 0) return;
-    if (gp.block >= g.link_blocks) { link_extra_rows<ALGO, V, T>(a, g, tile, gp.block); return; }
+    if (gp.block >= g.link_blocks) { link_extra_rows<ALGO, V, T, FIRST>(a, g, tile, gp.block); return; }
     const int wave = gp.block * kWavesPerBlock + wave_id_in_block();
     const int sub = wave % SUBS;
     int r_begin, r_end;
@@ -219,8 +243,15 @@
     for (int k = 0; k < D; ++k) qc[k] = qn[k] = 0;
     if (r_begin < r_end) {
         row_slots<D>(a.qpos, a.cls_e0[r_begin], lane, qc);
-#pragma unroll
-        for (int k = 0; k < D; ++k) vload<W>(x[k], Qt + (size_t)qc[k] * F + lane_q);
+        if constexpr (FIRST) {
+            int cc[D];
+            row_slots<D>(a.edge_col, a.cls_e0[r_begin], lane, cc);
+#pragma unroll
+            for (int k = 0; k < D; ++k) vload<W>(x[k], chan_t + (size_t)cc[k] * F);
+        } else {
+#pragma unroll
+            for (int k = 0; k < D; ++k) vload<W>(x[k], Qt + (size_t)qc[k] * F + lane_q);
+        }
     }
     for (int r = r_begin; r < r_end; ++r) {
         const int e0 = a.cls_e0[r];
@@ -239,10 +270,21 @@
             for (int w = 0; w < W; ++w) old_mine[w] = load_field(pend_col, (W * lane + w) % V);
         }
         float out[D][W];
+        if constexpr (FIRST) {
+#pragma unroll
+            for (int k = 0; k < D; ++k) first_q<ALGO, W>(x[k]);
+        }
         check_node<ALGO, D, W, T>(x, out, ms_corr_of(a));
         if (r + 1 < r_end) {
-#pragma unroll
-            for (int k = 0; k < D; ++k) vload<W>(x[k], Qt + (size_t)qn[k] * F + lane_q);
+            if constexpr (FIRST) {
+                int cn[D];
+                row_slots<D>(a.edge_col, a.cls_e0[r + 1], lane, cn);
+#pragma unroll
+                for (int k = 0; k < D; ++k) vload<W>(x[k], chan_t + (size_t)cn[k] * F);
+            } else {
+#pragma unroll
+                for (int k = 0; k < D; ++k) vload<W>(x[k], Qt + (size_t)qn[k] * F + lane_q);
+            }
         }
 #pragma unroll
         for (int k = 0; k < D; ++k)
@@ -318,7 +360,7 @@
     }
 }
 
-template <int ALGO, int D, int V, typename T>
+template <int ALGO, int D, int V, typename T, bool FIRST = false>
 __global__ __launch_bounds__(kBlock) void check_link_narrow2_kernel(const CheckArgs a, const LinkArgs g)
 {
     constexpr size_t F = 64 * V;
@@ -327,7 +369,7 @@
     const GridPos gp = grid_pos(a.tiles_first);
     const int tile = tile_select<V>(a.tail, a.done, gp.row);
     if (tile < 0) return;
-    if (gp.block >= g.link_blocks) { link_extra_rows<ALGO, V, T>(a, g, tile, gp.block); return; }
+    if (gp.block >= g.link_blocks) { link_extra_rows<ALGO, V, T, FIRST>(a, g, tile, gp.block); return; }
     const int wave = gp.block * kWavesPerBlock + wave_id_in_block();
     const int sub = wave % V;
     int r_begin, r_end;
@@ -354,8 +396,13 @@
     float b0[D], b1[D], b2[D];
     auto load_row = [&](float (&dst)[D], int r) {
         const int e = a.cls_e0[r];
-#pragma unroll
-        for (int k = 0; k < D; ++k) { float t[1]; vload<1>(t, Qt + (size_t)edge_slot(a.qpos, e + k) * F); dst[k] = t[0]; }
+        if constexpr (FIRST) {
+#pragma unroll
+            for (int k = 0; k < D; ++k) { float t[1]; vload<1>(t, chan_t + (size_t)edge_slot(a.edge_col, e + k) * F); dst[k] = t[0]; }
+        } else {
+#pragma unroll
+            for (int k = 0; k < D; ++k) { float t[1]; vload<1>(t, Qt + (size_t)edge_slot(a.qpos, e + k) * F); dst[k] = t[0]; }
+        }
     };
     if (r_begin < r_end) load_row(b0, r_begin);
     if (r_begin + 1 < r_end) load_row(b1, r_begin + 1);
@@ -375,6 +422,10 @@
         float xx[D][1], out[D][1];
 #pragma unroll
         for (int k = 0; k < D; ++k) xx[k][0] = x[k];
+        if constexpr (FIRST) {
+#pragma unroll
+            for (int k = 0; k < D; ++k) first_q<ALGO, 1>(xx[k]);
+        }
         check_node<ALGO, D, 1, T>(xx, out, ms_corr_of(a));
 #pragma unroll
         for (int k = 0; k < D; ++k)
diff --git a/myldpccppapi_amd/csrc/flood_round.hpp b/myldpccppapi_amd/csrc/flood_round.hpp
--- a/myldpccppapi_amd/csrc/flood_round.hpp
+++ b/myldpccppapi_amd/csrc/flood_round.hpp
@@ -3,6 +3,7 @@
 #include "flood_common.hpp"
 #include "ldpc_expf.h"
 #include "llr_input.hpp"
+#include "syn_class_host.hpp"
 
 namespace ldpc {
 
@@ -110,20 +111,54 @@
     TailRef tail;
 };
 
-template <int V> __global__ __launch_bounds__(kBlock) void syndrome_kernel(const SyndromeArgs a)
+template <int V> __device__ __forceinline__ bool syndrome_block(const SyndromeArgs &a, int *tile_out, int *rb_out)
 {
     int tile, rb;
     if (a.tiles > 0) {
         const int xcd = blockIdx.x & 7, j = blockIdx.x >> 3;
         tile = xcd + 8 * (j / a.row_blocks);
         rb = j % a.row_blocks;
-        if (tile >= a.tiles) return;
+        if (tile >= a.tiles) return false;
     } else {
         tile = blockIdx.y;
         rb = blockIdx.x;
     }
     tile = tile_select<V>(a.tail, a.done, tile);
-    if (tile < 0) return;
+    if (tile < 0) return false;
+    *tile_out = tile;
+    *rb_out = rb;
+    return true;
+}
+
+template <int V> __device__ __forceinline__ void syndrome_publish(const uint64_t (&s)[V], uint64_t *fail, int tile)
+{
+    __shared__ uint64_t part[kWavesPerBlock][V];
+#pragma unroll
+    for (int v = 0; v < V; ++v) {
+        uint64_t x = s[v];
+#pragma unroll
+        for (int off = 32; off >= 1; off >>= 1) {
+            const uint32_t lo = __shfl_xor((uint32_t)x, off);
+            const uint32_t hi = __shfl_xor((uint32_t)(x >> 32), off);
+            x |= ((uint64_t)hi << 32) | lo;
+        }
+        if ((threadIdx.x & 63) == 0) part[threadIdx.x >> 6][v] = x;
+    }
+    __syncthreads();
+    if (threadIdx.x < V) {
+        uint64_t x = 0;
+#pragma unroll
+        for (int w = 0; w < kWavesPerBlock; ++w) x |= part[w][threadIdx.x];
+        unsigned long long *dst = reinterpret_cast<unsigned long long *>(&fail[(size_t)tile * V + threadIdx.x]);
+        const uint64_t seen = __hip_atomic_load(dst, __ATOMIC_RELAXED, __HIP_MEMORY_SCOPE_AGENT);
+        if (x & ~seen) atomicOr(dst, (unsigned long long)x);
+    }
+}
+
+template <int V> __global__ __launch_bounds__(kBlock) void syndrome_kernel(const SyndromeArgs a)
+{
+    int tile, rb;
+    if (!syndrome_block<V>(a, &tile, &rb)) return;
     const int m = rb * kBlock + threadIdx.x;
     const uint64_t *hard_t = a.hard + (size_t)tile * (size_t)a.N * V;
     uint64_t s[V];
@@ -136,27 +171,67 @@
             for (int v = 0; v < V; ++v) s[v] ^= hard_t[(size_t)c * V + v];
         }
     }
-    __shared__ uint64_t part[kWavesPerBlock][V];
-#pragma unroll
-    for (int v = 0; v < V; ++v) {
-        uint64_t x = s[v];
-#pragma unroll
-        for (int off = 32; off >= 1; off >>= 1) {
-            const uint32_t lo = __shfl_xor((uint32_t)x, off);
-            const uint32_t hi = __shfl_xor((uint32_t)(x >> 32), off);
-            x |= ((uint64_t)hi << 32) | lo;
-        }
-        if ((threadIdx.x & 63) == 0) part[threadIdx.x >> 6][v] = x;
-    }
-    __syncthreads();
-    if (threadIdx.x < V) {
-        uint64_t x = 0;
-#pragma unroll
-        for (int w = 0; w < kWavesPerBlock; ++w) x |= part[w][threadIdx.x];
-        unsigned long long *dst = reinterpret_cast<unsigned long long *>(&a.fail[(size_t)tile * V + threadIdx.x]);
-        const uint64_t seen = __hip_atomic_load(dst, __ATOMIC_RELAXED, __HIP_MEMORY_SCOPE_AGENT);
-        if (x & ~seen) atomicOr(dst, (unsigned long long)x);
-    }
+    syndrome_publish<V>(s, a.fail, tile);
+}
+
+constexpr int kSynPiece = 8;
+
+typedef uint64_t vu2 __attribute__((ext_vector_type(2)));
+
+template <int V, int D>
+__device__ __forceinline__ void syndrome_piece(const uint64_t *__restrict__ hard_t, const int32_t *__restrict__ ec, uint64_t (&s)[V])
+{
+    int c[D];
+#pragma unroll
+    for (int k = 0; k < D; ++k) c[k] = ec[k];
+    if constexpr (V == 1) {
+        uint64_t w[D];
+#pragma unroll
+        for (int k = 0; k < D; ++k) w[k] = hard_t[c[k]];
+#pragma unroll
+        for (int k = 0; k < D; ++k) s[0] ^= w[k];
+    } else {
+        vu2 w[D][V / 2];
+#pragma unroll
+        for (int k = 0; k < D; ++k)
+#pragma unroll
+            for (int h = 0; h < V / 2; ++h) w[k][h] = *reinterpret_cast<const vu2 *>(hard_t + (size_t)c[k] * V + 2 * h);
+#pragma unroll
+        for (int k = 0; k < D; ++k)
+#pragma unroll
+            for (int h = 0; h < V / 2; ++h) { s[2 * h] ^= w[k][h].x; s[2 * h + 1] ^= w[k][h].y; }
+    }
+}
+
+template <int V> __global__ __launch_bounds__(kBlock) void syndrome_class_kernel(const SyndromeArgs a, const SynClass *__restrict__ cls, int n_classes)
+{
+    int tile, rb;
+    if (!syndrome_block<V>(a, &tile, &rb)) return;
+    int ci = 0;
+    while (ci + 1 < n_classes && rb >= cls[ci + 1].block_begin) ++ci;
+    const int deg = cls[ci].degree;
+    const int i = (rb - cls[ci].block_begin) * kBlock + threadIdx.x;
+    const uint64_t *hard_t = a.hard + (size_t)tile * (size_t)a.N * V;
+    uint64_t s[V];
+#pragma unroll
+    for (int v = 0; v < V; ++v) s[v] = 0;
+    if (i < cls[ci].count) {
+        const int32_t *ec = a.edge_col + cls[ci].e0[i];
+        int k0 = 0;
+        for (; k0 + kSynPiece <= deg; k0 += kSynPiece) syndrome_piece<V, kSynPiece>(hard_t, ec + k0, s);
+        static_assert(kSynPiece == 8, "the remainder switch lists 1 .. kSynPiece - 1");
+        switch (deg - k0) {
+        case 1: syndrome_piece<V, 1>(hard_t, ec + k0, s); break;
+        case 2: syndrome_piece<V, 2>(hard_t, ec + k0, s); break;
+        case 3: syndrome_piece<V, 3>(hard_t, ec + k0, s); break;
+        case 4: syndrome_piece<V, 4>(hard_t, ec + k0, s); break;
+        case 5: syndrome_piece<V, 5>(hard_t, ec + k0, s); break;
+        case 6: syndrome_piece<V, 6>(hard_t, ec + k0, s); break;
+        case 7: syndrome_piece<V, 7>(hard_t, ec + k0, s); break;
+        default: break;
+        }
+    }
+    syndrome_publish<V>(s, a.fail, tile);
 }
 
 struct StateArgs {
diff --git a/myldpccppapi_amd/csrc/flood_tables.hpp b/myldpccppapi_amd/csrc/flood_tables.hpp
--- a/myldpccppapi_amd/csrc/flood_tables.hpp
+++ b/myldpccppapi_amd/csrc/flood_tables.hpp
@@ -22,6 +22,10 @@
     LinkFn link_narrow[kMaxUnrolledDegree + 1] = {};
     LinkFn link_deep[kMaxUnrolledDegree + 1] = {};
     LinkFn link_half[kMaxUnrolledDegree + 1] = {};
+    CheckFn check_first[kMaxUnrolledCheckDegreeMS + 1] = {}, check_wide_first[kMaxUnrolledCheckDegreeMS + 1] = {};
+    CheckGroupFn check_group_first[kCheckBuckets] = {};
+    LinkFn link_first[kMaxUnrolledDegree + 1] = {}, link_narrow_first[kMaxUnrolledDegree + 1] = {},
+           link_deep_first[kMaxUnrolledDegree + 1] = {}, link_half_first[kMaxUnrolledDegree + 1] = {};
     VarFn var[kMaxUnrolledDegree + 1] = {};
     CheckGroupFn check_group[kCheckBuckets] = {};
     int check_group_width = 1;
diff --git a/myldpccppapi_amd/csrc/flood_tables_impl.hpp b/myldpccppapi_amd/csrc/flood_tables_impl.hpp
--- a/myldpccppapi_amd/csrc/flood_tables_impl.hpp
+++ b/myldpccppapi_amd/csrc/flood_tables_impl.hpp
@@ -6,16 +6,18 @@
 namespace tables {
 
 template <int ALGO, int V, typename T, int D> struct FloodTable {
-    static void fill(CheckFn *c, CheckFn *cw, VarFn *v)
+    static void fill(CheckFn *c, CheckFn *cw, VarFn *v, CheckFn *cf, CheckFn *cwf)
     {
         c[D] = check_kernel<ALGO, D, V, 1, T>;
         cw[D] = check_kernel<ALGO, D, V, V, T>;
+        cf[D] = check_kernel<ALGO, D, V, 1, T, ALGO == kAlgoSP>;
+        cwf[D] = check_kernel<ALGO, D, V, V, T, ALGO == kAlgoSP>;
         v[D] = var_kernel<ALGO, D, V, T>;
-        FloodTable<ALGO, V, T, D - 1>::fill(c, cw, v);
+        FloodTable<ALGO, V, T, D - 1>::fill(c, cw, v, cf, cwf);
     }
 };
 template <int ALGO, int V, typename T> struct FloodTable<ALGO, V, T, 0> {
-    static void fill(CheckFn *c, CheckFn *cw, VarFn *v)
+    static void fill(CheckFn *c, CheckFn *cw, VarFn *v, CheckFn *, CheckFn *)
     {
         c[0] = cw[0] = check_kernel_generic<ALGO, V, T>;
         v[0] = var_kernel_generic<ALGO, V, T>;
@@ -23,46 +25,50 @@
 };
 
 template <int ALGO, int V, typename T, int D> struct CheckTableMS {
-    static void fill(CheckFn *c, CheckFn *cw)
+    static void fill(CheckFn *c, CheckFn *cw, CheckFn *cf, CheckFn *cwf)
     {
-        c[D] = cw[D] = check_kernel<ALGO, D, V, 1, T>;
-        CheckTableMS<ALGO, V, T, D - 1>::fill(c, cw);
+        c[D] = cw[D] = cf[D] = cwf[D] = check_kernel<ALGO, D, V, 1, T>;
+        CheckTableMS<ALGO, V, T, D - 1>::fill(c, cw, cf, cwf);
     }
 };
 template <int ALGO, int V, typename T> struct CheckTableMS<ALGO, V, T, kMaxUnrolledDegree> {
-    static void fill(CheckFn *, CheckFn *) {}
+    static void fill(CheckFn *, CheckFn *, CheckFn *, CheckFn *) {}
 };
 
-template <int ALGO, int V, typename T, int D> struct LinkHalf {
+template <int ALGO, int V, typename T, int D, bool FIRST> struct LinkHalf {
     static LinkFn get() { return nullptr; }
 };
-template <int ALGO, typename T, int D> struct LinkHalf<ALGO, 4, T, D> {
-    static LinkFn get() { return check_link_narrow_kernel<ALGO, D, 4, T, 2>; }
+template <int ALGO, typename T, int D, bool FIRST> struct LinkHalf<ALGO, 4, T, D, FIRST> {
+    static LinkFn get() { return check_link_narrow_kernel<ALGO, D, 4, T, 2, FIRST>; }
 };
-template <int ALGO, int V, typename T, int D> struct LinkTable {
+template <int ALGO, int V, typename T, int D, bool FIRST> struct LinkTable {
     static void fill(LinkFn *t, LinkFn *tn, LinkFn *td, LinkFn *th)
     {
-        t[D] = check_link_kernel<ALGO, D, V, T>;
-        tn[D] = check_link_narrow_kernel<ALGO, D, V, T>;
-        td[D] = check_link_narrow2_kernel<ALGO, D, V, T>;
-        th[D] = LinkHalf<ALGO, V, T, D>::get();
-        LinkTable<ALGO, V, T, D - 1>::fill(t, tn, td, th);
+        t[D] = check_link_kernel<ALGO, D, V, T, FIRST>;
+        tn[D] = check_link_narrow_kernel<ALGO, D, V, T, 1, FIRST>;
+        td[D] = check_link_narrow2_kernel<ALGO, D, V, T, FIRST>;
+        th[D] = LinkHalf<ALGO, V, T, D, FIRST>::get();
+        LinkTable<ALGO, V, T, D - 1, FIRST>::fill(t, tn, td, th);
     }
 };
-template <int ALGO, int V, typename T> struct LinkTable<ALGO, V, T, 1> {
+template <int ALGO, int V, typename T, bool FIRST> struct LinkTable<ALGO, V, T, 1, FIRST> {
     static void fill(LinkFn *, LinkFn *, LinkFn *, LinkFn *) {}
 };
 
 template <int ALGO, int V, typename T> void fill_v(FloodFns *f)
 {
     constexpr int DM = kMaxUnrolledDegree;
-    FloodTable<ALGO, V, T, DM>::fill(f->check, f->check_wide, f->var);
-    LinkTable<ALGO, V, T, DM>::fill(f->link, f->link_narrow, f->link_deep, f->link_half);
+    FloodTable<ALGO, V, T, DM>::fill(f->check, f->check_wide, f->var, f->check_first, f->check_wide_first);
+    LinkTable<ALGO, V, T, DM, false>::fill(f->link, f->link_narrow, f->link_deep, f->link_half);
+    LinkTable<ALGO, V, T, DM, true>::fill(f->link_first, f->link_narrow_first, f->link_deep_first, f->link_half_first);
     constexpr int GW = sizeof(T) == 1 ? V : (sizeof(T) == 2 && V == 4) ? 2 : 1;
     f->check_group_width = GW;
     f->check_group[0] = check_group_kernel<ALGO, V, T, 1, 8, GW>;
     f->check_group[1] = check_group_kernel<ALGO, V, T, 9, 16, GW>;
     f->check_group[2] = f->check_group[3] = nullptr;
+    f->check_group_first[0] = check_group_kernel<ALGO, V, T, 1, 8, GW, ALGO == kAlgoSP>;
+    f->check_group_first[1] = check_group_kernel<ALGO, V, T, 9, 16, GW, ALGO == kAlgoSP>;
+    f->check_group_first[2] = f->check_group_first[3] = nullptr;
     f->var_group[0] = var_group_kernel<ALGO, V, T, 1, 4>;
     f->var_group[1] = var_group_kernel<ALGO, V, T, 5, 8>;
     f->var_group[2] = var_group_kernel<ALGO, V, T, 9, 16>;
@@ -71,9 +77,9 @@
     f->init_in[kLlrI8] = init_kernel<ALGO, V, T, int8_t>;
     f->max_check_unrolled = DM;
     if (ALGO != kAlgoSP) {
-        CheckTableMS<ALGO, V, T, kMaxUnrolledCheckDegreeMS>::fill(f->check, f->check_wide);
-        f->check_group[2] = check_group_kernel<ALGO, V, T, 17, 24, GW>;
-        f->check_group[3] = check_group_kernel<ALGO, V, T, 25, 32, GW>;
+        CheckTableMS<ALGO, V, T, kMaxUnrolledCheckDegreeMS>::fill(f->check, f->check_wide, f->check_first, f->check_wide_first);
+        f->check_group[2] = f->check_group_first[2] = check_group_kernel<ALGO, V, T, 17, 24, GW>;
+        f->check_group[3] = f->check_group_first[3] = check_group_kernel<ALGO, V, T, 25, 32, GW>;
         f->max_check_unrolled = kMaxUnrolledCheckDegreeMS;
     }
 }
diff --git a/myldpccppapi_amd/csrc/introspect.hip b/myldpccppapi_amd/csrc/introspect.hip
--- a/myldpccppapi_amd/csrc/introspect.hip
+++ b/myldpccppapi_amd/csrc/introspect.hip
@@ -220,6 +220,22 @@
     return LDPC_OK;
 }
 
+int ldpc_decoder_set_round_tuning(ldpc_decoder *d, int32_t tune_first_chan, int32_t tune_syn_class)
+{
+    if (!d) return set_error(LDPC_ERR_ARG, "decoder is NULL");
+    if (tune_first_chan < 0 || tune_first_chan > 2 || tune_syn_class < 0 || tune_syn_class > 2)
+        return set_error(LDPC_ERR_ARG, "round tuning: each choice is 0 (automatic), 1 (on) or 2 (off), not %d / %d", tune_first_chan, tune_syn_class);
+    for (ldpc_decoder *sh : d->shards) {
+        const int rc = ldpc_decoder_set_round_tuning(sh, tune_first_chan, tune_syn_class);
+        if (rc) return rc;
+    }
+    for (ldpc_decoder *p = d; p; p = p->flood.child.get()) {
+        p->tune.first_chan = tune_first_chan;
+        p->tune.syn_class = tune_syn_class;
+    }
+    return LDPC_OK;
+}
+
 int ldpc_decoder_set_tap(ldpc_decoder *d, int32_t iter)
 {
     if (!d) return set_error(LDPC_ERR_ARG, "decoder is NULL");
diff --git a/myldpccppapi_amd/csrc/syn_class_host.hpp b/myldpccppapi_amd/csrc/syn_class_host.hpp
--- /dev/null
+++ b/myldpccppapi_amd/csrc/syn_class_host.hpp
@@ -0,0 +1,41 @@
+#pragma once
+
+#include <stdint.h>
+
+#include <vector>
+
+namespace ldpc {
+
+struct SynClass {
+    int32_t block_begin;
+    int32_t degree;
+    int32_t count;
+    int32_t pad;
+    const int32_t *e0;
+};
+
+struct SynRows {
+    int32_t degree, count;
+    const int32_t *e0;
+};
+
+inline int syn_class_table(const std::vector<SynRows> &classes, int rows_per_block, std::vector<SynClass> *out)
+{
+    int blocks = 0;
+    out->clear();
+    for (const SynRows &rc : classes) {
+        if (rc.degree <= 0 || rc.count <= 0) continue;
+        out->push_back(SynClass{blocks, rc.degree, rc.count, 0, rc.e0});
+        blocks += (rc.count + rows_per_block - 1) / rows_per_block;
+    }
+    return blocks;
+}
+
+inline int syn_class_of(const SynClass *cls, int n_classes, int rb)
+{
+    int ci = 0;
+    while (ci + 1 < n_classes && rb >= cls[ci + 1].block_begin) ++ci;
+    return ci;
+}
+
+}
diff --git a/myldpccppapi_amd/csrc/tune.hpp b/myldpccppapi_amd/csrc/tune.hpp
--- a/myldpccppapi_amd/csrc/tune.hpp
+++ b/myldpccppapi_amd/csrc/tune.hpp
@@ -13,6 +13,8 @@
     int ldsp_grid = 0, ldsp_per_cu = 0, ldsp_waves = 0;
     int place = 0;
     int q_order = 0;
+    int first_chan = 0;
+    int syn_class = 0;
 };
 
 inline Tune tune_from_config(const ldpc_decoder_config &c)
```

Result: slower. 1096 Mbit/s (-2.8%).
